# bytedance/ps-lite

Hardware: AMD Instinct MI355X
Metric: push+pull GB/s per worker + p50 round-trip µs, 1 MB & 64 MB, at 1/2/4/8 GPUs (higher is better)
Workload: dtype fp32; 1 GPU; model=dense push+pull (ps-lite test_benchmark PUSH_PULL), global_batch=128, seq_len=67108864, parallelism=byteps-joint x1 (worker+server per GPU), mode=dense, msg_bytes=67108864, batch_keys=False, overlap=True, op=assign

## Files before the change

csrc/coalesce_admit.h:

```cpp
#pragma once

#include <cstddef>
#include <cstdint>

namespace xps {
namespace kern {

struct Seg2 {
  void* dst0;
  void* dst1;
  const void* src;
  size_t nbytes;
};

static const int kMaxBatch2 = 64;

enum class Admit {
  kAdmit,
  kFlushFirst,
  kReject,
};

inline bool RangesOverlap(const void* a, const void* b, size_t alen, size_t blen) {
  uintptr_t p = reinterpret_cast<uintptr_t>(a), q = reinterpret_cast<uintptr_t>(b);
  return p < q + blen && q < p + alen;
}

inline Admit CoalesceAdmit(const Seg2* open, int n_open, const Seg2& s) {
  uintptr_t bits = reinterpret_cast<uintptr_t>(s.dst0) | reinterpret_cast<uintptr_t>(s.dst1) |
                   reinterpret_cast<uintptr_t>(s.src) | static_cast<uintptr_t>(s.nbytes);
  if (s.nbytes == 0 || (bits & 15u) != 0) return Admit::kReject;
  if (RangesOverlap(s.dst0, s.dst1, s.nbytes, s.nbytes) ||
      RangesOverlap(s.dst0, s.src, s.nbytes, s.nbytes) ||
      RangesOverlap(s.dst1, s.src, s.nbytes, s.nbytes)) {
    return Admit::kReject;
  }
  if (n_open >= kMaxBatch2) return Admit::kReject;
  for (int i = 0; i < n_open; ++i) {
    const Seg2& o = open[i];
    const void* theirs[3] = {o.dst0, o.dst1, o.src};
    for (const void* t : theirs) {
      if (RangesOverlap(s.dst0, t, s.nbytes, o.nbytes) ||
          RangesOverlap(s.dst1, t, s.nbytes, o.nbytes)) {
        return Admit::kFlushFirst;
      }
    }
    if (RangesOverlap(s.src, o.dst0, s.nbytes, o.nbytes) ||
        RangesOverlap(s.src, o.dst1, s.nbytes, o.nbytes)) {
      return Admit::kFlushFirst;
    }
  }
  return Admit::kAdmit;
}

}
}
```

csrc/customer.cc:

```cpp
#include "customer.h"

#include <chrono>

#include "postoffice.h"

namespace xps {

Customer::Customer(int app_id, int customer_id, RecvHandle handle, Postoffice* po)
    : app_id_(app_id), customer_id_(customer_id), handle_(std::move(handle)), po_(po) {
  po_->AddCustomer(this);
  thread_ = std::thread([this] { Receiving(); });
}

Customer::~Customer() {
  po_->RemoveCustomer(this);
  Message term;
  term.meta.control.cmd = Control::TERMINATE;
  queue_.Push(std::move(term));
  if (thread_.joinable()) thread_.join();
}

int Customer::NewRequest(int recver) {
  std::lock_guard<std::mutex> lk(mu_);
  int expected = recver >= 8 ? 1 : static_cast<int>(po_->GetNodeIDs(recver).size());
  tracker_.emplace_back();
  tracker_.back().expected = expected;
  return static_cast<int>(tracker_.size()) - 1;
}

Customer::Slot* Customer::GetSlot(int ts) {
  std::lock_guard<std::mutex> lk(mu_);
  XPS_CHECK_LT(static_cast<size_t>(ts), tracker_.size());
  return &tracker_[ts];
}

void Customer::WaitRequest(int ts) {
  Slot* s = GetSlot(ts);
  auto deadline = std::chrono::steady_clock::now() + std::chrono::microseconds(150);
  while (s->received.load(std::memory_order_acquire) < s->expected) {
    if (std::chrono::steady_clock::now() >= deadline) break;
  }
  if (s->received.load(std::memory_order_acquire) >= s->expected) return;
  static const int timeout_s = Environment::Get()->GetInt("XPS_WAIT_TIMEOUT_S", 0);
  std::unique_lock<std::mutex> lk(mu_);
  auto done = [s] { return s->received.load(std::memory_order_acquire) >= s->expected; };
  if (timeout_s <= 0) {
    cv_.wait(lk, done);
    return;
  }
  if (!cv_.wait_for(lk, std::chrono::seconds(timeout_s), done)) {
    XPS_LOG(Fatal) << "request ts=" << ts << " (app " << app_id_ << ") got "
                   << s->received.load() << "/" << s->expected << " responses after "
                   << timeout_s << " s — responder dead? (XPS_WAIT_TIMEOUT_S)";
  }
}

bool Customer::IsFinished(int ts) {
  Slot* s = GetSlot(ts);
  return s->received.load(std::memory_order_acquire) >= s->expected;
}

int Customer::NumResponse(int ts) {
  return GetSlot(ts)->received.load(std::memory_order_acquire);
}

void Customer::AddResponse(int ts, int num) {
  Slot* s = GetSlot(ts);
  int got = s->received.fetch_add(num, std::memory_order_acq_rel) + num;
  if (got >= s->expected) {
    std::lock_guard<std::mutex> lk(mu_);
    cv_.notify_all();
  }
}

thread_local int g_in_handler = 0;

bool InCustomerHandler() { return g_in_handler > 0; }

void Customer::RunHandle(Message& msg) {
  g_in_handler++;
  handle_(msg);
  g_in_handler--;
  if (!msg.meta.request) AddResponse(msg.meta.timestamp, 1);
}

void Customer::ProcessInline(Message& msg) {
  XPS_STAGE(customer_process);
  std::lock_guard<std::mutex> lk(handle_mu_);
  RunHandle(msg);
}

void Customer::Receiving() {
  while (true) {
    Message msg;
    queue_.WaitAndPop(&msg);
    if (msg.meta.control.cmd == Control::TERMINATE) break;
    std::lock_guard<std::mutex> lk(handle_mu_);
    RunHandle(msg);
  }
}

}
```

csrc/gpu_plane.cc:

```cpp
#include "gpu_plane.h"

#include <fcntl.h>
#include <hip/hip_runtime.h>
#include <semaphore.h>
#include <sys/prctl.h>
#include <time.h>
#include <unistd.h>

#include <cstring>

#include "hip_pool.h"
#include "host_par.h"
#include "host_pool.h"
#include "kernels.h"
#include "postoffice.h"
#include "wire.h"

namespace xps {

static const size_t kInlineMax = 4096;

#define XPS_HIP_CHECK(cmd)                                                            \
  do {                                                                                \
    hipError_t e_ = (cmd);                                                            \
    XPS_CHECK(e_ == hipSuccess) << "HIP error: " << hipGetErrorString(e_) << " in " #cmd; \
  } while (0)

std::atomic<uint64_t> g_zero_copy_recv{0};
std::atomic<uint64_t> g_fused_assign{0};

bool FusedAssignEnabled() {
  static const bool on = Environment::Get()->GetInt("XPS_FUSED_ASSIGN", 1) != 0;
  return on;
}

std::atomic<uint64_t> g_fused_launches{0};

bool CoalesceEnabled() {
  static const bool on = Environment::Get()->GetInt("XPS_COALESCE", 1) != 0;
  return on;
}

namespace {
struct CoTicket {
  const void* plane = nullptr;
  int peer = 0;
  std::shared_ptr<void> cev;
};
thread_local CoTicket t_co_ticket;

int64_t NowUs() {
  struct timespec ts;
  clock_gettime(CLOCK_MONOTONIC, &ts);
  return static_cast<int64_t>(ts.tv_sec) * 1000000 + ts.tv_nsec / 1000;
}
const int64_t kHoldQuietUs = 2000;
const size_t kCoBusyBytes = 16u << 20;

std::mutex g_map_mu;
struct HandleKey {
  char h[kIpcHandleBytes];
  bool operator==(const HandleKey& o) const { return memcmp(h, o.h, kIpcHandleBytes) == 0; }
};
struct HandleHash {
  size_t operator()(const HandleKey& k) const {
    size_t v = 1469598103934665603ull;
    for (char c : k.h) {
      v ^= static_cast<unsigned char>(c);
      v *= 1099511628211ull;
    }
    return v;
  }
};
std::unordered_map<HandleKey, void*, HandleHash> g_mapped;

class IpcOpenLock {
 public:
  IpcOpenLock() {
    sem_ = sem_open("/xps_ipc_open_lock", O_CREAT, 0600, 1);
  }
  void Lock() {
    if (sem_ == SEM_FAILED) return;
    struct timespec ts;
    clock_gettime(CLOCK_REALTIME, &ts);
    ts.tv_sec += 60;
    if (sem_timedwait(sem_, &ts) != 0) {
      XPS_LOG(Warning) << "ipc-open lock timeout; proceeding unlocked";
      timed_out_ = true;
    }
  }
  void Unlock() {
    if (sem_ != SEM_FAILED && !timed_out_) sem_post(sem_);
    timed_out_ = false;
  }

 private:
  sem_t* sem_ = SEM_FAILED;
  bool timed_out_ = false;
};
IpcOpenLock g_ipc_lock;
}

GpuPlane::GpuPlane(Postoffice* po, int device) : po_(po), device_(device) {
  my_host_hash_ = HostHash();
  inline_deliver_ = Environment::Get()->GetInt("XPS_INLINE_HANDLER", 1) != 0;
  lanes_ = Environment::Get()->GetInt("XPS_STREAMS_PER_PEER", 2);
  if (lanes_ < 1) lanes_ = 1;
  if (lanes_ > 2) lanes_ = 2;
  co_hold_ = Environment::Get()->GetInt("XPS_COALESCE_HOLD", 0) != 0;
  int cap_mb = Environment::Get()->GetInt("XPS_COALESCE_CAP_MB", 1024);
  co_byte_cap_ = static_cast<size_t>(cap_mb < 1 ? 1 : cap_mb) << 20;
}

GpuPlane::~GpuPlane() { Stop(); }

void GpuPlane::FillSelf(Node* self) {
  static std::once_flag gc_once;
  std::call_once(gc_once, [] { HostShmPool::GcStaleSegments(); });
  self->dev_id = device_;
  auto* pool = HbmPool::Get();
  if (device_ >= 0 && pool->initialized()) {
    self->pool_capacity = pool->capacity();
    self->pool_slab_bytes = pool->slab_bytes();
    self->pool_handles.resize(pool->slab_count());
    for (size_t i = 0; i < pool->slab_count(); ++i) {
      memcpy(self->pool_handles[i].data(), pool->slab_handle(i), kIpcHandleBytes);
    }
  }
  auto* hpool = HostShmPool::Get();
  hpool->Init(self->shm_uid);
  self->host_pool_uid = hpool->uid();
  self->host_pool_capacity = hpool->capacity();
  if (!started_) {
    auto* env = Environment::Get();
    if (!env->GetInt("XPS_PROBE_NO_RING", 0)) {
      XPS_CHECK(in_ring_.Create(self->shm_uid)) << "cannot create shm ring";
    }
    started_ = true;
    if (!env->GetInt("XPS_PROBE_NO_POLL", 0)) {
      poll_running_ = true;
      poll_thread_ = std::thread([this] { RingPollLoop(); });
    }
    if (device_ >= 0 && !env->GetInt("XPS_PROBE_NO_COMP", 0)) {
      comp_thread_ = std::thread([this] { CompletionLoop(); });
    }
  }
}

void GpuPlane::Stop() {
  if (stop_.exchange(true)) return;
  PrintStageStats(device_ >= 0 ? "gpu plane" : "host plane");
  if (poll_thread_.joinable()) poll_thread_.join();
  if (comp_thread_.joinable()) comp_thread_.join();
  {
    std::lock_guard<std::mutex> lk(local_mu_);
    for (auto& lm : local_q_) po_->van()->Deliver(std::move(lm.first));
    local_q_.clear();
  }
  if (device_ >= 0) {
    std::vector<Peer*> all;
    {
      std::shared_lock<std::shared_timed_mutex> lk(peers_mu_);
      for (auto& kv : peers_) all.push_back(kv.second.get());
    }
    for (Peer* peer : all) {
      CoFlush(peer);
      std::lock_guard<std::mutex> lk(peer->co.mu);
      peer->co.inflight.clear();
    }
  }
  {
    std::lock_guard<std::mutex> lk(pend_mu_);
    for (auto& kv : pending_) {
      for (auto& p : kv.second) {
        if (p.cev) {
          (void)hipEventSynchronize(p.cev->ev.load(std::memory_order_acquire));
          if (p.local_po) {
            DeliverLocal(p.local_po, p.resend, p.bytes);
          } else {
            Peer* peer = GetPeer(p.peer_id);
            auto ring = peer ? RingOf(peer) : nullptr;
            if (!ring || !ring->Push(p.payload.data(),
                                     static_cast<uint32_t>(p.payload.size()))) {
              (void)po_->van()->SendOverTcp(p.resend, p.peer_id);
            }
          }
          continue;
        }
        (void)hipEventSynchronize(p.ev);
        if (p.local_po) {
          DeliverLocal(p.local_po, p.resend, p.bytes);
          (void)hipEventDestroy(p.ev);
          continue;
        }
        Peer* peer = GetPeer(p.peer_id);
        auto ring = peer ? RingOf(peer) : nullptr;
        bool sent = ring && ring->Push(p.payload.data(),
                                       static_cast<uint32_t>(p.payload.size()));
        if (!sent) {
          (void)po_->van()->SendOverTcp(p.resend, p.peer_id);
        }
        (void)hipEventDestroy(p.ev);
      }
    }
    pending_.clear();
  }
  in_ring_.CloseAndUnlink();
  HostShmPool::Get()->Unlink();
  std::lock_guard<std::mutex> lk(ev_mu_);
  for (auto ev : event_pool_) (void)hipEventDestroy(ev);
  event_pool_.clear();
}

void GpuPlane::OnPeer(const Node& peer) {
  if (peer.host_hash != my_host_hash_) return;
  std::unique_lock<std::shared_timed_mutex> lk(peers_mu_);
  auto& p = peers_[peer.id];
  if (!p) p.reset(new Peer());
  if (p->node.shm_uid != 0 && peer.shm_uid != 0 && p->node.shm_uid != peer.shm_uid) {
    std::lock_guard<std::mutex> lk2(p->mu);
    XPS_LOG(Warning) << "peer " << peer.id << " was recovered (new process); resetting "
                        "plane caches for it";
    p->ring_ok.store(false, std::memory_order_release);
    p->ring_tried = false;
    std::atomic_store_explicit(&p->ring, std::shared_ptr<ShmRing>(),
                               std::memory_order_release);
    p->pool_tried = false;
    p->slab_bases.clear();
    p->local_po.store(nullptr, std::memory_order_release);
  }
  p->node = peer;
}

void GpuPlane::ImportPeers() {
  std::vector<int> ids;
  {
    std::shared_lock<std::shared_timed_mutex> lk(peers_mu_);
    for (auto& kv : peers_) ids.push_back(kv.first);
  }
  for (int id : ids) {
    Peer* p = GetPeer(id);
    if (p->node.pool_capacity) {
      bool ok = ImportPeerSlabs(p);
      XPS_VLOG(1) << "imported pool of peer " << id << " (" << p->node.pool_handles.size()
                  << " slabs): " << (ok ? "ok" : "FAILED");
    }
  }
}

GpuPlane::Peer* GpuPlane::GetPeer(int id) {
  {
    std::shared_lock<std::shared_timed_mutex> lk(peers_mu_);
    auto it = peers_.find(id);
    if (it != peers_.end()) return it->second.get();
  }
  std::unique_lock<std::shared_timed_mutex> lk(peers_mu_);
  auto& p = peers_[id];
  if (!p) {
    p.reset(new Peer());
    p->node = po_->van()->GetNode(id);
  }
  return p.get();
}

bool GpuPlane::EnsureRing(Peer* p) {
  if (p->ring_ok.load(std::memory_order_acquire)) return true;
  std::lock_guard<std::mutex> lk(p->mu);
  {
    auto cur = std::atomic_load_explicit(&p->ring, std::memory_order_acquire);
    if (cur && cur->ok()) return true;
  }
  if (p->ring_tried) return false;
  p->ring_tried = true;
  if (p->node.shm_uid == 0) return false;
  auto ring = std::make_shared<ShmRing>();
  if (!ring->Open(p->node.shm_uid)) return false;
  std::atomic_store_explicit(&p->ring, std::shared_ptr<ShmRing>(std::move(ring)),
                             std::memory_order_release);
  p->ring_ok.store(true, std::memory_order_release);
  return true;
}

std::shared_ptr<ShmRing> GpuPlane::RingOf(Peer* p) {
  if (!EnsureRing(p)) return nullptr;
  return std::atomic_load_explicit(&p->ring, std::memory_order_acquire);
}

bool GpuPlane::ImportPeerSlabs(Peer* p) {
  {
    std::lock_guard<std::mutex> lk(p->mu);
    if (p->pool_tried) return !p->slab_bases.empty();
    p->pool_tried = true;
  }
  std::vector<void*> bases;
  auto* pool = HbmPool::Get();
  size_t nslabs = p->node.pool_handles.size();
  bool same_process =
      pool->initialized() && nslabs == pool->slab_count() &&
      memcmp(p->node.pool_handles[0].data(), pool->slab_handle(0), kIpcHandleBytes) == 0;
  int peer_dev = p->node.dev_id;
  if (!same_process && peer_dev >= 0 && peer_dev != device_ &&
      Environment::Get()->GetInt("XPS_PEER_ACCESS_CHECK", 1)) {
    int ndev = 0;
    (void)hipGetDeviceCount(&ndev);
    if (peer_dev < ndev) {
      int can = 0;
      (void)hipDeviceCanAccessPeer(&can, device_, peer_dev);
      if (!can) {
        XPS_LOG(Warning) << "device " << device_ << " cannot peer-access device " << peer_dev
                         << " (peer node " << p->node.id
                         << "): keeping this peer on the TCP path";
        std::lock_guard<std::mutex> lk(p->mu);
        p->slab_bases.clear();
        return false;
      }
      XPS_HIP_CHECK(hipSetDevice(device_));
      hipError_t pe = hipDeviceEnablePeerAccess(peer_dev, 0);
      if (pe != hipSuccess && pe != hipErrorPeerAccessAlreadyEnabled) {
        XPS_LOG(Warning) << "hipDeviceEnablePeerAccess(" << peer_dev
                         << ") failed: " << hipGetErrorString(pe)
                         << " (continuing; hipIpc lazy enable may still cover it)";
      }
    }
  }
  for (size_t i = 0; i < nslabs; ++i) {
    void* base = nullptr;
    if (same_process) {
      base = pool->slab_base(i);
    } else {
      HandleKey key;
      memcpy(key.h, p->node.pool_handles[i].data(), kIpcHandleBytes);
      std::lock_guard<std::mutex> lk(g_map_mu);
      auto it = g_mapped.find(key);
      if (it != g_mapped.end()) {
        base = it->second;
      } else {
        XPS_HIP_CHECK(hipSetDevice(device_));
        hipIpcMemHandle_t h;
        memcpy(&h, p->node.pool_handles[i].data(), sizeof(h));
        XPS_VLOG(3) << "ipc-open slab " << i << " of peer " << p->node.id;
        g_ipc_lock.Lock();
        hipError_t e = hipIpcOpenMemHandle(&base, h, hipIpcMemLazyEnablePeerAccess);
        g_ipc_lock.Unlock();
        XPS_VLOG(3) << "ipc-open slab " << i << " of peer " << p->node.id << " -> " << base;
        if (e != hipSuccess) {
          XPS_LOG(Warning) << "hipIpcOpenMemHandle(peer " << p->node.id << " slab " << i
                           << ") failed: " << hipGetErrorString(e)
                           << " — peer stays on the TCP path";
          base = nullptr;
        } else {
          char probe[8];
          hipError_t e2 = hipMemcpy(probe, base, sizeof(probe), hipMemcpyDeviceToHost);
          if (e2 != hipSuccess) {
            XPS_LOG(Warning) << "peer " << p->node.id << " slab " << i
                             << " mapped but unreadable (" << hipGetErrorString(e2)
                             << ") — peer stays on the TCP path";
            base = nullptr;
          }
        }
        g_mapped[key] = base;
      }
    }
    if (!base) {
      std::lock_guard<std::mutex> lk(p->mu);
      p->slab_bases.clear();
      return false;
    }
    bases.push_back(base);
  }
  std::lock_guard<std::mutex> lk(p->mu);
  p->slab_bases = std::move(bases);
  return !p->slab_bases.empty();
}

char* GpuPlane::ResolvePeer(Peer* p, uint64_t global_off, uint64_t len) {
  if (!ImportPeerSlabs(p)) return nullptr;
  uint64_t slab_bytes = p->node.pool_slab_bytes;
  if (slab_bytes == 0) return nullptr;
  size_t idx = static_cast<size_t>(global_off / slab_bytes);
  uint64_t local = global_off % slab_bytes;
  std::lock_guard<std::mutex> lk(p->mu);
  if (idx >= p->slab_bases.size() || len > slab_bytes - local) {
    XPS_LOG(Warning) << "peer offset out of bounds: off=" << global_off << " len=" << len
                     << " slab=" << idx;
    return nullptr;
  }
  return static_cast<char*>(p->slab_bases[idx]) + local;
}

hipStream_t GpuPlane::StreamLane(int node_id, int lane) {
  if (lane >= lanes_) lane = lanes_ - 1;
  Peer* p = GetPeer(node_id);
  if (lane == 0) CoFlush(p);
  return RawLane(p, lane);
}

bool GpuPlane::LanesSplit(int node_id) {
  return lanes_ >= 2 && GetPeer(node_id)->node.dev_id != device_;
}


void GpuPlane::CoLaunchLocked(Peer* p) {
  Coalescer& co = p->co;
  if (co.n == 0) return;
  hipStream_t stream = RawLane(p, 0);
  XPS_HIP_CHECK(hipSetDevice(device_));
  if (co.n == 1) {
    const kern::Seg2& s = co.segs[0];
    kern::DenseAssign2(s.dst0, s.dst1, s.src, s.nbytes, stream);
  } else {
    kern::BatchedAssign2(co.segs, co.n, stream);
  }
  g_fused_launches.fetch_add(1, std::memory_order_relaxed);
  hipEvent_t ev = GetEvent();
  XPS_HIP_CHECK(hipEventRecord(ev, stream));
  co.open->bytes = co.bytes;
  co.open->ev.store(ev, std::memory_order_release);
  co.inflight.push_back(std::move(co.open));
  co.open.reset();
  co.n = 0;
  co.bytes = 0;
  co.n_open.store(0, std::memory_order_release);
}

bool GpuPlane::CoBusyLocked(Peer* p) {
  CoPruneLocked(p);
  size_t bytes = 0;
  for (auto& f : p->co.inflight) bytes += f->bytes;
  return p->co.inflight.size() >= 2 && bytes >= kCoBusyBytes;
}

void GpuPlane::CoPruneLocked(Peer* p) {
  auto& fl = p->co.inflight;
  while (!fl.empty()) {
    CoEvent* f = fl.front().get();
    if (!f->done.load(std::memory_order_acquire) &&
        hipEventQuery(f->ev.load(std::memory_order_acquire)) != hipSuccess) {
      break;
    }
    fl.pop_front();
  }
}

void GpuPlane::CoFlush(Peer* p) {
  if (p->co.n_open.load(std::memory_order_acquire) == 0) return;
  std::lock_guard<std::mutex> lk(p->co.mu);
  CoLaunchLocked(p);
}

std::shared_ptr<GpuPlane::CoEvent> GpuPlane::CoAppend(Peer* p, const kern::Seg2& seg) {
  if (!CoalesceEnabled()) return nullptr;
  Coalescer& co = p->co;
  std::lock_guard<std::mutex> lk(co.mu);
  kern::Admit a = kern::CoalesceAdmit(co.segs, co.n, seg);
  if (a != kern::Admit::kAdmit) CoLaunchLocked(p);
  if (a == kern::Admit::kReject) return nullptr;
  if (!co.open) co.open = std::make_shared<CoEvent>(this);
  std::shared_ptr<CoEvent> cev = co.open;
  co.segs[co.n++] = seg;
  co.bytes += seg.nbytes;
  co.n_open.store(co.n, std::memory_order_release);
  if (co.n >= kern::kMaxBatch || co.bytes >= co_byte_cap_) {
    CoLaunchLocked(p);
  } else if (co_hold_) {
    co.last_append_us = NowUs();
  } else {
    if (!CoBusyLocked(p)) CoLaunchLocked(p);
  }
  return cev;
}

bool GpuPlane::CoFrontUnlaunched(Peer* p, const std::shared_ptr<CoEvent>& cev) {
  Coalescer& co = p->co;
  std::lock_guard<std::mutex> lk(co.mu);
  if (co.open != cev) return true;
  if (co_hold_ && NowUs() - co.last_append_us < kHoldQuietUs) return false;
  CoLaunchLocked(p);
  return true;
}

void GpuPlane::CoRetired(Peer* p) {
  Coalescer& co = p->co;
  std::lock_guard<std::mutex> lk(co.mu);
  bool busy = CoBusyLocked(p);
  if (!co_hold_ && !busy) CoLaunchLocked(p);
}

bool GpuPlane::CoalesceAppend(int peer_id, const kern::Seg2& seg) {
  if (device_ < 0) return false;
  std::shared_ptr<CoEvent> cev = CoAppend(GetPeer(peer_id), seg);
  if (!cev) return false;
  t_co_ticket.plane = this;
  t_co_ticket.peer = peer_id;
  t_co_ticket.cev = std::move(cev);
  return true;
}

std::shared_ptr<GpuPlane::CoEvent> GpuPlane::TakeTicket(int peer_id) {
  if (!t_co_ticket.cev || t_co_ticket.plane != this || t_co_ticket.peer != peer_id) {
    return nullptr;
  }
  auto cev = std::static_pointer_cast<CoEvent>(t_co_ticket.cev);
  t_co_ticket.cev.reset();
  return cev;
}

void GpuPlane::CoalesceEnd(int peer_id) {
  if (!t_co_ticket.cev) return;
  t_co_ticket.cev.reset();
  CoFlush(GetPeer(peer_id));
}

hipStream_t GpuPlane::RawLane(Peer* p, int lane) {
  hipStream_t s = p->streams[lane].load(std::memory_order_acquire);
  if (s) return s;
  std::lock_guard<std::mutex> lk(p->mu);
  s = p->streams[lane].load(std::memory_order_relaxed);
  if (!s) {
    XPS_HIP_CHECK(hipSetDevice(device_));
    XPS_HIP_CHECK(hipStreamCreateWithFlags(&s, hipStreamNonBlocking));
    p->streams[lane].store(s, std::memory_order_release);
  }
  return s;
}

hipStream_t GpuPlane::StreamForPeer(int node_id) { return StreamLane(node_id, 0); }

hipStream_t GpuPlane::PullStreamForPeer(int node_id) {
  Peer* p = GetPeer(node_id);
  if (lanes_ < 2 || p->node.dev_id == device_) return StreamLane(node_id, 0);
  CoFlush(p);
  return StreamLane(node_id, 1);
}

std::vector<std::tuple<int, int64_t, int64_t>> GpuPlane::PeerBytes() {
  std::vector<std::tuple<int, int64_t, int64_t>> out;
  std::shared_lock<std::shared_timed_mutex> lk(peers_mu_);
  for (auto& kv : peers_) {
    int64_t tx = kv.second->tx_bytes.load(std::memory_order_relaxed);
    int64_t rx = kv.second->rx_bytes.load(std::memory_order_relaxed);
    if (tx || rx) out.emplace_back(kv.first, tx, rx);
  }
  return out;
}

hipEvent_t GpuPlane::GetEvent() {
  {
    std::lock_guard<std::mutex> lk(ev_mu_);
    if (!event_pool_.empty()) {
      hipEvent_t ev = event_pool_.back();
      event_pool_.pop_back();
      return ev;
    }
  }
  hipEvent_t ev;
  XPS_HIP_CHECK(hipSetDevice(device_));
  XPS_HIP_CHECK(hipEventCreateWithFlags(&ev, hipEventDisableTiming));
  return ev;
}

void GpuPlane::PutEvent(hipEvent_t ev) {
  std::lock_guard<std::mutex> lk(ev_mu_);
  event_pool_.push_back(ev);
}

Postoffice* GpuPlane::LocalPeer(Peer* p) {
  Postoffice* po = p->local_po.load(std::memory_order_acquire);
  if (po) return po;
  if (p->node.id == kEmptyNodeID) return nullptr;
  po = Postoffice::FindByNodeId(p->node.id);
  if (po) p->local_po.store(po, std::memory_order_release);
  return po;
}

static bool KernelLessAck(const Message& msg) {
  return !msg.meta.request && msg.meta.push && (msg.meta.option & kOptInPlace) &&
         (!msg.meta.pull || (msg.meta.option & kOptEntryPush));
}

static bool NeedsStaging(const Message& msg) {
  return !msg.meta.request && msg.meta.pull && msg.data.size() > 1 &&
         msg.data[1].on_device() && msg.data[1].size() > 0 &&
         (!(msg.meta.option & kOptPullAddr) || (msg.meta.option & kOptHostAddr));
}

bool GpuPlane::CanSend(const Message& msg, const Node& peer) {
  if (!started_ || stop_.load()) return false;
  if (peer.host_hash != my_host_hash_ || peer.shm_uid == 0) return false;
  if (LocalPeer(GetPeer(peer.id))) return !NeedsStaging(msg);
  if (peer.pool_capacity) {
    Peer* p = GetPeer(peer.id);
    std::lock_guard<std::mutex> lk(p->mu);
    if (p->pool_tried && p->slab_bases.empty()) return false;
  }
  size_t est = 160 + msg.meta.body.size();
  for (size_t i = 0; i < msg.data.size(); ++i) {
    const auto& d = msg.data[i];
    if (d.on_device()) {
      uint64_t off;
      if (!HbmPool::Get()->OffsetOf(d.data(), &off)) return false;
      est += 24;
      if (!msg.meta.request && msg.meta.pull && i == 1) {
        if (!(msg.meta.option & kOptPullAddr) || (msg.meta.option & kOptHostAddr) ||
            peer.pool_capacity == 0) {
          return false;
        }
      }
    } else if (d.size() > kInlineMax) {
      uint64_t off;
      if (!HostShmPool::Get()->OffsetOf(d.data(), &off)) return false;
      est += 24;
    } else {
      est += 24 + d.size();
    }
  }
  return est <= ShmRing::MaxPayload();
}

bool GpuPlane::Serialize(const Message& msg, const std::vector<char>& by_ref, std::string* out) {
  XPS_STAGE(serialize);
  std::string meta;
  PackMeta(msg.meta, &meta);
  out->clear();
  out->reserve(meta.size() + 64);
  ByteWriter w(out);
  w.U64(meta.size());
  w.Raw(meta.data(), meta.size());
  w.U8(static_cast<uint8_t>(msg.data.size()));
  for (size_t i = 0; i < msg.data.size(); ++i) {
    const auto& d = msg.data[i];
    if (by_ref[i] == 1) {
      uint64_t off = 0;
      XPS_CHECK(HbmPool::Get()->OffsetOf(d.data(), &off));
      w.U8(1);
      w.U64(off);
      w.U64(d.size());
    } else if (by_ref[i] == 2) {
      uint64_t off = 0;
      XPS_CHECK(HostShmPool::Get()->OffsetOf(d.data(), &off));
      w.U8(2);
      w.U64(off);
      w.U64(d.size());
    } else {
      w.U8(0);
      w.U64(d.size());
      w.Raw(d.data(), d.size());
    }
  }
  return out->size() <= ShmRing::MaxPayload();
}

void GpuPlane::DeliverLocal(Postoffice* lpo, Message& msg, int64_t bytes) {
  Van* van = lpo->van();
  if (!van) {
    XPS_LOG(Warning) << "local peer " << msg.meta.recver << " already finalized; dropping";
    return;
  }
  auto* rplane = dynamic_cast<GpuPlane*>(van->plane());
  static const bool queue_req = Environment::Get()->GetInt("XPS_LOCAL_QUEUE_REQ", 0) != 0;
  if (InCustomerHandler() || (queue_req && msg.meta.request)) {
    if (rplane && rplane->poll_running_) {
      rplane->EnqueueLocal(std::move(msg), bytes);
      return;
    }
    XPS_CHECK(!InCustomerHandler())
        << "in-handler local send needs the receiver's poll thread";
  }
  van->recv_bytes_ += bytes;
  for (auto& d : msg.data) {
    if (d.size() && (d.on_device() || d.size() > kInlineMax)) {
      g_zero_copy_recv.fetch_add(1, std::memory_order_relaxed);
    }
  }
  if (inline_deliver_) {
    van->DeliverInline(msg);
  } else {
    van->Deliver(std::move(msg));
  }
}

bool GpuPlane::LocalPullRead(int peer_id, void* dst, uint64_t entry_off, size_t len,
                             Message resp) {
  if (device_ < 0 || !started_ || stop_.load()) return false;
  Peer* p = GetPeer(peer_id);
  char* src = ResolvePeer(p, entry_off, len);
  if (!src) return false;
  XPS_STAGE(local_pull_read);
  hipStream_t stream;
  if (Postoffice* elpo = LocalPeer(p)) {
    auto* rplane = dynamic_cast<GpuPlane*>(elpo->van() ? elpo->van()->plane() : nullptr);
    if (!rplane) return false;
    static const bool queue_req = Environment::Get()->GetInt("XPS_LOCAL_QUEUE_REQ", 0) != 0;
    if (!inline_deliver_ || queue_req) return false;
    stream = rplane->StreamForPeer(po_->node_id());
  } else {
    stream = StreamForPeer(peer_id);
  }
  XPS_HIP_CHECK(hipSetDevice(device_));
  kern::DenseAssign(dst, src, len, stream);
  g_zero_copy_recv.fetch_add(1, std::memory_order_relaxed);
  hipEvent_t ev = GetEvent();
  XPS_HIP_CHECK(hipEventRecord(ev, stream));
  int64_t bytes = static_cast<int64_t>(len) + 64;
  {
    std::lock_guard<std::mutex> lk(pend_mu_);
    pending_[peer_id].push_back(Pending{ev, peer_id, std::string(), std::move(resp), Message(),
                                        bytes, po_});
  }
  pending_count_.fetch_add(1);
  p->rx_bytes.fetch_add(bytes, std::memory_order_relaxed);
  return true;
}

bool GpuPlane::EntryPushPull(Message& msg, Peer* p, int64_t* bytes_out) {
  if (!FusedAssignEnabled()) return false;
  if (!(msg.meta.option & kOptPullAddr) || (msg.meta.option & kOptHostAddr)) return false;
  static const bool local_one_sided =
      Environment::Get()->GetInt("XPS_LOCAL_ONE_SIDED", 0) != 0;
  Postoffice* elpo = LocalPeer(p);
  GpuPlane* rplane =
      elpo ? dynamic_cast<GpuPlane*>(elpo->van() ? elpo->van()->plane() : nullptr) : nullptr;
  bool can = elpo ? (local_one_sided && rplane != nullptr) : EnsureRing(p);
  if (!can) return false;
  SArray<char> vals = msg.data[1];
  size_t len = vals.size();
  if (len == 0) return false;
  char* entry = ResolvePeer(p, msg.meta.entry_addr, len);
  char* dst = static_cast<char*>(HbmPool::Get()->PtrOf(msg.meta.addr, len));
  if (!entry || !dst || !kern::Disjoint3(entry, dst, vals.data(), len)) return false;
  XPS_STAGE(entry_push_pull);
  std::shared_ptr<CoEvent> cev;
  static const bool co_one_sided =
      Environment::Get()->GetInt("XPS_COALESCE_ONE_SIDED", 0) != 0;
  if (!elpo && co_one_sided) cev = CoAppend(p, kern::Seg2{entry, dst, vals.data(), len});
  hipStream_t stream = nullptr;
  if (!cev) {
    stream = elpo ? rplane->StreamForPeer(po_->node_id()) : StreamForPeer(p->node.id);
    XPS_HIP_CHECK(hipSetDevice(device_));
    kern::DenseAssign2(entry, dst, vals.data(), len, stream);
    g_fused_launches.fetch_add(1, std::memory_order_relaxed);
  }
  g_fused_assign.fetch_add(1, std::memory_order_relaxed);
  g_zero_copy_recv.fetch_add(1, std::memory_order_relaxed);
  Message meta_msg;
  meta_msg.meta = msg.meta;
  meta_msg.meta.option |= kOptInPlace;
  meta_msg.meta.val_len = static_cast<int64_t>(len);
  meta_msg.meta.data_type.clear();
  for (size_t i = 0; i < msg.data.size(); ++i) {
    if (i == 1 || msg.data[i].on_device()) continue;
    meta_msg.data.push_back(msg.data[i]);
    meta_msg.meta.data_type.push_back(msg.meta.data_type[i]);
  }
  int64_t bytes = 64 + static_cast<int64_t>(len);
  Message keepalive;
  keepalive.data.push_back(vals);
  std::string payload;
  if (!elpo) {
    std::vector<char> br(meta_msg.data.size(), 0);
    XPS_CHECK(Serialize(meta_msg, br, &payload));
  }
  hipEvent_t ev = nullptr;
  if (!cev) {
    ev = GetEvent();
    XPS_HIP_CHECK(hipEventRecord(ev, stream));
  }
  {
    std::lock_guard<std::mutex> lk(pend_mu_);
    pending_[p->node.id].push_back(Pending{ev, p->node.id, std::move(payload),
                                           std::move(meta_msg), std::move(keepalive), bytes,
                                           elpo, std::move(cev)});
  }
  pending_count_.fetch_add(1);
  p->tx_bytes.fetch_add(bytes, std::memory_order_relaxed);
  *bytes_out = bytes;
  return true;
}

void GpuPlane::EnqueueLocal(Message msg, int64_t bytes) {
  {
    std::lock_guard<std::mutex> lk(local_mu_);
    local_q_.emplace_back(std::move(msg), bytes);
  }
  local_count_.fetch_add(1, std::memory_order_release);
}

int64_t GpuPlane::SendLocal(Message& msg, Peer* p, Postoffice* lpo) {
  XPS_STAGE(plane_send_local);
  bool response = !msg.meta.request;
  int64_t bytes = 64;
  for (auto& d : msg.data) bytes += static_cast<int64_t>(d.size());

  if (response && msg.meta.pull && msg.data.size() > 1 && !msg.data[1].on_device() &&
      msg.data[1].size() > 0 && (msg.meta.option & kOptPullAddr) &&
      (msg.meta.option & kOptHostAddr)) {
    void* base = HostShmPool::MapPeer(p->node.host_pool_uid, p->node.host_pool_capacity);
    SArray<char> vals = msg.data[1];
    if (base && msg.meta.addr <= p->node.host_pool_capacity &&
        vals.size() <= p->node.host_pool_capacity - msg.meta.addr) {
      HostPar::CopyBytes(static_cast<char*>(base) + msg.meta.addr, vals.data(), vals.size());
      g_zero_copy_recv.fetch_add(1, std::memory_order_relaxed);
      Message meta_msg;
      meta_msg.meta = msg.meta;
      meta_msg.meta.option |= kOptInPlace;
      meta_msg.meta.val_len = static_cast<int64_t>(vals.size());
      meta_msg.meta.data_type.clear();
      for (size_t i = 0; i < msg.data.size(); ++i) {
        if (i == 1 || msg.data[i].on_device()) continue;
        SArray<char> copy(msg.data[i].size());
        memcpy(copy.data(), msg.data[i].data(), msg.data[i].size());
        meta_msg.data.push_back(copy);
        meta_msg.meta.data_type.push_back(msg.meta.data_type[i]);
      }
      DeliverLocal(lpo, meta_msg, bytes);
      p->tx_bytes.fetch_add(bytes, std::memory_order_relaxed);
      return bytes;
    }
  }

  if (response && msg.meta.pull && msg.data.size() > 1 && msg.data[1].on_device() &&
      (msg.meta.option & kOptPullAddr) && !(msg.meta.option & kOptHostAddr)) {
    SArray<char> vals = msg.data[1];
    char* dst = ResolvePeer(p, msg.meta.addr, vals.size());
    if (!dst) {
      for (int l = 0; l < lanes_; ++l) (void)hipStreamSynchronize(StreamLane(p->node.id, l));
      return -1;
    }
    hipStream_t stream = (msg.meta.option & kOptPullLane) ? PullStreamForPeer(p->node.id)
                                                          : StreamForPeer(p->node.id);
    XPS_HIP_CHECK(hipSetDevice(device_));
    kern::DenseAssign(dst, vals.data(), vals.size(), stream);
    g_zero_copy_recv.fetch_add(1, std::memory_order_relaxed);
    Message meta_msg;
    meta_msg.meta = msg.meta;
    meta_msg.meta.option |= kOptInPlace;
    meta_msg.meta.val_len = static_cast<int64_t>(vals.size());
    meta_msg.meta.data_type.clear();
    for (size_t i = 0; i < msg.data.size(); ++i) {
      if (i == 1 || msg.data[i].on_device()) continue;
      meta_msg.data.push_back(msg.data[i]);
      meta_msg.meta.data_type.push_back(msg.meta.data_type[i]);
    }
    msg.data.clear();
    Message keepalive;
    keepalive.data.push_back(vals);
    hipEvent_t ev = GetEvent();
    XPS_HIP_CHECK(hipEventRecord(ev, stream));
    {
      std::lock_guard<std::mutex> lk(pend_mu_);
      pending_[p->node.id].push_back(Pending{ev, p->node.id, std::string(),
                                             std::move(meta_msg), std::move(keepalive), bytes,
                                             lpo});
    }
    pending_count_.fetch_add(1);
    p->tx_bytes.fetch_add(bytes, std::memory_order_relaxed);
    return bytes;
  }

  bool kernel_less_ack = KernelLessAck(msg);
  if (response && device_ >= 0 && !kernel_less_ack) {
    XPS_STAGE(local_defer);
    std::shared_ptr<CoEvent> cev = TakeTicket(p->node.id);
    hipEvent_t ev = nullptr;
    if (!cev) {
      hipStream_t stream = (msg.meta.option & kOptPullLane) ? PullStreamForPeer(p->node.id)
                                                            : StreamForPeer(p->node.id);
      ev = GetEvent();
      XPS_HIP_CHECK(hipSetDevice(device_));
      XPS_HIP_CHECK(hipEventRecord(ev, stream));
    }
    Message resend = msg;
    {
      std::lock_guard<std::mutex> lk(pend_mu_);
      pending_[p->node.id].push_back(Pending{ev, p->node.id, std::string(), std::move(resend),
                                             Message(), bytes, lpo, std::move(cev)});
    }
    pending_count_.fetch_add(1);
  } else {
    Message copy = msg;
    if (response) {
      for (auto& d : copy.data) {
        if (!d.on_device() && d.size()) {
          SArray<char> snap(d.size());
          memcpy(snap.data(), d.data(), d.size());
          d = snap;
        }
      }
    }
    DeliverLocal(lpo, copy, bytes);
  }
  p->tx_bytes.fetch_add(bytes, std::memory_order_relaxed);
  return bytes;
}

int64_t GpuPlane::Send(Message& msg, const Node& peer_node) {
  XPS_STAGE(plane_send);
  XPS_VLOG(3) << "plane send -> " << peer_node.id << ": " << msg.DebugString();
  Peer* p = GetPeer(peer_node.id);
  {
    std::lock_guard<std::mutex> lk(p->mu);
    if (p->node.shm_uid == 0) p->node = peer_node;
  }

  static const bool local_one_sided =
      Environment::Get()->GetInt("XPS_LOCAL_ONE_SIDED", 0) != 0;
  if (msg.meta.request && msg.meta.push && !msg.meta.pull &&
      (msg.meta.option & kOptEntryPush) && device_ >= 0 && msg.data.size() > 1 &&
      msg.data[1].on_device()) {
    Postoffice* elpo = LocalPeer(p);
    GpuPlane* rplane =
        elpo ? dynamic_cast<GpuPlane*>(elpo->van() ? elpo->van()->plane() : nullptr) : nullptr;
    bool can = elpo ? (local_one_sided && rplane != nullptr) : EnsureRing(p);
    SArray<char> vals = msg.data[1];
    char* dst = can ? ResolvePeer(p, msg.meta.addr, vals.size()) : nullptr;
    if (dst) {
      XPS_STAGE(entry_push);
      hipStream_t stream = elpo ? rplane->StreamForPeer(po_->node_id())
                                : StreamForPeer(p->node.id);
      XPS_HIP_CHECK(hipSetDevice(device_));
      kern::DenseAssign(dst, vals.data(), vals.size(), stream);
      g_zero_copy_recv.fetch_add(1, std::memory_order_relaxed);
      Message meta_msg;
      meta_msg.meta = msg.meta;
      meta_msg.meta.option |= kOptInPlace;
      meta_msg.meta.val_len = static_cast<int64_t>(vals.size());
      meta_msg.meta.data_type.clear();
      for (size_t i = 0; i < msg.data.size(); ++i) {
        if (i == 1 || msg.data[i].on_device()) continue;
        meta_msg.data.push_back(msg.data[i]);
        meta_msg.meta.data_type.push_back(msg.meta.data_type[i]);
      }
      int64_t bytes = 64 + static_cast<int64_t>(vals.size());
      Message keepalive;
      keepalive.data.push_back(vals);
      std::string payload;
      if (!elpo) {
        std::vector<char> br(meta_msg.data.size(), 0);
        XPS_CHECK(Serialize(meta_msg, br, &payload));
      }
      hipEvent_t ev = GetEvent();
      XPS_HIP_CHECK(hipEventRecord(ev, stream));
      {
        std::lock_guard<std::mutex> lk(pend_mu_);
        pending_[p->node.id].push_back(Pending{ev, p->node.id, std::move(payload),
                                               std::move(meta_msg), std::move(keepalive),
                                               bytes, elpo});
      }
      pending_count_.fetch_add(1);
      p->tx_bytes.fetch_add(bytes, std::memory_order_relaxed);
      return bytes;
    }
    msg.meta.option &= ~kOptEntryPush;
  }

  if (msg.meta.request && msg.meta.push && msg.meta.pull && (msg.meta.option & kOptEntryPush)) {
    int64_t bytes = 0;
    if (device_ >= 0 && msg.data.size() > 1 && msg.data[1].on_device() &&
        EntryPushPull(msg, p, &bytes)) {
      msg.meta.option |= kOptInPlace;
      return bytes;
    }
    msg.meta.option &= ~kOptEntryPush;
    msg.meta.entry_addr = 0;
  }

  if (Postoffice* lpo = LocalPeer(p)) return SendLocal(msg, p, lpo);
  bool response = !msg.meta.request;
  auto sync_peer_lanes = [this, &peer_node] {
    for (int l = 0; l < lanes_; ++l) (void)hipStreamSynchronize(StreamLane(peer_node.id, l));
  };
  if (!EnsureRing(p)) {
    if (response && device_ >= 0) sync_peer_lanes();
    return -1;
  }

  if (response && msg.meta.pull && msg.data.size() > 1 && !msg.data[1].on_device() &&
      msg.data[1].size() > 0 && (msg.meta.option & kOptPullAddr) &&
      (msg.meta.option & kOptHostAddr)) {
    void* base = HostShmPool::MapPeer(p->node.host_pool_uid, p->node.host_pool_capacity);
    SArray<char> vals = msg.data[1];
    if (base && msg.meta.addr <= p->node.host_pool_capacity &&
        vals.size() <= p->node.host_pool_capacity - msg.meta.addr) {
      HostPar::CopyBytes(static_cast<char*>(base) + msg.meta.addr, vals.data(), vals.size());
      Message meta_msg;
      meta_msg.meta = msg.meta;
      meta_msg.meta.option |= kOptInPlace;
      meta_msg.meta.val_len = static_cast<int64_t>(vals.size());
      for (size_t i = 0; i < msg.data.size(); ++i) {
        if (i == 1 || msg.data[i].on_device() || msg.data[i].size() > kInlineMax) continue;
        meta_msg.data.push_back(msg.data[i]);
        meta_msg.meta.data_type.push_back(msg.meta.data_type[i]);
      }
      std::vector<char> br(meta_msg.data.size(), 0);
      std::string payload;
      if (!Serialize(meta_msg, br, &payload)) {
        meta_msg.data.clear();
        meta_msg.meta.data_type.clear();
        XPS_CHECK(Serialize(meta_msg, {}, &payload));
      }
      int64_t bytes = static_cast<int64_t>(vals.size() + payload.size());
      auto ring = RingOf(p);
      if (!ring || !ring->Push(payload.data(), static_cast<uint32_t>(payload.size()))) return -1;
      p->tx_bytes.fetch_add(bytes, std::memory_order_relaxed);
      return bytes;
    }
    return -1;
  }

  if (response && msg.meta.pull && msg.data.size() > 1 && msg.data[1].on_device() &&
      (msg.meta.option & kOptPullAddr)) {
    SArray<char> vals = msg.data[1];
    char* dst = ResolvePeer(p, msg.meta.addr, vals.size());
    if (!dst) {
      sync_peer_lanes();
      return -1;
    }
    hipStream_t stream = (msg.meta.option & kOptPullLane) ? PullStreamForPeer(peer_node.id)
                                                          : StreamForPeer(peer_node.id);
    XPS_HIP_CHECK(hipSetDevice(device_));
    kern::DenseAssign(dst, vals.data(), vals.size(), stream);
    Message meta_msg;
    meta_msg.meta = msg.meta;
    meta_msg.meta.option |= kOptInPlace;
    meta_msg.meta.val_len = static_cast<int64_t>(vals.size());
    meta_msg.meta.data_type.clear();
    for (size_t i = 0; i < msg.data.size(); ++i) {
      if (i == 1 || msg.data[i].on_device()) continue;
      meta_msg.data.push_back(msg.data[i]);
      meta_msg.meta.data_type.push_back(msg.meta.data_type[i]);
    }
    std::vector<char> by_ref(meta_msg.data.size(), 0);
    std::string payload;
    if (!Serialize(meta_msg, by_ref, &payload)) {
      meta_msg.data.clear();
      meta_msg.meta.data_type.clear();
      XPS_CHECK(Serialize(meta_msg, {}, &payload));
    }
    int64_t bytes = static_cast<int64_t>(vals.size() + payload.size());
    msg.data.clear();
    Message keepalive;
    keepalive.data.push_back(vals);
    DeferSendInternal(p, peer_node.id, stream, std::move(meta_msg), std::move(keepalive),
                      std::move(payload), bytes);
    p->tx_bytes.fetch_add(bytes, std::memory_order_relaxed);
    return bytes;
  }

  std::vector<char> by_ref(msg.data.size(), 0);
  int64_t ref_bytes = 0;
  for (size_t i = 0; i < msg.data.size(); ++i) {
    if (msg.data[i].on_device()) {
      by_ref[i] = 1;
      ref_bytes += msg.data[i].size();
      if (i == 1) msg.meta.option |= kOptValsByRef;
    } else if (msg.data[i].size() > kInlineMax) {
      by_ref[i] = 2;
      ref_bytes += msg.data[i].size();
    }
  }
  std::string payload;
  if (!Serialize(msg, by_ref, &payload)) {
    if (response && device_ >= 0) (void)hipStreamSynchronize(StreamForPeer(peer_node.id));
    return -1;
  }
  int64_t bytes = static_cast<int64_t>(payload.size()) + ref_bytes;
  bool kernel_less_ack = KernelLessAck(msg);
  if (response && device_ >= 0 && !kernel_less_ack) {
    hipStream_t stream = (msg.meta.option & kOptPullLane) ? PullStreamForPeer(peer_node.id)
                                                          : StreamForPeer(peer_node.id);
    Message resend = msg;
    DeferSendInternal(p, peer_node.id, stream, std::move(resend), Message(), std::move(payload),
                      bytes);
  } else {
    auto ring = RingOf(p);
    if (!ring || !ring->Push(payload.data(), static_cast<uint32_t>(payload.size()))) return -1;
    XPS_VLOG(3) << "plane send done -> " << peer_node.id;
  }
  p->tx_bytes.fetch_add(bytes, std::memory_order_relaxed);
  return bytes;
}

void GpuPlane::DeferSendInternal(Peer* p, int peer_id, hipStream_t stream, Message resend,
                                 Message keepalive, std::string payload, int64_t bytes) {
  XPS_STAGE(defer_queue);
  XPS_CHECK_GE(device_, 0) << "deferred sends are a GPU-plane feature";
  hipEvent_t ev = GetEvent();
  XPS_HIP_CHECK(hipSetDevice(device_));
  XPS_HIP_CHECK(hipEventRecord(ev, stream));
  {
    std::lock_guard<std::mutex> lk(pend_mu_);
    pending_[peer_id].push_back(Pending{ev, peer_id, std::move(payload), std::move(resend),
                                        std::move(keepalive), bytes});
  }
  pending_count_.fetch_add(1);
  XPS_VLOG(3) << "deferred send queued -> " << peer_id;
}

void GpuPlane::CompletionLoop() {
  XPS_HIP_CHECK(hipSetDevice(device_));
  prctl(PR_SET_TIMERSLACK, 1000);
  const int kSpin = Environment::Get()->GetInt("XPS_POLL_SPIN", 200000);
  int idle = 0;
  std::vector<int> ids;
  while (!stop_.load()) {
    bool did = false;
    if (pending_count_.load(std::memory_order_acquire) > 0) {
      ids.clear();
      {
        std::lock_guard<std::mutex> lk(pend_mu_);
        for (auto& kv : pending_) {
          if (!kv.second.empty()) ids.push_back(kv.first);
        }
      }
      for (int id : ids) {
        while (!stop_.load()) {
          hipEvent_t front_ev = nullptr;
          std::shared_ptr<CoEvent> cev;
          {
            std::lock_guard<std::mutex> lk(pend_mu_);
            auto& dq = pending_[id];
            if (dq.empty()) break;
            front_ev = dq.front().ev;
            cev = dq.front().cev;
          }
          bool retired = false;
          if (cev) {
            front_ev = cev->ev.load(std::memory_order_acquire);
            if (!front_ev) {
              if (!CoFrontUnlaunched(GetPeer(id), cev)) break;
              continue;
            }
          }
          if (!cev || !cev->done.load(std::memory_order_acquire)) {
            hipError_t e = hipEventQuery(front_ev);
            if (e == hipErrorNotReady) break;
            XPS_CHECK(e == hipSuccess) << "hipEventQuery: " << hipGetErrorString(e);
            if (cev) {
              cev->done.store(true, std::memory_order_release);
              retired = true;
            }
          }
          XPS_STAGE(defer_release);
          if (retired) CoRetired(GetPeer(id));
          Pending front;
          {
            std::lock_guard<std::mutex> lk(pend_mu_);
            auto& dq = pending_[id];
            front = std::move(dq.front());
            dq.pop_front();
          }
          pending_count_.fetch_sub(1);
          if (front.local_po) {
            DeliverLocal(front.local_po, front.resend, front.bytes);
            if (front.ev) PutEvent(front.ev);
            did = true;
            continue;
          }
          Peer* peer = GetPeer(front.peer_id);
          auto ring = peer ? RingOf(peer) : nullptr;
          bool sent = ring && ring->Push(front.payload.data(),
                                         static_cast<uint32_t>(front.payload.size()));
          if (sent) {
            XPS_VLOG(3) << "deferred send done -> " << front.peer_id;
          } else {
            XPS_LOG(Warning) << "deferred plane send failed -> " << front.peer_id
                             << "; falling back to TCP";
            if (po_->van()->SendOverTcp(front.resend, front.peer_id) < 0) {
              XPS_LOG(Warning) << "TCP fallback to " << front.peer_id
                               << " failed too (peer dead?)";
            }
          }
          if (front.ev) PutEvent(front.ev);
          did = true;
        }
      }
    }
    if (did) {
      idle = 0;
    } else if (++idle > kSpin) {
      usleep(20);
    }
  }
}

void GpuPlane::RingPollLoop() {
  if (device_ >= 0) XPS_HIP_CHECK(hipSetDevice(device_));
  prctl(PR_SET_TIMERSLACK, 1000);
  const int kSpin = Environment::Get()->GetInt("XPS_POLL_SPIN", 200000);
  std::vector<char> buf(ShmRing::MaxPayload());
  int idle = 0;
  std::deque<std::pair<Message, int64_t>> local;
  while (!stop_.load()) {
    if (local_count_.load(std::memory_order_acquire) > 0) {
      {
        std::lock_guard<std::mutex> lk(local_mu_);
        local.swap(local_q_);
      }
      local_count_.fetch_sub(static_cast<int>(local.size()));
      for (auto& lm : local) {
        XPS_STAGE(local_handle);
        po_->van()->recv_bytes_ += lm.second;
        for (auto& d : lm.first.data) {
          if (d.size() && (d.on_device() || d.size() > kInlineMax)) {
            g_zero_copy_recv.fetch_add(1, std::memory_order_relaxed);
          }
        }
        if (inline_deliver_) {
          po_->van()->DeliverInline(lm.first);
        } else {
          po_->van()->Deliver(std::move(lm.first));
        }
      }
      idle = 0;
      local.clear();
    }
    uint32_t n = in_ring_.Pop(buf.data());
    if (n == 0) {
      if (++idle > kSpin) usleep(20);
      continue;
    }
    idle = 0;
    XPS_STAGE(ring_handle);
    ByteReader r(buf.data(), n);
    uint64_t meta_len = r.U64();
    Message msg;
    {
      std::vector<char> meta(meta_len);
      r.Raw(meta.data(), meta_len);
      UnpackMeta(meta.data(), meta_len, &msg.meta);
    }
    int nblobs = r.U8();
    int64_t ref_bytes = 0;
    bool ok = true;
    for (int i = 0; i < nblobs; ++i) {
      int kind = r.U8();
      if (kind == 0) {
        uint64_t len = r.U64();
        SArray<char> d(len);
        r.Raw(d.data(), len);
        msg.data.push_back(d);
      } else if (kind == 1) {
        uint64_t off = r.U64();
        uint64_t len = r.U64();
        Peer* sender = GetPeer(msg.meta.sender);
        char* ptr = sender ? ResolvePeer(sender, off, len) : nullptr;
        if (!ptr) {
          XPS_LOG(Warning) << "dropping by-ref blob: sender pool not mapped (from "
                           << msg.meta.sender << ")";
          ok = false;
          break;
        }
        msg.data.push_back(SArray<char>(ptr, len, device_));
        ref_bytes += len;
        g_zero_copy_recv.fetch_add(1, std::memory_order_relaxed);
      } else {
        uint64_t off = r.U64();
        uint64_t len = r.U64();
        Peer* sender = GetPeer(msg.meta.sender);
        void* base = sender ? HostShmPool::MapPeer(sender->node.host_pool_uid,
                                                   sender->node.host_pool_capacity)
                            : nullptr;
        if (!base || off > sender->node.host_pool_capacity ||
            len > sender->node.host_pool_capacity - off) {
          XPS_LOG(Warning) << "dropping host-ref blob: sender host pool not mapped (from "
                           << msg.meta.sender << ")";
          ok = false;
          break;
        }
        msg.data.push_back(SArray<char>(static_cast<char*>(base) + off, len, kCPU));
        ref_bytes += len;
        g_zero_copy_recv.fetch_add(1, std::memory_order_relaxed);
      }
    }
    if (!ok) continue;
    XPS_VLOG(3) << "ring recv: " << msg.DebugString();
    po_->van()->recv_bytes_ += n + ref_bytes;
    if (msg.meta.sender != kEmptyNodeID) {
      GetPeer(msg.meta.sender)->rx_bytes.fetch_add(n + ref_bytes, std::memory_order_relaxed);
    }
    if (inline_deliver_) {
      po_->van()->DeliverInline(msg);
    } else {
      po_->van()->Deliver(std::move(msg));
    }
  }
}

std::shared_ptr<DataPlane> CreateGpuPlane(Postoffice* po, int device) {
  return std::make_shared<GpuPlane>(po, device);
}

}
```

csrc/gpu_plane.h:

```cpp
#pragma once

#include <hip/hip_runtime.h>

#include <atomic>
#include <deque>
#include <memory>
#include <shared_mutex>
#include <thread>
#include <tuple>
#include <unordered_map>
#include <vector>

#include "kernels.h"
#include "shm_ring.h"
#include "van.h"

namespace xps {

extern std::atomic<uint64_t> g_zero_copy_recv;
extern std::atomic<uint64_t> g_fused_assign;
bool FusedAssignEnabled();
extern std::atomic<uint64_t> g_fused_launches;
bool CoalesceEnabled();

class Postoffice;

class GpuPlane : public DataPlane {
 public:
  GpuPlane(Postoffice* po, int device);
  ~GpuPlane() override;

  void FillSelf(Node* self) override;
  void ImportPeers() override;
  bool CanSend(const Message& msg, const Node& peer) override;
  int64_t Send(Message& msg, const Node& peer) override;
  void OnPeer(const Node& peer) override;
  void Stop() override;

  hipStream_t StreamForPeer(int node_id);
  hipStream_t PullStreamForPeer(int node_id);
  int lanes() const { return lanes_; }
  bool LanesSplit(int node_id);

  bool CoalesceAppend(int peer_id, const kern::Seg2& seg);
  void CoalesceEnd(int peer_id);
  std::vector<std::tuple<int, int64_t, int64_t>> PeerBytes();
  int device() const { return device_; }

  bool LocalPullRead(int peer_id, void* dst, uint64_t entry_off, size_t len, Message resp);
  hipEvent_t GetEvent();
  void PutEvent(hipEvent_t ev);
  char* PeerDst(int peer_id, uint64_t global_off, uint64_t len) {
    return ResolvePeer(GetPeer(peer_id), global_off, len);
  }

 private:
  struct CoEvent {
    explicit CoEvent(GpuPlane* pl) : plane(pl) {}
    ~CoEvent() {
      if (hipEvent_t e = ev.load(std::memory_order_acquire)) plane->PutEvent(e);
    }
    GpuPlane* plane;
    std::atomic<hipEvent_t> ev{nullptr};
    std::atomic<bool> done{false};
    size_t bytes = 0;
  };
  struct Coalescer {
    std::mutex mu;
    kern::Seg2 segs[kern::kMaxBatch];
    int n = 0;
    std::atomic<int> n_open{0};
    size_t bytes = 0;
    std::shared_ptr<CoEvent> open;
    std::deque<std::shared_ptr<CoEvent>> inflight;
    int64_t last_append_us = 0;
  };

  struct Peer {
    Node node;
    Coalescer co;
    std::atomic<Postoffice*> local_po{nullptr};
    std::shared_ptr<ShmRing> ring;
    bool ring_tried = false;
    std::atomic<bool> ring_ok{false};
    std::vector<void*> slab_bases;
    bool pool_tried = false;
    std::atomic<hipStream_t> streams[2] = {{nullptr}, {nullptr}};
    std::atomic<int64_t> tx_bytes{0};
    std::atomic<int64_t> rx_bytes{0};
    std::mutex mu;
  };

  struct Pending {
    hipEvent_t ev;
    int peer_id;
    std::string payload;
    Message resend;
    Message keepalive;
    int64_t bytes;
    Postoffice* local_po = nullptr;
    std::shared_ptr<CoEvent> cev;
  };

  Peer* GetPeer(int id);
  Postoffice* LocalPeer(Peer* p);
  int64_t SendLocal(Message& msg, Peer* p, Postoffice* lpo);
  void DeliverLocal(Postoffice* lpo, Message& msg, int64_t bytes);
  void EnqueueLocal(Message msg, int64_t bytes);
  bool EnsureRing(Peer* p);
  std::shared_ptr<ShmRing> RingOf(Peer* p);
  bool ImportPeerSlabs(Peer* p);
  char* ResolvePeer(Peer* p, uint64_t global_off, uint64_t len);
  bool Serialize(const Message& msg, const std::vector<char>& by_ref, std::string* out);
  void RingPollLoop();
  void CompletionLoop();
  hipStream_t StreamLane(int node_id, int lane);
  hipStream_t RawLane(Peer* p, int lane);
  std::shared_ptr<CoEvent> CoAppend(Peer* p, const kern::Seg2& seg);
  void CoLaunchLocked(Peer* p);
  void CoPruneLocked(Peer* p);
  bool CoBusyLocked(Peer* p);
  void CoFlush(Peer* p);
  bool CoFrontUnlaunched(Peer* p, const std::shared_ptr<CoEvent>& cev);
  void CoRetired(Peer* p);
  std::shared_ptr<CoEvent> TakeTicket(int peer_id);
  bool EntryPushPull(Message& msg, Peer* p, int64_t* bytes_out);
  void DeferSendInternal(Peer* p, int peer_id, hipStream_t stream, Message resend,
                         Message keepalive, std::string payload, int64_t bytes);

  Postoffice* po_;
  int device_;
  int lanes_ = 2;
  bool co_hold_ = false;
  size_t co_byte_cap_ = 1ull << 30;
  uint64_t my_host_hash_;
  ShmRing in_ring_;
  bool started_ = false;
  bool inline_deliver_ = true;

  std::shared_timed_mutex peers_mu_;
  std::unordered_map<int, std::unique_ptr<Peer>> peers_;

  std::thread poll_thread_;
  std::thread comp_thread_;
  std::atomic<bool> stop_{false};

  std::mutex pend_mu_;
  std::unordered_map<int, std::deque<Pending>> pending_;
  std::atomic<int> pending_count_{0};

  std::mutex local_mu_;
  std::deque<std::pair<Message, int64_t>> local_q_;
  std::atomic<int> local_count_{0};
  bool poll_running_ = false;

  std::mutex ev_mu_;
  std::vector<hipEvent_t> event_pool_;
};

std::shared_ptr<DataPlane> CreateGpuPlane(Postoffice* po, int device);

}
```

csrc/kv_app.h:

```cpp
#pragma once

#include <unistd.h>

#include <algorithm>
#include <atomic>
#include <chrono>
#include <condition_variable>
#include <functional>
#include <mutex>
#include <set>
#include <unordered_map>
#include <vector>

#include "gpu_plane.h"
#include "hip_pool.h"
#include "hip_util.h"
#include "host_par.h"
#include "host_pool.h"
#include "simple_app.h"

namespace xps {

static const int kCmdDefault = 0;
static const int kCmdAssign = 1;
static const int kCmdSum = 2;

template <typename V>
struct KVPairs {
  SArray<Key> keys;
  SArray<V> vals;
  SArray<int> lens;
  SArray<Key> keys_dev;
};

struct KVMeta {
  int cmd = 0;
  bool push = false;
  bool pull = false;
  int sender = kEmptyNodeID;
  int timestamp = -1;
  int customer_id = 0;
  Key key = 0;
  uint64_t addr = 0;
  uint64_t entry_addr = 0;
  int64_t val_len = 0;
  int option = 0;
  int src_dev = kCPU;
  int dst_dev = kCPU;
};

template <typename V>
class KVWorker : public SimpleApp {
 public:
  using Callback = std::function<void()>;
  using SlicedKVs = std::vector<std::pair<bool, KVPairs<V>>>;
  using Slicer = std::function<void(const KVPairs<V>&, const std::vector<Range>&, SlicedKVs*)>;

  explicit KVWorker(int app_id, int customer_id, int instance_idx = 0)
      : SimpleApp(Postoffice::GetWorker(instance_idx), DeferCustomer{}) {
    slicer_ = [this](const KVPairs<V>& s, const std::vector<Range>& r, SlicedKVs* out) {
      DefaultSlicer(s, r, out);
    };
    obj_.reset(new Customer(app_id, customer_id,
                            [this](const Message& m) { Process(m); }, po_));
  }

  int Push(const std::vector<Key>& keys, const std::vector<V>& vals,
           const std::vector<int>& lens = {}, int cmd = 0, const Callback& cb = nullptr) {
    return ZPush(SArray<Key>(keys), SArray<V>(vals), SArray<int>(lens), cmd, cb);
  }

  int Pull(const std::vector<Key>& keys, std::vector<V>* vals, std::vector<int>* lens = nullptr,
           int cmd = 0, const Callback& cb = nullptr) {
    SArray<Key> skeys(keys);
    int ts = AddPullRequest_(skeys, vals, lens, cmd, cb);
    return ts;
  }

  int ZPush(const SArray<Key>& keys, const SArray<V>& vals, const SArray<int>& lens = {},
            int cmd = 0, const Callback& cb = nullptr, const SArray<Key>& keys_dev = {}) {
    int ts = obj_->NewRequest(kServerGroup);
    AddCallback(ts, cb);
    KVPairs<V> kvs;
    kvs.keys = keys;
    kvs.vals = vals;
    kvs.lens = lens;
    kvs.keys_dev = keys_dev;
    Send(ts, true, false, cmd, kvs);
    return ts;
  }

  int ZPushPull(const SArray<Key>& keys, const SArray<V>& vals, SArray<V>* outs,
                const SArray<int>& lens = {}, int cmd = 0, const Callback& cb = nullptr,
                const SArray<Key>& keys_dev = {}) {
    XPS_CHECK(outs && outs->size()) << "ZPushPull needs a pre-sized outs buffer";
    int ts = obj_->NewRequest(kServerGroup);
    {
      std::lock_guard<std::mutex> lk(mu_);
      pull_dst_[ts] = {outs, nullptr};
    }
    AddCallback(ts, cb);
    KVPairs<V> kvs;
    kvs.keys = keys;
    kvs.vals = vals;
    kvs.lens = lens;
    kvs.keys_dev = keys_dev;
    Send(ts, true, true, cmd, kvs, outs);
    return ts;
  }

  int ZPull(const SArray<Key>& keys, SArray<V>* vals, SArray<int>* lens = nullptr, int cmd = 0,
            const Callback& cb = nullptr, const SArray<Key>& keys_dev = {}) {
    XPS_CHECK(vals && vals->size()) << "ZPull needs a pre-sized vals buffer";
    int ts = obj_->NewRequest(kServerGroup);
    {
      std::lock_guard<std::mutex> lk(mu_);
      pull_dst_[ts] = {vals, lens};
    }
    AddCallback(ts, cb);
    KVPairs<V> kvs;
    kvs.keys = keys;
    kvs.vals = *vals;
    if (lens) kvs.lens = *lens;
    kvs.keys_dev = keys_dev;
    Send(ts, false, true, cmd, kvs);
    return ts;
  }

  void Wait(int timestamp) { obj_->WaitRequest(timestamp); }

  bool HasEntry(const Key& key, size_t nbytes) {
    const auto& ranges = po_->GetServerKeyRanges();
    size_t i = 0;
    while (i + 1 < ranges.size() && key >= ranges[i + 1].begin) ++i;
    if (ranges.empty()) return false;
    int sid = ServerRankToID(static_cast<int>(i));
    std::lock_guard<std::mutex> lk(mu_);
    const EntryRec* rec = FindEntryLocked(sid, key);
    return rec && rec->len == static_cast<int64_t>(nbytes) &&
           po_->van()->GetNode(sid).shm_uid == rec->uid;
  }

  void set_slicer(Slicer s) { slicer_ = std::move(s); }

  void DefaultSlicer(const KVPairs<V>& send, const std::vector<Range>& ranges, SlicedKVs* sliced) {
    sliced->resize(ranges.size());
    size_t n = send.keys.size();
    std::vector<size_t> pos(ranges.size() + 1);
    const Key* begin = send.keys.begin();
    const Key* end = send.keys.end();
    for (size_t i = 0; i < ranges.size(); ++i) {
      pos[i] = std::lower_bound(begin, end, ranges[i].begin) - begin;
    }
    pos[ranges.size()] = n;
    std::vector<size_t> val_off(n + 1, 0);
    if (!send.lens.empty()) {
      XPS_CHECK_EQ(send.lens.size(), n);
      for (size_t i = 0; i < n; ++i) val_off[i + 1] = val_off[i] + send.lens[i];
    } else if (n > 0) {
      size_t k = send.vals.size() / n;
      for (size_t i = 0; i <= n; ++i) val_off[i] = i * k;
    }
    for (size_t i = 0; i < ranges.size(); ++i) {
      size_t a = pos[i], b = pos[i + 1];
      auto& out = (*sliced)[i];
      out.first = b > a;
      if (!out.first) continue;
      out.second.keys = send.keys.Segment(a, b);
      if (!send.keys_dev.empty()) {
        out.second.keys_dev = send.keys_dev.Segment(a, b);
      }
      if (!send.vals.empty()) {
        out.second.vals = send.vals.Segment(val_off[a], val_off[b]);
      }
      if (!send.lens.empty()) {
        out.second.lens = send.lens.Segment(a, b);
      }
    }
  }

 private:
  int AddPullRequest_(const SArray<Key>& keys, std::vector<V>* vals, std::vector<int>* lens,
                      int cmd, const Callback& cb) {
    int ts = obj_->NewRequest(kServerGroup);
    {
      std::lock_guard<std::mutex> lk(mu_);
      vec_pull_dst_[ts] = {vals, lens};
    }
    AddCallback(ts, cb);
    KVPairs<V> kvs;
    kvs.keys = keys;
    Send(ts, false, true, cmd, kvs);
    return ts;
  }

  void AddCallback(int ts, const Callback& cb) {
    if (!cb) return;
    std::lock_guard<std::mutex> lk(mu_);
    callbacks_[ts] = cb;
  }

  void Send(int ts, bool push, bool pull, int cmd, KVPairs<V>& kvs, SArray<V>* dst = nullptr) {
    SlicedKVs sliced;
    slicer_(kvs, po_->GetServerKeyRanges(), &sliced);
    int skipped = 0;
    for (auto& s : sliced)
      if (!s.first) ++skipped;
    if (skipped) obj_->AddResponse(ts, skipped);
    {
      std::lock_guard<std::mutex> lk(mu_);
      expected_[ts] = static_cast<int>(sliced.size()) - skipped;
    }
    if (static_cast<int>(sliced.size()) == skipped) {
      RunCallback(ts);
      return;
    }
    size_t val_elem_off = 0;
    for (size_t i = 0; i < sliced.size(); ++i) {
      if (!sliced[i].first) continue;
      auto& s = sliced[i].second;
      Message msg;
      msg.meta.app_id = obj_->app_id();
      msg.meta.customer_id = obj_->customer_id();
      msg.meta.request = true;
      msg.meta.push = push;
      msg.meta.pull = pull;
      msg.meta.head = cmd;
      msg.meta.timestamp = ts;
      msg.meta.recver = ServerRankToID(static_cast<int>(i));
      if (s.keys.size() >= 1) msg.meta.key = s.keys[0];
      msg.meta.src_dev = push ? s.vals.device() : kvs.vals.device();
      msg.meta.dst_dev = msg.meta.src_dev;
      if (!s.keys_dev.empty()) {
        msg.AddData(s.keys_dev);
      } else {
        msg.AddData(s.keys);
      }
      if (push) {
        msg.meta.val_len = static_cast<int64_t>(s.vals.nbytes());
        msg.AddData(s.vals);
        if (!s.lens.empty()) msg.AddData(s.lens);
        {
          std::lock_guard<std::mutex> lk(mu_);
          auto nit = entry_cache_.find(msg.meta.recver);
          if (nit != entry_cache_.end() && !nit->second.empty()) {
            if (!pull && s.keys.size() == 1 && cmd != kCmdSum && s.vals.on_device()) {
              auto it = nit->second.find(s.keys[0]);
              if (it != nit->second.end() &&
                  it->second.len == static_cast<int64_t>(s.vals.nbytes()) &&
                  po_->van()->GetNode(msg.meta.recver).shm_uid == it->second.uid) {
                msg.meta.addr = it->second.off;
                msg.meta.option |= kOptEntryPush;
                it->second.one_sided = true;
              } else if (it != nit->second.end()) {
                it->second.one_sided = false;
              }
            } else {
              for (size_t ki = 0; ki < s.keys.size(); ++ki) {
                auto it = nit->second.find(s.keys[ki]);
                if (it != nit->second.end()) it->second.one_sided = false;
              }
            }
          }
        }
        if (pull && dst) {
          size_t elem_off = static_cast<size_t>(s.vals.data() - kvs.vals.data());
          const V* dptr = dst->data() + elem_off;
          uint64_t off = 0;
          if (dst->on_device()) {
            if (HbmPool::Get()->OffsetOf(dptr, &off)) {
              msg.meta.addr = off;
              msg.meta.option |= kOptPullAddr;
            }
          } else if (HostShmPool::Get()->OffsetOf(dptr, &off)) {
            msg.meta.addr = off;
            msg.meta.option |= kOptPullAddr | kOptHostAddr;
          }
          if (s.keys.size() == 1 && cmd != kCmdSum && s.vals.on_device() &&
              dst->on_device() && (msg.meta.option & kOptPullAddr) && FusedAssignEnabled()) {
            std::lock_guard<std::mutex> lk(mu_);
            const EntryRec* rec = FindEntryLocked(msg.meta.recver, s.keys[0]);
            if (rec && rec->len == static_cast<int64_t>(s.vals.nbytes()) &&
                po_->van()->GetNode(msg.meta.recver).shm_uid == rec->uid) {
              msg.meta.entry_addr = rec->off;
              msg.meta.option |= kOptEntryPush;
            }
          }
        }
      } else {
        if (s.keys.size() == 1 && cmd != kCmdSum && s.vals.on_device() &&
            s.vals.nbytes() > 0) {
          uint64_t eoff = 0;
          bool hit = false;
          {
            std::lock_guard<std::mutex> lk(mu_);
            auto nit = entry_cache_.find(msg.meta.recver);
            if (nit != entry_cache_.end()) {
              auto it = nit->second.find(s.keys[0]);
              if (it != nit->second.end() && it->second.one_sided &&
                  it->second.len == static_cast<int64_t>(s.vals.nbytes()) &&
                  po_->van()->GetNode(msg.meta.recver).shm_uid == it->second.uid) {
                eoff = it->second.off;
                hit = true;
              }
            }
          }
          if (hit) {
            auto* plane = dynamic_cast<GpuPlane*>(po_->van()->plane());
            if (plane) {
              Message resp;
              resp.meta.app_id = obj_->app_id();
              resp.meta.customer_id = obj_->customer_id();
              resp.meta.request = false;
              resp.meta.pull = true;
              resp.meta.head = cmd;
              resp.meta.timestamp = ts;
              resp.meta.sender = msg.meta.recver;
              resp.meta.recver = po_->node_id();
              resp.meta.key = s.keys[0];
              resp.meta.option = kOptInPlace;
              resp.meta.val_len = static_cast<int64_t>(s.vals.nbytes());
              if (plane->LocalPullRead(msg.meta.recver, s.vals.data(), eoff,
                                       s.vals.nbytes(), std::move(resp))) {
                continue;
              }
            }
          }
        }
        msg.meta.val_len = static_cast<int64_t>(s.vals.nbytes());
        if (!s.vals.empty()) {
          uint64_t off = 0;
          if (s.vals.on_device()) {
            if (HbmPool::Get()->OffsetOf(s.vals.data(), &off)) {
              msg.meta.addr = off;
              msg.meta.option |= kOptPullAddr;
            }
          } else if (HostShmPool::Get()->OffsetOf(s.vals.data(), &off)) {
            msg.meta.addr = off;
            msg.meta.option |= kOptPullAddr | kOptHostAddr;
          }
        }
        if (!s.lens.empty()) msg.AddData(s.lens);
      }
      po_->van()->Send(msg);
      if (push && pull && s.keys.size() == 1) {
        bool did = (msg.meta.option & kOptEntryPush) && (msg.meta.option & kOptInPlace);
        std::lock_guard<std::mutex> lk(mu_);
        auto nit = entry_cache_.find(msg.meta.recver);
        if (nit != entry_cache_.end()) {
          auto it = nit->second.find(s.keys[0]);
          if (it != nit->second.end()) it->second.one_sided = did;
        }
      }
      (void)val_elem_off;
    }
  }

  void Process(const Message& msg) {
    if (msg.meta.request) return;
    int ts = msg.meta.timestamp;
    bool last = false;
    KVPairs<V> kvs;
    if (msg.meta.pull) {
      if (!msg.data.empty()) {
        kvs.keys = SArray<Key>::View(msg.data[0]);
        if (msg.data.size() > 1) kvs.vals = SArray<V>::View(msg.data[1]);
        if (msg.data.size() > 2) kvs.lens = SArray<int>::View(msg.data[2]);
      }
      if (kvs.keys.empty() || kvs.keys.on_device()) {
        kvs.keys = SArray<Key>({msg.meta.key});
      }
    }
    {
      std::lock_guard<std::mutex> lk(mu_);
      if (msg.meta.pull) {
        if (msg.meta.push && (msg.meta.option & kOptEntryAddr)) {
          CacheEntryLocked(msg.meta.sender, msg.meta.key, msg.meta.entry_addr, msg.meta.val_len);
        }
        auto& got = recv_kvs_[ts];
        got.push_back(RecvSlice{kvs, msg.meta.option, msg.meta.val_len});
        last = static_cast<int>(got.size()) >= expected_[ts];
      } else {
        if (msg.meta.option & kOptEntryAddr) {
          CacheEntryLocked(msg.meta.sender, msg.meta.key, msg.meta.addr, msg.meta.val_len);
        }
        int n = ++push_acks_[ts];
        last = n >= expected_[ts];
      }
    }
    if (last) {
      if (msg.meta.pull) MergePull(ts);
      RunCallback(ts);
    }
  }

  void MergePull(int ts) {
    std::vector<RecvSlice> got;
    SArray<V>* dst_vals = nullptr;
    SArray<int>* dst_lens = nullptr;
    std::vector<V>* vec_vals = nullptr;
    std::vector<int>* vec_lens = nullptr;
    {
      std::lock_guard<std::mutex> lk(mu_);
      got.swap(recv_kvs_[ts]);
      recv_kvs_.erase(ts);
      auto it = pull_dst_.find(ts);
      if (it != pull_dst_.end()) {
        dst_vals = it->second.first;
        dst_lens = it->second.second;
        pull_dst_.erase(it);
      }
      auto it2 = vec_pull_dst_.find(ts);
      if (it2 != vec_pull_dst_.end()) {
        vec_vals = it2->second.first;
        vec_lens = it2->second.second;
        vec_pull_dst_.erase(it2);
      }
    }
    std::sort(got.begin(), got.end(), [](const RecvSlice& a, const RecvSlice& b) {
      Key ka = a.kvs.keys.empty() ? 0 : a.kvs.keys[0];
      Key kb = b.kvs.keys.empty() ? 0 : b.kvs.keys[0];
      return ka < kb;
    });
    if (vec_vals) {
      vec_vals->clear();
      if (vec_lens) vec_lens->clear();
      for (auto& g : got) {
        vec_vals->insert(vec_vals->end(), g.kvs.vals.begin(), g.kvs.vals.end());
        if (vec_lens) {
          for (size_t i = 0; i < g.kvs.lens.size(); ++i) vec_lens->push_back(g.kvs.lens[i]);
        }
      }
      return;
    }
    if (!dst_vals) return;
    size_t off = 0;
    for (auto& g : got) {
      if (g.option & kOptInPlace) {
        off += static_cast<size_t>(g.val_len) / sizeof(V);
        continue;
      }
      size_t n = g.kvs.vals.size();
      if (n == 0) continue;
      XPS_CHECK_LE(off + n, dst_vals->size()) << "pull response overflows dst";
      if (dst_vals->on_device()) {
        gpu::CopyHostToDevice(dst_vals->data() + off, g.kvs.vals.data(), n * sizeof(V),
                              dst_vals->device());
      } else {
        memcpy(dst_vals->data() + off, g.kvs.vals.data(), n * sizeof(V));
      }
      off += n;
    }
    if (dst_lens && !got.empty()) {
      size_t loff = 0;
      for (auto& g : got) {
        for (size_t i = 0; i < g.kvs.lens.size() && loff < dst_lens->size(); ++i) {
          (*dst_lens)[loff++] = g.kvs.lens[i];
        }
      }
    }
  }

  void RunCallback(int ts) {
    Callback cb;
    {
      std::lock_guard<std::mutex> lk(mu_);
      auto it = callbacks_.find(ts);
      if (it != callbacks_.end()) {
        cb = it->second;
        callbacks_.erase(it);
      }
      expected_.erase(ts);
      push_acks_.erase(ts);
    }
    if (cb) cb();
  }

  struct RecvSlice {
    KVPairs<V> kvs;
    int option = 0;
    int64_t val_len = 0;
  };

  struct EntryRec {
    uint64_t off;
    int64_t len;
    uint64_t uid;
    bool one_sided = false;
  };
  std::unordered_map<int, std::unordered_map<Key, EntryRec>> entry_cache_;

  void CacheEntryLocked(int server_id, Key key, uint64_t off, int64_t len) {
    entry_cache_[server_id][key] = EntryRec{off, len, po_->van()->GetNode(server_id).shm_uid};
  }

  const EntryRec* FindEntryLocked(int server_id, Key key) const {
    auto nit = entry_cache_.find(server_id);
    if (nit == entry_cache_.end()) return nullptr;
    auto it = nit->second.find(key);
    return it == nit->second.end() ? nullptr : &it->second;
  }

  Slicer slicer_;
  std::mutex mu_;
  std::unordered_map<int, Callback> callbacks_;
  std::unordered_map<int, int> expected_;
  std::unordered_map<int, int> push_acks_;
  std::unordered_map<int, std::vector<RecvSlice>> recv_kvs_;
  std::unordered_map<int, std::pair<SArray<V>*, SArray<int>*>> pull_dst_;
  std::unordered_map<int, std::pair<std::vector<V>*, std::vector<int>*>> vec_pull_dst_;
};

template <typename V>
class KVServer : public SimpleApp {
 public:
  using ReqHandle = std::function<void(const KVMeta&, const KVPairs<V>&, KVServer<V>*)>;

  explicit KVServer(int app_id, int instance_idx = 0)
      : SimpleApp(Postoffice::GetServer(instance_idx), DeferCustomer{}) {
    obj_.reset(new Customer(app_id, app_id, [this](const Message& m) { Process(m); }, po_));
  }

  void set_request_handle(ReqHandle h) {
    {
      std::lock_guard<std::mutex> lk(handle_mu_);
      request_handle2_ = std::move(h);
      handle_set_.store(true, std::memory_order_release);
    }
    handle_cv_.notify_all();
  }

  void Response(const KVMeta& req, const KVPairs<V>& res = KVPairs<V>()) {
    Message msg;
    msg.meta.app_id = obj_->app_id();
    msg.meta.customer_id = req.customer_id;
    msg.meta.request = false;
    msg.meta.push = req.push;
    msg.meta.pull = req.pull;
    msg.meta.head = req.cmd;
    msg.meta.timestamp = req.timestamp;
    msg.meta.recver = req.sender;
    msg.meta.key = req.key;
    msg.meta.addr = req.addr;
    msg.meta.entry_addr = req.entry_addr;
    msg.meta.option = req.option;
    msg.meta.val_len = req.val_len;
    msg.meta.src_dev = res.vals.device();
    msg.meta.dst_dev = req.dst_dev;
    if (req.pull && (!res.vals.empty() || !res.keys.empty())) {
      if (!res.vals.empty()) msg.meta.val_len = static_cast<int64_t>(res.vals.nbytes());
      msg.AddData(res.keys);
      msg.AddData(res.vals);
      if (!res.lens.empty()) msg.AddData(res.lens);
    }
    po_->van()->Send(msg);
  }

 private:
  void Process(const Message& msg) {
    if (msg.meta.simple_app) {
      SimpleApp::Process(msg);
      return;
    }
    KVMeta meta;
    meta.cmd = msg.meta.head;
    meta.push = msg.meta.push;
    meta.pull = msg.meta.pull;
    meta.sender = msg.meta.sender;
    meta.timestamp = msg.meta.timestamp;
    meta.customer_id = msg.meta.customer_id;
    meta.key = msg.meta.key;
    meta.addr = msg.meta.addr;
    meta.entry_addr = msg.meta.entry_addr;
    meta.val_len = msg.meta.val_len;
    meta.option = msg.meta.option;
    meta.src_dev = msg.meta.src_dev;
    meta.dst_dev = msg.meta.dst_dev;
    KVPairs<V> kvs;
    if (!msg.data.empty()) {
      kvs.keys = SArray<Key>::View(msg.data[0]);
      if (msg.data.size() > 1 && msg.meta.push) kvs.vals = SArray<V>::View(msg.data[1]);
      size_t lens_idx = msg.meta.push ? 2 : 1;
      if (msg.data.size() > lens_idx) kvs.lens = SArray<int>::View(msg.data[lens_idx]);
    } else if (msg.meta.key || msg.meta.val_len) {
      kvs.keys = SArray<Key>({msg.meta.key});
    }
    if (!handle_set_.load(std::memory_order_acquire)) {
      std::unique_lock<std::mutex> lk(handle_mu_);
      bool ok = handle_cv_.wait_for(lk, std::chrono::seconds(60),
                                    [this] { return handle_set_.load(); });
      XPS_CHECK(ok) << "KVServer has no request handle after 60 s";
    }
    request_handle2_(meta, kvs, this);
  }

  ReqHandle request_handle2_;
  std::mutex handle_mu_;
  std::condition_variable handle_cv_;
  std::atomic<bool> handle_set_{false};
};

inline void SumInto(float* dst, const float* src, size_t n) { HostPar::SumF32(dst, src, n); }
template <typename V>
inline void SumInto(V* dst, const V* src, size_t n) {
  for (size_t j = 0; j < n; ++j) dst[j] += src[j];
}

template <typename V>
struct KVServerDefaultHandle {
  void operator()(const KVMeta& req, const KVPairs<V>& kvs, KVServer<V>* server) {
    size_t n = kvs.keys.size();
    KVPairs<V> res;
    if (req.push) {
      XPS_CHECK(!kvs.vals.on_device()) << "default handle is CPU-only";
      size_t off = 0;
      for (size_t i = 0; i < n; ++i) {
        size_t len = kvs.lens.empty() ? kvs.vals.size() / n : kvs.lens[i];
        auto& entry = store[kvs.keys[i]];
        if (entry.size() < len) entry.resize(len, V(0));
        if (req.cmd == kCmdAssign) {
          HostPar::CopyBytes(entry.data(), kvs.vals.data() + off, len * sizeof(V));
        } else {
          SumInto(entry.data(), kvs.vals.data() + off, len);
        }
        off += len;
      }
    }
    if (req.pull) {
      res.keys = kvs.keys;
      if (n == 1) {
        auto& entry = store[kvs.keys[0]];
        res.vals = SArray<V>(entry.data(), entry.size(), kCPU);
        SArray<int> lens(1);
        lens[0] = static_cast<int>(entry.size());
        res.lens = lens;
      } else {
        size_t total = 0;
        for (size_t i = 0; i < n; ++i) total += store[kvs.keys[i]].size();
        res.vals.Resize(total);
        SArray<int> lens(n);
        size_t off = 0;
        for (size_t i = 0; i < n; ++i) {
          auto& entry = store[kvs.keys[i]];
          std::copy(entry.begin(), entry.end(), res.vals.data() + off);
          off += entry.size();
          lens[i] = static_cast<int>(entry.size());
        }
        res.lens = lens;
      }
    }
    server->Response(req, res);
  }
  std::unordered_map<Key, std::vector<V>> store;
};

template <typename V>
struct KVServerReduceHandle {
  explicit KVServerReduceHandle(int num_workers) : num_workers_(std::max(1, num_workers)) {}

  void operator()(const KVMeta& req, const KVPairs<V>& kvs, KVServer<V>* server) {
    XPS_CHECK(!(req.push && req.pull))
        << "ZPushPull is not supported in reduce mode (pulls are held per round)";
    if (req.push) {
      HandlePush(req, kvs, server);
    } else if (req.pull) {
      HandlePull(req, kvs, server);
    } else {
      server->Response(req);
    }
  }

  struct Group {
    std::vector<Key> keys;
    std::vector<size_t> lens;
    std::vector<V> buf;
    int pushes = 0;
    int pulls = 0;
    std::vector<KVMeta> waiting_pulls;
    std::vector<KVMeta> waiting_next_pulls;
    std::vector<std::pair<KVMeta, KVPairs<V>>> waiting_pushes;
    std::set<int> pulled;
  };
  std::unordered_map<uint64_t, Group> store;
  int num_workers_;

  Group& GroupFor(const SArray<Key>& keys) {
    uint64_t h = 1469598103934665603ull;
    const unsigned char* p = reinterpret_cast<const unsigned char*>(keys.data());
    for (size_t i = 0; i < keys.nbytes(); ++i) {
      h ^= p[i];
      h *= 1099511628211ull;
    }
    Group& g = store[h];
    if (g.keys.empty()) {
      g.keys.assign(keys.begin(), keys.end());
    } else {
      XPS_CHECK(g.keys.size() == keys.size() &&
                std::equal(g.keys.begin(), g.keys.end(), keys.begin()))
          << "reduce mode needs a consistent key->message grouping across workers";
    }
    return g;
  }

 private:
  void HandlePush(const KVMeta& req, const KVPairs<V>& kvs, KVServer<V>* server) {
    XPS_CHECK(!kvs.vals.on_device()) << "KVServerReduceHandle is CPU-only";
    size_t n = kvs.keys.size();
    Group& g = GroupFor(kvs.keys);
    if (g.pushes >= num_workers_) {
      g.waiting_pushes.emplace_back(req, kvs);
      return;
    }
    if (g.lens.size() != n) {
      g.lens.resize(n);
      for (size_t i = 0; i < n; ++i) {
        g.lens[i] = kvs.lens.empty() ? kvs.vals.size() / n : static_cast<size_t>(kvs.lens[i]);
      }
    }
    size_t total = 0;
    for (size_t l : g.lens) total += l;
    if (g.buf.size() < total) g.buf.resize(total, V(0));
    const V* __restrict__ v = kvs.vals.data();
    V* __restrict__ b = g.buf.data();
    if (g.pushes == 0) {
      HostPar::CopyBytes(b, v, total * sizeof(V));
    } else {
      SumInto(b, v, total);
    }
    g.pushes++;
    server->Response(req);
    if (g.pushes >= num_workers_) {
      std::vector<KVMeta> waiting;
      waiting.swap(g.waiting_pulls);
      for (auto& w : waiting) RespondPull(w, g, server);
    }
  }

  void HandlePull(const KVMeta& req, const KVPairs<V>& kvs, KVServer<V>* server) {
    Group& g = GroupFor(kvs.keys);
    if (g.pulled.count(req.sender)) {
      g.waiting_next_pulls.push_back(req);
      return;
    }
    if (g.pushes < num_workers_) {
      g.waiting_pulls.push_back(req);
      return;
    }
    RespondPull(req, g, server);
  }

  void RespondPull(const KVMeta& req, Group& g, KVServer<V>* server) {
    KVPairs<V> res;
    res.keys = SArray<Key>(g.keys);
    res.vals = SArray<V>(g.buf.data(), g.buf.size(), kCPU);
    SArray<int> lens(g.keys.size());
    for (size_t i = 0; i < g.keys.size(); ++i) lens[i] = static_cast<int>(g.lens[i]);
    res.lens = lens;
    server->Response(req, res);
    g.pulled.insert(req.sender);
    g.pulls++;
    if (g.pulls >= num_workers_) {
      g.pushes = 0;
      g.pulls = 0;
      g.pulled.clear();
      std::vector<std::pair<KVMeta, KVPairs<V>>> dpush;
      dpush.swap(g.waiting_pushes);
      for (auto& d : dpush) HandlePush(d.first, d.second, server);
      std::vector<KVMeta> dpull;
      dpull.swap(g.waiting_next_pulls);
      for (auto& d : dpull) {
        if (g.pushes >= num_workers_) {
          RespondPull(d, g, server);
        } else {
          g.waiting_pulls.push_back(d);
        }
      }
    }
  }
};

}
```

csrc/message.h:

```cpp
#pragma once

#include <array>
#include <sstream>
#include <string>
#include <vector>

#include "sarray.h"

namespace xps {

static const int kIpcHandleBytes = 64;

struct Node {
  enum Role : int { SCHEDULER = 0, SERVER = 1, WORKER = 2, JOINT = 3 };
  static const char* RoleStr(int r) {
    static const char* s[] = {"scheduler", "server", "worker", "joint"};
    return (r >= 0 && r < 4) ? s[r] : "?";
  }
  int role = -1;
  int id = kEmptyNodeID;
  std::string hostname;
  int port = -1;
  int aux_id = -1;
  int dev_id = kCPU;
  uint64_t host_hash = 0;
  int is_recovery = 0;
  uint64_t pool_capacity = 0;
  uint64_t pool_slab_bytes = 0;
  std::vector<std::array<char, kIpcHandleBytes>> pool_handles;
  uint64_t shm_uid = 0;
  uint64_t host_pool_uid = 0;
  uint64_t host_pool_capacity = 0;

  std::string DebugString() const {
    std::ostringstream os;
    os << "role=" << RoleStr(role) << " id=" << id << " addr=" << hostname << ":" << port
       << " dev=" << dev_id << " aux=" << aux_id << (is_recovery ? " recovery" : "");
    return os.str();
  }
};

struct Control {
  enum Command : int { EMPTY = 0, ADD_NODE, BARRIER, HEARTBEAT, TERMINATE, ACK, HANDSHAKE };
  int cmd = EMPTY;
  std::vector<Node> node;
  int barrier_group = 0;
  int barrier_token = 0;
  int instance_barrier = 0;
  uint64_t msg_sig = 0;
  bool empty() const { return cmd == EMPTY; }
  std::string DebugString() const {
    std::ostringstream os;
    static const char* names[] = {"EMPTY",     "ADD_NODE", "BARRIER",  "HEARTBEAT",
                                  "TERMINATE", "ACK",      "HANDSHAKE"};
    os << "cmd=" << names[cmd];
    if (cmd == BARRIER) os << " group=" << barrier_group << " tok=" << barrier_token;
    for (auto& n : node) os << " {" << n.DebugString() << "}";
    return os.str();
  }
};

static const int kOptInPlace = 1;
static const int kOptValsByRef = 2;
static const int kOptPullAddr = 4;
static const int kOptHostAddr = 8;
static const int kOptPullLane = 16;
static const int kOptEntryAddr = 32;
static const int kOptEntryPush = 64;

enum DataType : int { kChar = 0, kInt32, kInt64, kUint64, kFloat32, kFloat64, kUint8 };
inline size_t DataTypeSize(int t) {
  switch (t) {
    case kChar: case kUint8: return 1;
    case kInt32: case kFloat32: return 4;
    default: return 8;
  }
}

struct Meta {
  static const int kEmpty = -1;
  int app_id = kEmpty;
  int customer_id = kEmpty;
  int timestamp = kEmpty;
  int sender = kEmptyNodeID;
  int recver = kEmptyNodeID;
  bool request = false;
  bool push = false;
  bool pull = false;
  bool simple_app = false;
  int head = kEmpty;
  std::string body;
  Key key = 0;
  uint64_t addr = 0;
  uint64_t entry_addr = 0;
  int64_t val_len = 0;
  int option = 0;
  uint64_t msg_sig = 0;
  uint64_t seq = 0;
  std::vector<int> data_type;
  int src_dev = kCPU;
  int dst_dev = kCPU;
  Control control;

  std::string DebugString() const {
    std::ostringstream os;
    os << "meta[app=" << app_id << " cust=" << customer_id << " ts=" << timestamp
       << " " << sender << "->" << recver
       << (request ? " req" : " res") << (push ? " push" : "") << (pull ? " pull" : "")
       << " key=" << key << " val_len=" << val_len;
    if (!control.empty()) os << " ctrl{" << control.DebugString() << "}";
    os << "]";
    return os.str();
  }
};

struct Message {
  Meta meta;
  std::vector<SArray<char>> data;

  template <typename V>
  void AddData(const SArray<V>& v) {
    XPS_CHECK_LT(data.size(), 4u);
    meta.data_type.push_back(DataTypeOf<V>());
    data.push_back(SArray<char>::View(v));
  }

  template <typename V>
  static int DataTypeOf();

  std::string DebugString() const {
    std::ostringstream os;
    os << meta.DebugString();
    if (!data.empty()) {
      os << " data:[";
      for (auto& d : data) os << d.size() << (d.on_device() ? "d" : "h") << ",";
      os << "]";
    }
    return os.str();
  }
};

template <> inline int Message::DataTypeOf<char>() { return kChar; }
template <> inline int Message::DataTypeOf<uint8_t>() { return kUint8; }
template <> inline int Message::DataTypeOf<int>() { return kInt32; }
template <> inline int Message::DataTypeOf<int64_t>() { return kInt64; }
template <> inline int Message::DataTypeOf<uint64_t>() { return kUint64; }
template <> inline int Message::DataTypeOf<float>() { return kFloat32; }
template <> inline int Message::DataTypeOf<double>() { return kFloat64; }

}
```

csrc/postoffice.cc:

```cpp
#include "postoffice.h"

#include <chrono>

#include "van.h"

namespace xps {

Postoffice::Postoffice(int role, int instance_idx) : role_(role), instance_idx_(instance_idx) {}

Postoffice::~Postoffice() = default;

void Postoffice::EnsureVan() {
  if (!van_) van_.reset(new Van(this));
}

void Postoffice::Start(int customer_id, bool do_barrier) {
  if (started_) return;
  auto* env = Environment::Get();
  num_workers_ = env->GetInt("DMLC_NUM_WORKER", 0);
  num_servers_ = env->GetInt("DMLC_NUM_SERVER", 0);
  node_id_ = kEmptyNodeID;
  {
    std::lock_guard<std::mutex> lk(mu_);
    server_key_ranges_.clear();
  }
  EnsureVan();
  started_ = true;
  van_->Start(customer_id);
  if (van_->my_node().is_recovery) do_barrier = false;
  if (do_barrier) {
    Barrier(customer_id, kScheduler | kServerGroup | kWorkerGroup);
  }
  if (do_barrier && !is_scheduler()) {
    for (int id : GetNodeIDs(kServerGroup | kWorkerGroup)) {
      if (id == node_id_ && van_->plane()) van_->plane()->ImportPeers();
      Barrier(customer_id, kServerGroup | kWorkerGroup);
    }
  }
}

void Postoffice::Finalize(int customer_id, bool do_barrier) {
  if (!started_) return;
  if (do_barrier) {
    Barrier(customer_id, kScheduler | kServerGroup | kWorkerGroup);
  }
  van_->Stop();
  van_.reset();
  started_ = false;
  if (exit_cb_) exit_cb_();
}

int Postoffice::my_rank() const { return IDtoRank(node_id_); }

std::vector<int> Postoffice::GetNodeIDs(int group) const {
  std::vector<int> ids;
  if (group & kScheduler) ids.push_back(kScheduler);
  if (group & kServerGroup) {
    for (int r = 0; r < num_servers_; ++r) ids.push_back(ServerRankToID(r));
  }
  if (group & kWorkerGroup) {
    for (int r = 0; r < num_workers_; ++r) ids.push_back(WorkerRankToID(r));
  }
  return ids;
}

const std::vector<Range>& Postoffice::GetServerKeyRanges() {
  std::lock_guard<std::mutex> lk(mu_);
  if (server_key_ranges_.empty()) {
    int n = std::max(num_servers_, 1);
    uint64_t step = kMaxKey / n;
    for (int i = 0; i < n; ++i) {
      Range r;
      r.begin = step * i;
      r.end = (i == n - 1) ? kMaxKey : step * (i + 1);
      server_key_ranges_.push_back(r);
    }
  }
  return server_key_ranges_;
}

void Postoffice::AddCustomer(Customer* c) {
  std::lock_guard<std::mutex> lk(mu_);
  int key = (c->app_id() << 16) | (c->customer_id() & 0xFFFF);
  XPS_CHECK_EQ(customers_.count(key), 0u)
      << "duplicate customer app=" << c->app_id() << " id=" << c->customer_id();
  customers_[key] = c;
  customer_cv_.notify_all();
}

void Postoffice::RemoveCustomer(Customer* c) {
  std::lock_guard<std::mutex> lk(mu_);
  customers_.erase((c->app_id() << 16) | (c->customer_id() & 0xFFFF));
}

Customer* Postoffice::GetCustomer(int app_id, int customer_id, int timeout_sec) const {
  int key = (app_id << 16) | (customer_id & 0xFFFF);
  std::unique_lock<std::mutex> lk(mu_);
  bool ok = customer_cv_.wait_for(lk, std::chrono::seconds(timeout_sec),
                                  [&] { return customers_.count(key) > 0; });
  return ok ? customers_.at(key) : nullptr;
}

void Postoffice::Barrier(int customer_id, int group) {
  XPS_CHECK(van_->IsReady());
  int token;
  {
    std::lock_guard<std::mutex> lk(barrier_mu_);
    barrier_done_ = false;
    token = ++barrier_seq_;
    barrier_token_ = token;
    barrier_group_ = group;
  }
  Message req;
  req.meta.control.cmd = Control::BARRIER;
  req.meta.control.barrier_group = group;
  req.meta.request = true;
  req.meta.recver = kScheduler;
  req.meta.app_id = 0;
  req.meta.customer_id = customer_id;
  req.meta.timestamp = token;
  van_->Send(req);
  std::unique_lock<std::mutex> lk(barrier_mu_);
  barrier_cv_.wait(lk, [this] { return barrier_done_; });
}

void Postoffice::Manage(const Message& msg) {
  if (msg.meta.control.cmd == Control::BARRIER && !msg.meta.request) {
    std::lock_guard<std::mutex> lk(barrier_mu_);
    if (msg.meta.control.barrier_group != barrier_group_ ||
        msg.meta.timestamp != barrier_token_) {
      XPS_VLOG(2) << "ignoring stale barrier response (group "
                  << msg.meta.control.barrier_group << " token " << msg.meta.timestamp << ")";
      return;
    }
    barrier_done_ = true;
    barrier_cv_.notify_all();
  }
}

void Postoffice::UpdateHeartbeat(int node_id, time_t t) {
  std::lock_guard<std::mutex> lk(heartbeat_mu_);
  heartbeats_[node_id] = t;
}

std::vector<int> Postoffice::GetDeadNodes(int timeout_sec) {
  std::vector<int> dead;
  if (!van_->IsReady() || timeout_sec == 0) return dead;
  time_t now = time(nullptr);
  std::lock_guard<std::mutex> lk(heartbeat_mu_);
  for (int id : GetNodeIDs(kWorkerGroup | kServerGroup)) {
    auto it = heartbeats_.find(id);
    if ((it == heartbeats_.end() || it->second + timeout_sec < now) &&
        start_time_ + timeout_sec < now) {
      dead.push_back(id);
    }
  }
  return dead;
}

namespace {
std::mutex reg_mu;
std::unique_ptr<Postoffice> reg_scheduler;
std::vector<std::unique_ptr<Postoffice>> reg_servers;
std::vector<std::unique_ptr<Postoffice>> reg_workers;
}

Postoffice* Postoffice::GetScheduler() {
  std::lock_guard<std::mutex> lk(reg_mu);
  if (!reg_scheduler) reg_scheduler.reset(new Postoffice(Node::SCHEDULER));
  return reg_scheduler.get();
}

Postoffice* Postoffice::GetServer(int idx) {
  std::lock_guard<std::mutex> lk(reg_mu);
  while (static_cast<int>(reg_servers.size()) <= idx) {
    reg_servers.emplace_back(new Postoffice(Node::SERVER, reg_servers.size()));
  }
  return reg_servers[idx].get();
}

Postoffice* Postoffice::GetWorker(int idx) {
  std::lock_guard<std::mutex> lk(reg_mu);
  while (static_cast<int>(reg_workers.size()) <= idx) {
    reg_workers.emplace_back(new Postoffice(Node::WORKER, reg_workers.size()));
  }
  return reg_workers[idx].get();
}

Postoffice* Postoffice::FindByNodeId(int id) {
  std::lock_guard<std::mutex> lk(reg_mu);
  auto match = [id](Postoffice* po) {
    return po && po->started_ && po->node_id_ == id && po->van_ && po->van_->IsReady();
  };
  if (match(reg_scheduler.get())) return reg_scheduler.get();
  for (auto& p : reg_servers) {
    if (match(p.get())) return p.get();
  }
  for (auto& p : reg_workers) {
    if (match(p.get())) return p.get();
  }
  return nullptr;
}

void Postoffice::ClearRegistry() {
  std::lock_guard<std::mutex> lk(reg_mu);
  if (reg_scheduler) reg_scheduler.release();
  for (auto& p : reg_servers) p.release();
  for (auto& p : reg_workers) p.release();
  reg_servers.clear();
  reg_workers.clear();
}

}
```

csrc/postoffice.h:

```cpp
#pragma once

#include <atomic>
#include <condition_variable>
#include <memory>
#include <mutex>
#include <unordered_map>
#include <vector>

#include "customer.h"
#include "message.h"

namespace xps {

class Van;

struct Range {
  uint64_t begin = 0;
  uint64_t end = 0;
  uint64_t size() const { return end - begin; }
};

class Postoffice {
 public:
  Postoffice(int role, int instance_idx = 0);
  ~Postoffice();

  void EnsureVan();
  void Start(int customer_id, bool do_barrier);
  void Finalize(int customer_id, bool do_barrier);

  Van* van() const { return van_.get(); }
  int role() const { return role_; }
  bool is_worker() const { return role_ == Node::WORKER; }
  bool is_server() const { return role_ == Node::SERVER; }
  bool is_scheduler() const { return role_ == Node::SCHEDULER; }
  int num_workers() const { return num_workers_; }
  int num_servers() const { return num_servers_; }
  int instance_idx() const { return instance_idx_; }

  int my_rank() const;
  int node_id() const { return node_id_; }
  void set_node_id(int id) { node_id_ = id; }
  int preferred_rank() const { return preferred_rank_; }
  void set_preferred_rank(int r) { preferred_rank_ = r; }

  std::vector<int> GetNodeIDs(int group) const;
  const std::vector<Range>& GetServerKeyRanges();

  void AddCustomer(Customer* c);
  void RemoveCustomer(Customer* c);
  Customer* GetCustomer(int app_id, int customer_id, int timeout_sec = 15) const;

  void Barrier(int customer_id, int group);
  void Manage(const Message& msg);

  void UpdateHeartbeat(int node_id, time_t t);
  std::vector<int> GetDeadNodes(int timeout_sec = 60);

  void RegisterExitCallback(std::function<void()> cb) { exit_cb_ = std::move(cb); }

  static Postoffice* GetScheduler();
  static Postoffice* GetServer(int idx = 0);
  static Postoffice* GetWorker(int idx = 0);
  static Postoffice* FindByNodeId(int id);
  static void ClearRegistry();

 private:
  friend class Van;

  int role_;
  int instance_idx_;
  std::atomic<int> node_id_{kEmptyNodeID};
  int preferred_rank_ = -1;
  int num_workers_ = 0;
  int num_servers_ = 0;
  std::unique_ptr<Van> van_;
  bool started_ = false;

  mutable std::mutex mu_;
  std::unordered_map<int, Customer*> customers_;
  mutable std::condition_variable customer_cv_;

  std::mutex barrier_mu_;
  std::condition_variable barrier_cv_;
  bool barrier_done_ = false;
  int barrier_seq_ = 0;
  int barrier_token_ = 0;
  int barrier_group_ = 0;

  std::mutex heartbeat_mu_;
  std::unordered_map<int, time_t> heartbeats_;
  time_t start_time_ = time(nullptr);

  std::vector<Range> server_key_ranges_;
  std::function<void()> exit_cb_;
};

}
```

csrc/pybind.cc:

```cpp
#include <pybind11/functional.h>
#include <pybind11/numpy.h>
#include <pybind11/pybind11.h>
#include <pybind11/stl.h>

#include <atomic>
#include <thread>

#include "gpu_plane.h"
#include "hip_pool.h"
#include "hip_util.h"
#include "host_pool.h"
#include "kernels.h"
#include "kv_app.h"
#include "kv_utils.h"
#include "ps.h"
#include "server_handlers.h"
#include "shm_ring.h"
#include "simple_app.h"
#include "tile_runs.h"
#include "van.h"
#include "wire.h"

namespace py = pybind11;
using namespace xps;
// ... 238 lines not shown
      fclose(f);
    } else {
      XPS_LOG(Fatal) << "no checkpointable handler installed";
    }
  }

  void LoadCheckpoint(const std::string& path) {
    py::gil_scoped_release rel;
    if (dense_) {
      dense_->Load(path);
    } else if (sparse_) {
      sparse_->Load(path);
    } else if (default_ || reduce_) {
      FILE* f = fopen(path.c_str(), "rb");
      XPS_CHECK(f) << "cannot open checkpoint " << path;
      uint64_t n = 0;
      XPS_CHECK_EQ(fread(&n, 8, 1, f), 1u);
      for (uint64_t i = 0; i < n; ++i) {
        uint64_t key, len;
        XPS_CHECK_EQ(fread(&key, 8, 1, f), 1u);
        XPS_CHECK_EQ(fread(&len, 8, 1, f), 1u);
        auto& v = default_ ? default_->store[key]
                           : reduce_->store[key].buf;
        v.resize(len / sizeof(float));
        XPS_CHECK_EQ(fread(v.data(), 1, len, f), len);
      }
      fclose(f);
    } else {
      XPS_LOG(Fatal) << "no checkpointable handler installed";
    }
  }

  void SetGpuDenseHandle(const std::string& mode, const std::string& dtype) {
    DenseMode m = mode == "sum" ? DenseMode::kSum
                  : mode == "reduce" ? DenseMode::kReduce
                                     : DenseMode::kAssign;
    DenseDtype d = dtype == "bf16" ? DenseDtype::kBf16 : DenseDtype::kF32;
    auto h = std::make_shared<GpuDenseHandler>(s_.postoffice(), m, d);
    dense_ = h;
    s_.set_request_handle([h](const KVMeta& m2, const KVPairs<float>& kvs, KVServer<float>* srv) {
      (*h)(m2, kvs, srv);
    });
  }

  void SetGpuSparseHandle(size_t rows, size_t row_len, bool accumulate, int key_shift) {
    auto h = std::make_shared<GpuSparseHandler>(s_.postoffice(), rows, row_len, accumulate,
                                                key_shift);
    sparse_ = h;
    s_.set_request_handle([h](const KVMeta& m, const KVPairs<float>& kvs, KVServer<float>* srv) {
      (*h)(m, kvs, srv);
    });
  }

  uintptr_t SparseTablePtr() const { return sparse_ ? sparse_->table_ptr() : 0; }

  void SetPythonHandle(py::function fn) {
    s_.set_request_handle([fn](const KVMeta& m, const KVPairs<float>& kvs, KVServer<float>* srv) {
      KVPairs<float> res;
      {
        py::gil_scoped_acquire gil;
        py::dict meta;
        meta["cmd"] = m.cmd;
        meta["push"] = m.push;
        meta["pull"] = m.pull;
        meta["sender"] = m.sender;
        meta["timestamp"] = m.timestamp;
        meta["key"] = m.key;
        meta["val_len"] = m.val_len;
        py::array_t<uint64_t> keys(kvs.keys.size());
        std::copy(kvs.keys.begin(), kvs.keys.end(), keys.mutable_data());
        py::array_t<float> vals(kvs.vals.size());
        if (kvs.vals.size()) {
          XPS_CHECK(!kvs.vals.on_device()) << "python handle got device vals";
          std::copy(kvs.vals.begin(), kvs.vals.end(), vals.mutable_data());
        }
        py::object out = fn(meta, keys, vals);
        if (m.pull) {
          XPS_CHECK(!out.is_none()) << "pull handler must return vals";
          auto arr = py::cast<py::array_t<float>>(out);
          res.keys = kvs.keys;
          res.vals.CopyFrom(arr.data(), arr.size());
          size_t n = kvs.keys.size();
          SArray<int> lens(n);
          for (size_t i = 0; i < n; ++i) lens[i] = static_cast<int>(arr.size() / n);
          res.lens = lens;
        }
      }
      srv->Response(m, res);
    });
  }

 private:
  KVServer<float> s_;
  std::shared_ptr<GpuSparseHandler> sparse_;
  std::shared_ptr<GpuDenseHandler> dense_;
  std::shared_ptr<KVServerDefaultHandle<float>> default_;
  std::shared_ptr<KVServerReduceHandle<float>> reduce_;
};

class PySimpleApp {
 public:
  PySimpleApp(const std::string& role, int app_id, int customer_id)
      : app_(app_id, role == "worker" ? customer_id : app_id, GetPO(role)) {}

  void SetRequestHandle(py::function fn) {
    app_.set_request_handle([fn](const SimpleData& d, SimpleApp* app) {
      std::string reply;
      {
        py::gil_scoped_acquire gil;
        py::object out = fn(d.head, py::bytes(d.body));
        if (!out.is_none()) reply = py::cast<std::string>(out);
      }
      app->Response(d, reply);
    });
  }

  void SetResponseHandle(py::function fn) {
    app_.set_response_handle([fn](const SimpleData& d, SimpleApp*) {
      py::gil_scoped_acquire gil;
      fn(d.head, py::bytes(d.body));
    });
  }

  int Request(int head, const std::string& body, int recver) {
    py::gil_scoped_release rel;
    return app_.Request(head, body, recver);
  }

  void Wait(int ts) {
    py::gil_scoped_release rel;
    app_.Wait(ts);
  }

 private:
  SimpleApp app_;
};

}

PYBIND11_MODULE(_core, m) {
  m.doc() = "xps: MI355X-native parameter-server core";

  m.def("init_env", [](const std::map<std::string, std::string>& kv) {
    Environment::Get()->Init(kv);
  });
  m.def("env", [](const std::string& k) { return Environment::Get()->GetStr(k, ""); });
  m.def("start",
        [](int customer_id, const std::string& role, int rank, bool barrier, int device) {
          py::gil_scoped_release rel;
          Start(customer_id, role, rank, barrier, device);
        },
        py::arg("customer_id") = 0, py::arg("role") = "worker", py::arg("rank") = -1,
        py::arg("barrier") = true, py::arg("device") = -2);
  m.def("finalize",
        [](int customer_id, const std::string& role, bool barrier) {
          py::gil_scoped_release rel;
          Finalize(customer_id, role, barrier);
        },
        py::arg("customer_id") = 0, py::arg("role") = "worker", py::arg("barrier") = true);
  m.def("clear_registry", []() { Postoffice::ClearRegistry(); });
  m.def("barrier", [](const std::string& role, int group, int idx) {
    py::gil_scoped_release rel;
    GetPO(role, idx)->Barrier(0, group);
  }, py::arg("role"), py::arg("group"), py::arg("idx") = 0);
  m.def("num_workers", &NumWorkers);
  m.def("num_servers", &NumServers);
  m.def("my_rank", [](const std::string& role, int idx) { return GetPO(role, idx)->my_rank(); },
        py::arg("role"), py::arg("idx") = 0);
  m.def("node_id", [](const std::string& role, int idx) { return GetPO(role, idx)->node_id(); },
        py::arg("role"), py::arg("idx") = 0);
  m.def("send_bytes", [](const std::string& role) {
    auto* van = GetPO(role)->van();
    return van ? van->send_bytes_.load() : int64_t(0);
  });
  m.def("recv_bytes", [](const std::string& role) {
    auto* van = GetPO(role)->van();
    return van ? van->recv_bytes_.load() : int64_t(0);
  });
  m.def("gpu_count", []() { return gpu::DeviceCount(); });
  m.def("device_sync", [](int dev) {
    py::gil_scoped_release rel;
    gpu::DeviceSync(dev);
  }, py::arg("dev") = -1);

  m.attr("SCHEDULER_GROUP") = kScheduler;
  m.attr("SERVER_GROUP") = kServerGroup;
  m.attr("WORKER_GROUP") = kWorkerGroup;

  m.def("pool_init", [](int device, size_t capacity) { HbmPool::Get()->Init(device, capacity); },
        py::arg("device"), py::arg("capacity") = 0);
  m.def("pool_ipc_handle", [](size_t slab) {
    return py::bytes(HbmPool::Get()->slab_handle(slab), kIpcHandleBytes);
  }, py::arg("slab") = 0);
  m.def("make_stream_events", []() {
    py::gil_scoped_release rel;
    hipStream_t s;
    XPS_CHECK(hipStreamCreateWithFlags(&s, hipStreamNonBlocking) == hipSuccess);
    hipEvent_t ev;
    XPS_CHECK(hipEventCreateWithFlags(&ev, hipEventDisableTiming) == hipSuccess);
    XPS_CHECK(hipEventRecord(ev, s) == hipSuccess);
    while (hipEventQuery(ev) != hipSuccess) {}
    return reinterpret_cast<uintptr_t>(s);
  });
  m.def("kernel_on_stream", [](uintptr_t stream, uintptr_t dst, uintptr_t src, size_t n) {
    py::gil_scoped_release rel;
    kern::DenseSumF32(reinterpret_cast<float*>(dst), reinterpret_cast<float*>(src), n,
                      reinterpret_cast<hipStream_t>(stream));
    hipEvent_t ev;
    XPS_CHECK(hipEventCreateWithFlags(&ev, hipEventDisableTiming) == hipSuccess);
    XPS_CHECK(hipEventRecord(ev, reinterpret_cast<hipStream_t>(stream)) == hipSuccess);
    while (hipEventQuery(ev) != hipSuccess) {}
    (void)hipEventDestroy(ev);
  });
  m.def("ipc_open", [](py::bytes handle) {
    std::string h = handle;
    py::gil_scoped_release rel;
    hipIpcMemHandle_t hh;
    memcpy(&hh, h.data(), sizeof(hh));
    void* ptr = nullptr;
    hipError_t e = hipIpcOpenMemHandle(&ptr, hh, hipIpcMemLazyEnablePeerAccess);
    XPS_CHECK(e == hipSuccess) << "hipIpcOpenMemHandle: " << hipGetErrorString(e);
    return reinterpret_cast<uintptr_t>(ptr);
  });
  m.def("pool_in_use", []() { return HbmPool::Get()->bytes_in_use(); });
  m.def("pool_contains", [](uintptr_t p) {
    uint64_t off = 0;
    return HbmPool::Get()->OffsetOf(reinterpret_cast<const void*>(p), &off);
  });
  py::class_<PoolBuffer>(m, "PoolBuffer")
      .def_property_readonly("ptr", &PoolBuffer::ptr)
      .def_property_readonly("nbytes", &PoolBuffer::nbytes)
      .def_property_readonly("device", &PoolBuffer::device)
      .def("copy_from", &PoolBuffer::copy_from)
      .def("to_numpy_f32", &PoolBuffer::to_numpy_f32);
  m.def("pool_alloc", [](size_t nbytes) {
    PoolBuffer b;
    b.arr = HbmPool::Get()->AllocArray(nbytes);
    return b;
  });
  m.def("host_alloc", [](size_t nbytes) {
    PoolBuffer b;
    b.arr = HostShmPool::Get()->AllocArray(nbytes);
    return b;
  });

  py::class_<PyKVWorker>(m, "KVWorker")
      .def(py::init<int, int, int>(), py::arg("app_id") = 0, py::arg("customer_id") = 0,
           py::arg("instance_idx") = 0)
      .def("push", &PyKVWorker::Push, py::arg("keys"), py::arg("vals"),
           py::arg("lens") = py::array_t<int>())
      .def("pull", &PyKVWorker::PullBlocking, py::arg("keys"))
      .def("zpush_ptr", &PyKVWorker::ZPushPtr, py::arg("keys"), py::arg("vals_ptr"),
           py::arg("vals_bytes"), py::arg("device"), py::arg("lens") = py::array_t<int>(),
           py::arg("cmd") = 0, py::arg("keys_dev_ptr") = 0)
      .def("zpushpull_ptr", &PyKVWorker::ZPushPullPtr, py::arg("keys"), py::arg("vals_ptr"),
           py::arg("out_ptr"), py::arg("nbytes"), py::arg("device") = -1,
           py::arg("lens") = py::array_t<int>(), py::arg("cmd") = 0,
           py::arg("keys_dev_ptr") = 0)
      .def("zpull_ptr", &PyKVWorker::ZPullPtr, py::arg("keys"), py::arg("vals_ptr"),
           py::arg("vals_bytes"), py::arg("device"), py::arg("lens") = py::array_t<int>(),
           py::arg("cmd") = 0, py::arg("keys_dev_ptr") = 0)
      .def("wait", &PyKVWorker::Wait)
      .def("round", &PyKVWorker::Round, py::arg("keys"), py::arg("ptrs"), py::arg("nbytes"),
           py::arg("device"), py::arg("cmd") = 0, py::arg("pull") = false)
      .def("round_mixed", &PyKVWorker::RoundMixed, py::arg("keys"), py::arg("push_ptrs"),
           py::arg("pull_ptrs"), py::arg("sizes"), py::arg("device"), py::arg("cmd") = 0,
           py::arg("overlap") = true);

  py::class_<PyKVServer>(m, "KVServer")
      .def(py::init<int, int>(), py::arg("app_id") = 0, py::arg("instance_idx") = 0)
      .def("set_default_handle", &PyKVServer::SetDefaultHandle)
      .def("set_reduce_handle", &PyKVServer::SetReduceHandle, py::arg("num_workers"))
      .def("set_gpu_dense_handle", &PyKVServer::SetGpuDenseHandle, py::arg("mode") = "assign",
           py::arg("dtype") = "f32")
      .def("set_gpu_sparse_handle", &PyKVServer::SetGpuSparseHandle, py::arg("rows"),
           py::arg("row_len"), py::arg("accumulate") = true, py::arg("key_shift") = 0)
      .def("register_entry", &PyKVServer::RegisterEntry, py::arg("key"), py::arg("ptr"),
           py::arg("nbytes"), py::arg("device") = 0)
      .def("sparse_table_ptr", &PyKVServer::SparseTablePtr)
      .def("save_checkpoint", &PyKVServer::SaveCheckpoint)
      .def("load_checkpoint", &PyKVServer::LoadCheckpoint)
      .def("set_python_handle", &PyKVServer::SetPythonHandle);

  m.def("zero_copy_recv_count", []() { return g_zero_copy_recv.load(); });
  m.def("fused_assign_count", []() { return g_fused_assign.load(); });
  m.def("fused_assign_launches", []() { return g_fused_launches.load(); });
  m.def("coalesce_admit",
        [](const std::vector<std::tuple<uintptr_t, uintptr_t, uintptr_t, size_t>>& open,
           const std::tuple<uintptr_t, uintptr_t, uintptr_t, size_t>& seg) {
          auto conv = [](const std::tuple<uintptr_t, uintptr_t, uintptr_t, size_t>& t) {
            return kern::Seg2{reinterpret_cast<void*>(std::get<0>(t)),
                              reinterpret_cast<void*>(std::get<1>(t)),
                              reinterpret_cast<const void*>(std::get<2>(t)), std::get<3>(t)};
          };
          std::vector<kern::Seg2> segs;
          for (auto& t : open) segs.push_back(conv(t));
          switch (kern::CoalesceAdmit(segs.data(), static_cast<int>(segs.size()), conv(seg))) {
            case kern::Admit::kAdmit: return "admit";
            case kern::Admit::kFlushFirst: return "flush";
            default: return "reject";
          }
        },
        py::arg("open"), py::arg("seg"));
  m.def("tile_runs",
        [](const std::vector<unsigned long long>& chunk_counts,
           unsigned long long chunks_per_block, unsigned long long block_index) {
          if (chunks_per_block == 0) throw std::invalid_argument("tile_runs: empty tile");
          std::vector<unsigned long long> prefix(chunk_counts.size() + 1, 0);
          for (size_t i = 0; i < chunk_counts.size(); ++i) {
            if (chunk_counts[i] == 0) throw std::invalid_argument("tile_runs: empty segment");
            prefix[i + 1] = prefix[i] + chunk_counts[i];
          }
          int n = static_cast<int>(chunk_counts.size());
          std::vector<std::tuple<int, unsigned long long, unsigned long long>> out;
          kern::TileRunIter it = kern::TileRunsBegin(prefix.data(), n, chunks_per_block,
                                                     block_index);
          kern::TileRun run;
          while (kern::TileRunsNext(prefix.data(), &it, &run)) {
            out.emplace_back(run.seg, run.lo, run.hi);
          }
          return out;
        },
        py::arg("chunk_counts"), py::arg("chunks_per_block"), py::arg("block_index"));

  m.def("plane_peer_bytes", [](const std::string& role, int idx) {
    py::dict out;
    auto* po = GetPO(role, idx);
    auto* plane = po->van() ? dynamic_cast<GpuPlane*>(po->van()->plane()) : nullptr;
    if (plane) {
      for (auto& t : plane->PeerBytes()) {
        out[py::int_(std::get<0>(t))] = py::make_tuple(std::get<1>(t), std::get<2>(t));
      }
    }
    return out;
  }, py::arg("role") = "worker", py::arg("idx") = 0);

  m.def("_order_nodes", [](std::vector<std::tuple<std::string, std::string, int>> in) {
    std::vector<Node> nodes;
    for (auto& t : in) {
      Node n;
      n.role = std::get<0>(t) == "worker" ? Node::WORKER : Node::SERVER;
      n.hostname = std::get<1>(t);
      n.port = std::get<2>(t);
      nodes.push_back(n);
    }
    auto less = NodeRankOrder(nodes);
    std::sort(nodes.begin(), nodes.end(), less);
    std::vector<std::tuple<std::string, std::string, int>> out;
    for (auto& n : nodes) {
      out.emplace_back(n.role == Node::WORKER ? "worker" : "server", n.hostname, n.port);
    }
    return out;
  });

  m.def("_host_pool_init_for_test", [](uint64_t uid, size_t bytes) {
    HostShmPool::Get()->Init(uid, bytes);
  });
  m.def("_gc_stale_shm", []() { HostShmPool::GcStaleSegments(); });

  m.def("_ring_stress", [](int producers, int per, int payload) {
    ShmRing ring;
    XPS_CHECK(ring.Create(0xabcdef12345ull + getpid()));
    std::atomic<long> received{0}, sum{0}, pushed{0};
    std::atomic<bool> done{false};
    std::thread consumer([&]() {
      std::vector<char> buf(ShmRing::MaxPayload());
      while (true) {
        uint32_t n = ring.Pop(buf.data());
        if (n == 0) {
          if (done.load() && received.load() >= pushed.load()) break;
          std::this_thread::yield();
          continue;
        }
        long v = 0;
        for (uint32_t i = 0; i < n; ++i) v += static_cast<unsigned char>(buf[i]);
        sum.fetch_add(v);
        received.fetch_add(1);
      }
    });
    std::vector<std::thread> ps;
    std::atomic<long> expect{0};
    for (int p = 0; p < producers; ++p) {
      ps.emplace_back([&, p]() {
        std::vector<char> msg(payload);
        for (int i = 0; i < per; ++i) {
          for (int b = 0; b < payload; ++b) msg[b] = static_cast<char>((p + i + b) & 0x7f);
          long v = 0;
          for (int b = 0; b < payload; ++b) v += static_cast<unsigned char>(msg[b]);
          if (ring.Push(msg.data(), payload)) {
            expect.fetch_add(v);
            pushed.fetch_add(1);
          }
        }
      });
    }
    for (auto& t : ps) t.join();
    done.store(true);
    consumer.join();
    ring.CloseAndUnlink();
    return py::make_tuple(static_cast<long>(received.load()),
                          static_cast<long>(pushed.load()),
                          sum.load() == expect.load());
  });

  m.def("_test_meta_roundtrip", []() {
    Meta m;
    m.app_id = 7;
    m.customer_id = 3;
    m.timestamp = 42;
    m.sender = 9;
    m.recver = 8;
    m.request = true;
    m.push = true;
    m.head = 2;
    m.body = "hello\x00world";
    m.key = 0xDEADBEEFCAFEull;
    m.addr = 1234567;
    m.val_len = 1 << 20;
    m.option = kOptPullAddr | kOptHostAddr;
    m.seq = 987654321;
    m.data_type = {kUint64, kFloat32, kInt32};
    m.control.cmd = Control::ADD_NODE;
    Node n;
    n.role = Node::WORKER;
    n.id = 11;
    n.hostname = "10.0.0.5";
    n.port = 1234;
    n.shm_uid = 0x1122334455667788ull;
    n.host_pool_uid = 77;
    n.host_pool_capacity = 1 << 30;
    n.pool_capacity = 2ull << 30;
    n.pool_slab_bytes = 1ull << 30;
    n.pool_handles.resize(2);
    n.pool_handles[0][0] = 'x';
    n.pool_handles[1][63] = 'y';
    m.control.node.push_back(n);
    std::string buf;
    PackMeta(m, &buf);
    Meta out;
    UnpackMeta(buf.data(), buf.size(), &out);
    bool ok = out.app_id == m.app_id && out.customer_id == m.customer_id &&
              out.timestamp == m.timestamp && out.sender == m.sender &&
              out.recver == m.recver && out.request == m.request && out.push == m.push &&
              out.head == m.head && out.body == m.body && out.key == m.key &&
              out.addr == m.addr && out.val_len == m.val_len && out.option == m.option &&
              out.seq == m.seq &&
              out.data_type == m.data_type && out.control.cmd == m.control.cmd &&
              out.control.node.size() == 1;
    auto& on = out.control.node[0];
    ok = ok && on.role == n.role && on.id == n.id && on.hostname == n.hostname &&
         on.port == n.port && on.shm_uid == n.shm_uid && on.host_pool_uid == n.host_pool_uid &&
         on.host_pool_capacity == n.host_pool_capacity && on.pool_capacity == n.pool_capacity &&
         on.pool_slab_bytes == n.pool_slab_bytes && on.pool_handles.size() == 2 &&
         on.pool_handles[0][0] == 'x' && on.pool_handles[1][63] == 'y';
    return ok;
  });

  m.def("_pack_meta_sample", []() {
    Meta m;
    m.app_id = 1;
    m.body = "abc";
    m.control.cmd = Control::ADD_NODE;
    Node n;
    n.hostname = "127.0.0.1";
    n.pool_handles.resize(1);
    m.control.node.push_back(n);
    std::string buf;
    PackMeta(m, &buf);
    return py::bytes(buf);
  });
  m.def("_meta_roundtrip_fields",
        [](int app_id, int customer_id, int timestamp, int sender, int recver, bool request,
           bool push, bool pull, bool simple_app, int head, const std::string& body, uint64_t key,
           uint64_t addr, int64_t val_len, int option, uint64_t msg_sig, uint64_t seq,
           const std::string& hostname, int port, uint64_t shm_uid, int nhandles) {
          Meta m;
          m.app_id = app_id;
          m.customer_id = customer_id;
          m.timestamp = timestamp;
          m.sender = sender;
          m.recver = recver;
          m.request = request;
          m.push = push;
          m.pull = pull;
          m.simple_app = simple_app;
          m.head = head;
          m.body = body;
          m.key = key;
          m.addr = addr;
          m.val_len = val_len;
          m.option = option;
          m.msg_sig = msg_sig;
          m.seq = seq;
          m.control.cmd = Control::ADD_NODE;
          Node n;
          n.hostname = hostname;
          n.port = port;
          n.shm_uid = shm_uid;
          n.pool_handles.resize(nhandles);
          m.control.node.push_back(n);
          std::string buf;
          PackMeta(m, &buf);
          Meta o;
          UnpackMeta(buf.data(), buf.size(), &o);
          auto& on = o.control.node.at(0);
          return o.app_id == m.app_id && o.customer_id == m.customer_id &&
                 o.timestamp == m.timestamp && o.sender == m.sender && o.recver == m.recver &&
                 o.request == m.request && o.push == m.push && o.pull == m.pull &&
                 o.simple_app == m.simple_app && o.head == m.head && o.body == m.body &&
                 o.key == m.key && o.addr == m.addr && o.val_len == m.val_len &&
                 o.option == m.option && o.msg_sig == m.msg_sig && o.seq == m.seq &&
                 on.hostname == n.hostname && on.port == n.port && on.shm_uid == n.shm_uid &&
                 on.pool_handles.size() == static_cast<size_t>(nhandles);
        });

  m.def("_unpack_meta_raw", [](py::bytes b) {
    std::string s = b;
    Meta out;
    UnpackMeta(s.data(), s.size(), &out);
    return true;
  });

  m.def("parallel_ordered_match",
        [](py::array_t<uint64_t> src_keys, py::array_t<float> src_vals,
           py::array_t<uint64_t> dst_keys, size_t k, bool accumulate, int nthreads) {
          SArray<Key> sk;
          sk.CopyFrom(src_keys.data(), src_keys.size());
          SArray<float> sv;
          sv.CopyFrom(src_vals.data(), src_vals.size());
          SArray<Key> dk;
          dk.CopyFrom(dst_keys.data(), dst_keys.size());
          SArray<float> dv;
          size_t n = ParallelOrderedMatch(sk, sv, dk, &dv, k,
                                          accumulate ? AssignOp::kPlus : AssignOp::kAssign,
                                          nthreads);
          py::array_t<float> out(dv.size());
          std::copy(dv.begin(), dv.end(), out.mutable_data());
          return py::make_tuple(n, out);
        },
        py::arg("src_keys"), py::arg("src_vals"), py::arg("dst_keys"), py::arg("k") = 1,
        py::arg("accumulate") = false, py::arg("nthreads") = 4);
  m.def("parallel_sort", [](py::array_t<uint64_t> keys, int nthreads) {
    SArray<Key> k;
    k.CopyFrom(keys.data(), keys.size());
    ParallelSort(&k, nthreads);
    py::array_t<uint64_t> out(k.size());
    std::copy(k.begin(), k.end(), out.mutable_data());
    return out;
  }, py::arg("keys"), py::arg("nthreads") = 4);

  m.def("k_dense_assign", [](uintptr_t dst, uintptr_t src, size_t nbytes) {
    kern::DenseAssign(reinterpret_cast<void*>(dst), reinterpret_cast<void*>(src), nbytes, nullptr);
    gpu::DeviceSync(-1);
  });
  m.def("k_dense_assign2",
        [](uintptr_t dst0, uintptr_t dst1, uintptr_t src, size_t nbytes, int grid_cap) {
          kern::DenseAssign2(reinterpret_cast<void*>(dst0), reinterpret_cast<void*>(dst1),
                             reinterpret_cast<void*>(src), nbytes, nullptr, grid_cap);
          gpu::DeviceSync(-1);
        },
        py::arg("dst0"), py::arg("dst1"), py::arg("src"), py::arg("nbytes"),
        py::arg("grid_cap") = 0);
  m.def("k_batched_assign2",
        [](const std::vector<std::tuple<uintptr_t, uintptr_t, uintptr_t, size_t>>& segs,
           int tile_cap) {
          std::vector<kern::Seg2> v;
          for (auto& t : segs) {
            v.push_back(kern::Seg2{reinterpret_cast<void*>(std::get<0>(t)),
                                   reinterpret_cast<void*>(std::get<1>(t)),
                                   reinterpret_cast<const void*>(std::get<2>(t)),
                                   std::get<3>(t)});
            if (kern::CoalesceAdmit(nullptr, 0, v.back()) != kern::Admit::kAdmit) {
              throw std::invalid_argument("k_batched_assign2: segment " +
                                          std::to_string(v.size() - 1) +
                                          " is misaligned, not a 16 B multiple or "
                                          "self-overlapping");
            }
          }
          kern::BatchedAssign2(v.data(), static_cast<int>(v.size()), nullptr, tile_cap);
          gpu::DeviceSync(-1);
        },
        py::arg("segs"), py::arg("tile_cap") = 0);
  m.def("k_dense_sum_f32", [](uintptr_t dst, uintptr_t src, size_t n) {
    kern::DenseSumF32(reinterpret_cast<float*>(dst), reinterpret_cast<float*>(src), n, nullptr);
    gpu::DeviceSync(-1);
  });
  m.def("k_dense_sum_bf16", [](uintptr_t dst, uintptr_t src, size_t n) {
    kern::DenseSumBf16(reinterpret_cast<uint16_t*>(dst), reinterpret_cast<uint16_t*>(src), n,
                       nullptr);
    gpu::DeviceSync(-1);
  });
  m.def("k_sparse_gather_f32",
        [](uintptr_t table, uintptr_t rows, size_t nrows, size_t row_len, uintptr_t out) {
          kern::SparseGatherF32(reinterpret_cast<float*>(table),
                                reinterpret_cast<uint64_t*>(rows), nrows, row_len,
                                reinterpret_cast<float*>(out), nullptr);
          gpu::DeviceSync(-1);
        });
  m.def("k_sparse_scatter_add_f32",
        [](uintptr_t table, uintptr_t rows, size_t nrows, size_t row_len, uintptr_t src,
           bool atomic) {
          kern::SparseScatterAddF32(reinterpret_cast<float*>(table),
                                    reinterpret_cast<uint64_t*>(rows), nrows, row_len,
                                    reinterpret_cast<float*>(src), atomic, nullptr);
          gpu::DeviceSync(-1);
        });
// ... 10 lines not shown
```

csrc/server_handlers.cc:

```cpp
#include "server_handlers.h"

#include "gpu_plane.h"
#include "hip_pool.h"
#include "kernels.h"

namespace xps {

#define XPS_HIP_CHECK(cmd)                                                            \
  do {                                                                                \
    hipError_t e_ = (cmd);                                                            \
    XPS_CHECK(e_ == hipSuccess) << "HIP error: " << hipGetErrorString(e_) << " in " #cmd; \
  } while (0)

static GpuPlane* ThePlane(Postoffice* po) {
  return dynamic_cast<GpuPlane*>(po->van() ? po->van()->plane() : nullptr);
}

static hipStream_t PeerStream(Postoffice* po, int sender, hipStream_t* fallback) {
  auto* plane = ThePlane(po);
  if (plane) return plane->StreamForPeer(sender);
  if (!*fallback) {
    XPS_HIP_CHECK(hipStreamCreateWithFlags(fallback, hipStreamNonBlocking));
  }
  return *fallback;
}

static hipStream_t PeerPullStream(Postoffice* po, int sender, hipStream_t* fallback) {
  auto* plane = ThePlane(po);
  if (plane) return plane->PullStreamForPeer(sender);
  if (!*fallback) {
    XPS_HIP_CHECK(hipStreamCreateWithFlags(fallback, hipStreamNonBlocking));
  }
  return *fallback;
}

static hipEvent_t EventAlloc(Postoffice* po) {
  if (auto* plane = ThePlane(po)) return plane->GetEvent();
  hipEvent_t ev;
  XPS_HIP_CHECK(hipEventCreateWithFlags(&ev, hipEventDisableTiming));
  return ev;
}

static void EventFree(Postoffice* po, hipEvent_t ev) {
  if (auto* plane = ThePlane(po)) {
    plane->PutEvent(ev);
  } else {
    (void)hipEventDestroy(ev);
  }
}


static EventRef MakeEventRef(Postoffice* po, hipStream_t s) {
  hipEvent_t ev = EventAlloc(po);
  XPS_HIP_CHECK(hipEventRecord(ev, s));
  return EventRef(ev, [po](hipEvent_t e) { EventFree(po, e); });
}

GpuDenseHandler::GpuDenseHandler(Postoffice* po, DenseMode mode, DenseDtype dtype)
    : po_(po), mode_(mode), dtype_(dtype) {
  XPS_CHECK(HbmPool::Get()->initialized()) << "GpuDenseHandler needs the HBM pool";
  num_workers_ = std::max(1, po_->num_workers());
  chain_ = num_workers_ > 1;
}

void GpuDenseHandler::SumKernel(void* dst, const void* src, size_t nbytes, hipStream_t s) {
  if (dtype_ == DenseDtype::kBf16) {
    kern::DenseSumBf16(static_cast<uint16_t*>(dst), static_cast<const uint16_t*>(src),
                       nbytes / 2, s);
  } else {
    kern::DenseSumF32(static_cast<float*>(dst), static_cast<const float*>(src), nbytes / 4, s);
  }
}

void GpuDenseHandler::BatchedSum(const kern::CopyDesc* descs, int n, hipStream_t s) {
  if (dtype_ == DenseDtype::kBf16) {
    kern::BatchedSumBf16(descs, n, s);
  } else {
    kern::BatchedSumF32(descs, n, s);
  }
}

bool GpuDenseHandler::NeedChain(int sender) {
  if (chain_) return true;
  auto* plane = ThePlane(po_);
  return plane && plane->LanesSplit(sender);
}

GpuDenseHandler::~GpuDenseHandler() = default;

void GpuDenseHandler::OrderAfter(Entry* e, hipStream_t s) {
  if (e->last_ev) XPS_HIP_CHECK(hipStreamWaitEvent(s, e->last_ev.get(), 0));
}

hipStream_t GpuDenseHandler::Stream(int sender) {
  return PeerStream(po_, sender, &fallback_stream_);
}

hipStream_t GpuDenseHandler::PullStream(int sender) {
  return PeerPullStream(po_, sender, &fallback_stream_);
}

void GpuDenseHandler::operator()(const KVMeta& req, const KVPairs<float>& kvs,
                                 KVServer<float>* server) {
  if (req.push && req.pull) {
    XPS_CHECK(mode_ != DenseMode::kReduce)
        << "ZPushPull is not supported in reduce mode (pulls are held per round)";
    if (req.option & kOptInPlace) {
      server->Response(req);
      return;
    }
    if (TryFusedAssign(req, kvs, server)) return;
    HandlePush(req, kvs, server, false);
    HandlePull(req, kvs, server);
    return;
  }
  if (req.push) {
    HandlePush(req, kvs, server);
  } else if (req.pull) {
    HandlePull(req, kvs, server);
  } else {
    server->Response(req);
  }
}

bool GpuDenseHandler::TryFusedAssign(const KVMeta& req, const KVPairs<float>& kvs,
                                     KVServer<float>* server) {
  if (!FusedAssignEnabled()) return false;
  if (mode_ != DenseMode::kAssign || req.cmd == kCmdSum) return false;
  if (kvs.keys.size() != 1 || !kvs.vals.on_device()) return false;
  if (!(req.option & kOptPullAddr) || (req.option & kOptHostAddr)) return false;
  size_t len = kvs.lens.empty() ? kvs.vals.nbytes()
                                : static_cast<size_t>(kvs.lens[0]) * sizeof(float);
  if (len == 0 || len != kvs.vals.nbytes() || static_cast<int64_t>(len) != req.val_len) {
    return false;
  }
  auto* plane = ThePlane(po_);
  if (!plane) return false;
  char* dst = plane->PeerDst(req.sender, req.addr, len);
  if (!dst) return false;
  XPS_STAGE(dense_fused_assign);
  XPS_HIP_CHECK(hipSetDevice(HbmPool::Get()->device()));
  Entry* e;
  {
    std::lock_guard<std::mutex> lk(mu_);
    e = &store_[kvs.keys[0]];
    if (e->buf.size() < len) {
      if (!e->buf.empty()) e->retired.push_back(e->buf);
      e->buf = HbmPool::Get()->AllocArray(len);
      XPS_HIP_CHECK(hipMemset(e->buf.data(), 0, len));
    }
  }
  if (e->buf.size() != len) return false;
  const char* src = reinterpret_cast<const char*>(kvs.vals.data());
  if (!kern::Disjoint3(e->buf.data(), dst, src, len)) return false;
  bool chain = NeedChain(req.sender);
  bool coalesced = !chain && !e->last_ev &&
                   plane->CoalesceAppend(req.sender, kern::Seg2{e->buf.data(), dst, src, len});
  if (!coalesced) {
    hipStream_t stream = Stream(req.sender);
    OrderAfter(e, stream);
    kern::DenseAssign2(e->buf.data(), dst, src, len, stream);
    g_fused_launches.fetch_add(1, std::memory_order_relaxed);
    if (chain) e->last_ev = MakeEventRef(po_, stream);
  }
  g_fused_assign.fetch_add(1, std::memory_order_relaxed);
  g_zero_copy_recv.fetch_add(1, std::memory_order_relaxed);
  KVMeta r = req;
  r.option |= kOptInPlace;
  r.option &= ~(kOptPullLane | kOptEntryPush);
  r.val_len = static_cast<int64_t>(len);
  uint64_t eoff = 0;
  if (HbmPool::Get()->OffsetOf(e->buf.data(), &eoff)) {
    r.entry_addr = eoff;
    r.option |= kOptEntryAddr;
  }
  server->Response(r);
  if (coalesced) plane->CoalesceEnd(req.sender);
  return true;
}

GpuDenseHandler::Group* GpuDenseHandler::GroupFor(const SArray<Key>& keys) {
  uint64_t h = 1469598103934665603ull;
  const unsigned char* p = reinterpret_cast<const unsigned char*>(keys.data());
  for (size_t i = 0; i < keys.nbytes(); ++i) {
    h ^= p[i];
    h *= 1099511628211ull;
  }
  Group* g;
  {
    std::lock_guard<std::mutex> lk(mu_);
    g = &groups_[h];
  }
  if (g->keys.empty()) {
    g->keys.assign(keys.begin(), keys.end());
    g->ents.reserve(keys.size());
    std::lock_guard<std::mutex> lk(mu_);
    for (Key k : g->keys) g->ents.push_back(&store_[k]);
  } else {
    XPS_CHECK(g->keys.size() == keys.size() &&
              std::equal(g->keys.begin(), g->keys.end(), keys.begin()))
        << "reduce mode needs a consistent key->message grouping across workers "
           "(key-set hash collision or inconsistent bucketing)";
  }
  return g;
}

void GpuDenseHandler::HandleReducePush(const KVMeta& req, const KVPairs<float>& kvs,
                                       KVServer<float>* server) {
  XPS_STAGE(reduce_push);
  size_t n = kvs.keys.size();
  Group* g = GroupFor(kvs.keys);
  if (g->pushes >= num_workers_) {
    g->waiting_pushes.emplace_back(req, kvs);
    return;
  }
  XPS_CHECK(kvs.vals.on_device()) << "reduce mode needs device vals (pool buffers)";
  if (g->lens.size() != n) {
    g->lens.resize(n);
    for (size_t i = 0; i < n; ++i) {
      g->lens[i] = kvs.lens.empty() ? kvs.vals.nbytes() / n
                                    : static_cast<size_t>(kvs.lens[i]) * sizeof(float);
    }
  }
  hipStream_t stream = Stream(req.sender);
  XPS_HIP_CHECK(hipSetDevice(HbmPool::Get()->device()));
  if (g->last_ev) XPS_HIP_CHECK(hipStreamWaitEvent(stream, g->last_ev.get(), 0));
  bool first = g->pushes == 0;
  if (first) {
    for (auto& ev : g->pull_guard) {
      XPS_HIP_CHECK(hipStreamWaitEvent(stream, ev.get(), 0));
    }
    g->pull_guard.clear();
  }
  std::vector<kern::CopyDesc> descs;
  descs.reserve(n);
  size_t off = 0;
  bool aligned = true;
  for (size_t i = 0; i < n; ++i) {
    size_t len = g->lens[i];
    Entry* e = g->ents[i];
    if (e->buf.size() < len) e->buf = HbmPool::Get()->AllocArray(len);
    descs.push_back({e->buf.data(), reinterpret_cast<const char*>(kvs.vals.data()) + off, len});
    aligned = aligned && (len % 16 == 0);
    off += len;
  }
  if (aligned) {
    if (first) {
      kern::BatchedAssign(descs.data(), static_cast<int>(n), stream);
    } else {
      BatchedSum(descs.data(), static_cast<int>(n), stream);
    }
  } else {
    for (auto& d : descs) {
      if (first) {
        kern::DenseAssign(d.dst, d.src, d.nbytes, stream);
      } else {
        SumKernel(d.dst, d.src, d.nbytes, stream);
      }
    }
  }
  g->pushes++;
  EventRef ev = MakeEventRef(po_, stream);
  g->round_events.push_back(ev);
  g->last_ev = ev;
  server->Response(req);
  if (g->pushes >= num_workers_) {
    std::vector<KVMeta> waiting;
    waiting.swap(g->waiting_pulls);
    for (auto& w : waiting) RespondPull(w, g, server);
  }
}

void GpuDenseHandler::HandlePush(const KVMeta& req, const KVPairs<float>& kvs,
                                 KVServer<float>* server, bool respond) {
  XPS_STAGE(dense_push);
  size_t n = kvs.keys.size();
  XPS_CHECK_GT(n, 0u);
  if (mode_ == DenseMode::kReduce) {
    HandleReducePush(req, kvs, server);
    return;
  }
  if (req.option & kOptInPlace) {
    if (respond) server->Response(req);
    return;
  }
  hipStream_t stream = Stream(req.sender);
  XPS_HIP_CHECK(hipSetDevice(HbmPool::Get()->device()));
  bool chain = NeedChain(req.sender);
  bool sum_all = mode_ == DenseMode::kAssign ? req.cmd == kCmdSum : req.cmd != kCmdAssign;
  if (kvs.vals.on_device() && n > 1) {
    std::vector<kern::CopyDesc> descs;
    std::vector<Entry*> ents;
    descs.reserve(n);
    ents.reserve(n);
    size_t boff = 0;
    bool aligned = true;
    for (size_t i = 0; i < n; ++i) {
      size_t len = kvs.lens.empty() ? kvs.vals.nbytes() / n
                                    : static_cast<size_t>(kvs.lens[i]) * sizeof(float);
      Entry* e;
      {
        std::lock_guard<std::mutex> lk(mu_);
        e = &store_[kvs.keys[i]];
        if (e->buf.size() < len) {
          e->buf = HbmPool::Get()->AllocArray(len);
          XPS_HIP_CHECK(hipMemset(e->buf.data(), 0, len));
        }
      }
      ents.push_back(e);
      descs.push_back({e->buf.data(),
                       reinterpret_cast<const char*>(kvs.vals.data()) + boff, len});
      aligned = aligned && (len % 16 == 0) && (boff % 16 == 0);
      boff += len;
    }
    if (aligned) {
      for (Entry* e : ents) OrderAfter(e, stream);
      if (sum_all) {
        BatchedSum(descs.data(), static_cast<int>(n), stream);
      } else {
        kern::BatchedAssign(descs.data(), static_cast<int>(n), stream);
      }
      if (chain) {
        EventRef ev = MakeEventRef(po_, stream);
        for (Entry* e : ents) e->last_ev = ev;
      }
      auto* plane0 = po_->van() ? po_->van()->plane() : nullptr;
      if (!plane0) XPS_HIP_CHECK(hipStreamSynchronize(stream));
      if (respond) server->Response(req);
      return;
    }
  }
  size_t off = 0;
  bool synced = false;
  Entry* last_e = nullptr;
  for (size_t i = 0; i < n; ++i) {
    size_t len = kvs.lens.empty() ? kvs.vals.nbytes() / n
                                  : static_cast<size_t>(kvs.lens[i]) * sizeof(float);
    Entry* e;
    {
      std::lock_guard<std::mutex> lk(mu_);
      e = &store_[kvs.keys[i]];
      if (e->buf.size() < len) {
        if (!e->buf.empty()) e->retired.push_back(e->buf);
        e->buf = HbmPool::Get()->AllocArray(len);
        XPS_HIP_CHECK(hipMemset(e->buf.data(), 0, len));
      }
    }
    last_e = e;
    bool sum = sum_all;
    const char* src = reinterpret_cast<const char*>(kvs.vals.data()) + off;
    if (kvs.vals.on_device()) {
      OrderAfter(e, stream);
      {
        XPS_STAGE(push_kernel_launch);
        if (sum) {
          SumKernel(e->buf.data(), src, len, stream);
        } else {
          kern::DenseAssign(e->buf.data(), src, len, stream);
        }
      }
      if (chain) {
        XPS_STAGE(push_chain_event);
        e->last_ev = MakeEventRef(po_, stream);
      }
    } else {
      if (chain && e->last_ev) {
        XPS_HIP_CHECK(hipEventSynchronize(e->last_ev.get()));
        e->last_ev.reset();
      }
      if (sum) {
        SArray<char> scratch = HbmPool::Get()->AllocArray(len);
        XPS_HIP_CHECK(hipMemcpy(scratch.data(), src, len, hipMemcpyHostToDevice));
        SumKernel(e->buf.data(), scratch.data(), len, stream);
        XPS_HIP_CHECK(hipStreamSynchronize(stream));
        synced = true;
      } else {
        XPS_HIP_CHECK(hipMemcpy(e->buf.data(), src, len, hipMemcpyHostToDevice));
      }
    }
    off += len;
  }
  auto* plane = po_->van() ? po_->van()->plane() : nullptr;
  if (!plane && !synced) XPS_HIP_CHECK(hipStreamSynchronize(stream));
  if (!respond) return;
  if (mode_ == DenseMode::kAssign && n == 1 && last_e && plane) {
    uint64_t eoff = 0;
    if (HbmPool::Get()->OffsetOf(last_e->buf.data(), &eoff)) {
      KVMeta r = req;
      r.addr = eoff;
      r.val_len = static_cast<int64_t>(last_e->buf.size());
      r.option |= kOptEntryAddr;
      server->Response(r);
      return;
    }
  }
  server->Response(req);
}

void GpuDenseHandler::RespondPull(const KVMeta& req, Group* g, KVServer<float>* server) {
  XPS_STAGE(reduce_respond_pull);
  hipStream_t stream = PullStream(req.sender);
  for (auto& ev : g->round_events) {
    XPS_HIP_CHECK(hipStreamWaitEvent(stream, ev.get(), 0));
  }
  size_t n = g->keys.size();
  size_t total = 0;
  for (size_t len : g->lens) total += len;
  SArray<Key> keys(g->keys);
  SArray<int> lens(n);
  for (size_t i = 0; i < n; ++i) lens[i] = static_cast<int>(g->lens[i] / sizeof(float));
  bool responded = false;
  if (req.option & kOptPullAddr) {
    if (auto* plane = ThePlane(po_)) {
      std::vector<kern::CopyDesc> descs;
      descs.reserve(n);
      uint64_t off = 0;
      bool ok = true;
      for (size_t i = 0; i < n && ok; ++i) {
        size_t len = g->lens[i];
        char* dst = plane->PeerDst(req.sender, req.addr + off, len);
        ok = dst != nullptr && len % 16 == 0;
        if (ok) {
          descs.push_back({dst, g->ents[i]->buf.data(), len});
          off += len;
        }
      }
      if (ok) {
        kern::BatchedAssign(descs.data(), static_cast<int>(n), stream);
        KVMeta r2 = req;
        r2.option |= kOptInPlace | kOptPullLane;
        r2.val_len = static_cast<int64_t>(total);
        KVPairs<float> res2;
        res2.keys = keys;
        res2.lens = lens;
        server->Response(r2, res2);
        responded = true;
      }
    }
  }
  if (!responded) {
    KVPairs<float> res;
    res.keys = keys;
    res.lens = lens;
    if (n == 1) {
      res.vals = SArray<float>::View(g->ents[0]->buf);
    } else {
      SArray<char> tmp = HbmPool::Get()->AllocArray(total);
      std::vector<kern::CopyDesc> descs;
      descs.reserve(n);
      size_t off = 0;
      bool aligned = true;
      for (size_t i = 0; i < n; ++i) {
        descs.push_back({tmp.data() + off, g->ents[i]->buf.data(), g->lens[i]});
        aligned = aligned && (g->lens[i] % 16 == 0) && (off % 16 == 0);
        off += g->lens[i];
      }
      if (aligned) {
        kern::BatchedAssign(descs.data(), static_cast<int>(n), stream);
      } else {
        for (auto& d : descs) kern::DenseAssign(d.dst, d.src, d.nbytes, stream);
      }
// ... 322 lines not shown
```

csrc/van.cc:

```cpp
#include <tuple>

#include "van.h"

#include <unistd.h>

#include <algorithm>
#include <chrono>
#include <random>
#include <set>

#include "hip_util.h"
#include "postoffice.h"
#include "resender.h"
#include "wire.h"

namespace xps {

Van::Van(Postoffice* po) : po_(po) {}

Van::~Van() { Stop(); }

void Van::Start(int customer_id) {
  auto* env = Environment::Get();
  scheduler_.role = Node::SCHEDULER;
  scheduler_.id = kScheduler;
  scheduler_.hostname = env->GetStr("DMLC_PS_ROOT_URI", "127.0.0.1");
  scheduler_.port = env->GetInt("DMLC_PS_ROOT_PORT", 9000);

  my_node_.role = po_->role();
  my_node_.hostname = LocalIP();
  my_node_.host_hash = HostHash();
  my_node_.aux_id = po_->preferred_rank() >= 0 ? po_->preferred_rank()
                                               : env->GetInt("DMLC_RANK", -1);
  std::random_device rd;
  my_uid_ = (static_cast<uint64_t>(rd()) << 32) ^ rd() ^ (static_cast<uint64_t>(getpid()) << 16);
  my_node_.shm_uid = my_uid_;
  if (plane_) plane_->FillSelf(&my_node_);

  drop_rate_ = env->GetInt("PS_DROP_MSG", 0);
  heartbeat_interval_ = env->GetInt("PS_HEARTBEAT_INTERVAL", 0);
  if (env->GetInt("PS_RESEND", 0)) {
    resender_.reset(new Resender(env->GetInt("PS_RESEND_TIMEOUT", 1000), 10, this));
  }
  if (env->GetInt("ENABLE_PROFILING", 0)) {
    std::string path = env->GetStr("PROFILE_PATH", "");
    if (path.empty()) {
      path = std::string("xps_profile_van_") +
             (po_->is_worker() ? "worker" : po_->is_server() ? "server" : "sched") + "_" +
             std::to_string(getpid());
    } else {
      path += "_" + std::to_string(getpid());
    }
    trace_file_ = fopen(path.c_str(), "w");
  }

  int want_port = 0;
  if (po_->is_scheduler()) {
    want_port = scheduler_.port;
    my_node_ = scheduler_;
    my_node_.host_hash = HostHash();
    my_node_.shm_uid = my_uid_;
    if (plane_) plane_->FillSelf(&my_node_);
  } else if (env->GetInt("DMLC_PORT", 0) && po_->instance_idx() == 0) {
    want_port = env->GetInt("DMLC_PORT", 0);
  }
  int bound = listener_.Bind(want_port, po_->is_scheduler() ? 1 : 40);
  XPS_CHECK_GE(bound, 0) << "failed to bind port " << want_port << " role "
                         << Node::RoleStr(my_node_.role);
  my_node_.port = bound;
  listener_.StartAccepting([this](int fd) { OnNewConnection(fd); });

  XPS_VLOG(1) << "van up: " << my_node_.DebugString();

  if (po_->is_scheduler()) {
    po_->set_node_id(kScheduler);
    {
      std::lock_guard<std::mutex> lk(nodes_mu_);
      nodes_[kScheduler] = my_node_;
    }
    if (po_->num_workers() + po_->num_servers() == 0) ready_ = true;
  } else {
    int fd = TcpConnect(scheduler_.hostname, scheduler_.port);
    XPS_CHECK_GE(fd, 0) << "cannot reach scheduler at " << scheduler_.hostname << ":"
                        << scheduler_.port;
    auto conn = std::make_shared<TcpConn>(fd);
    {
      std::lock_guard<std::mutex> lk(conn_mu_);
      conns_[kScheduler] = conn;
      recv_threads_.emplace_back([this, conn] { RecvLoop(conn); });
    }
    {
      std::lock_guard<std::mutex> lk(nodes_mu_);
      nodes_[kScheduler] = scheduler_;
    }
    Message req;
    req.meta.control.cmd = Control::ADD_NODE;
    req.meta.request = true;
    req.meta.sender = kEmptyNodeID;
    req.meta.recver = kScheduler;
    req.meta.control.node.push_back(my_node_);
    std::string meta;
    PackMeta(req.meta, &meta);
    conn->SendFrame(meta, {});
  }

  auto deadline = std::chrono::steady_clock::now() + std::chrono::seconds(
      Environment::Get()->GetInt("XPS_BOOTSTRAP_TIMEOUT", 300));
  while (!ready_.load()) {
    XPS_CHECK(std::chrono::steady_clock::now() < deadline)
        << "bootstrap timeout: " << my_node_.DebugString();
    usleep(2000);
  }

  if (heartbeat_interval_ > 0 && !po_->is_scheduler()) {
    heartbeat_thread_ = std::thread([this] { HeartbeatLoop(); });
  }
}

void Van::Stop() {
  if (stopping_.exchange(true)) return;
  if (plane_) plane_->Stop();
  listener_.Stop();
  std::vector<std::thread> threads;
  {
    std::lock_guard<std::mutex> lk(conn_mu_);
    for (auto& kv : conns_) kv.second->Close();
    threads.swap(recv_threads_);
  }
  for (auto& t : threads) {
    if (t.joinable()) t.join();
  }
  if (heartbeat_thread_.joinable()) heartbeat_thread_.join();
  resender_.reset();
  if (trace_file_) {
    fclose(trace_file_);
    trace_file_ = nullptr;
  }
}

Node Van::GetNode(int id) {
  std::lock_guard<std::mutex> lk(nodes_mu_);
  auto it = nodes_.find(id);
  XPS_CHECK(it != nodes_.end()) << "unknown node id " << id;
  return it->second;
}

int64_t Van::Send(Message& msg) {
  if (msg.meta.sender == kEmptyNodeID) msg.meta.sender = my_node_.id;
  int recver = msg.meta.recver;
  XPS_CHECK_NE(recver, kEmptyNodeID) << "message has no recver";
  if (recver >= 8 || recver == kScheduler) return SendToNode(msg, recver);
  int64_t total = 0;
  for (int id : po_->GetNodeIDs(recver)) {
    Message copy = msg;
    copy.meta.recver = id;
    int64_t n = SendToNode(copy, id);
    if (n >= 0) total += n;
  }
  return total;
}

int64_t Van::SendToNode(Message& msg, int id) {
  MaybeTrace(msg, false);
  if (id != my_node_.id && msg.meta.control.empty() && msg.meta.seq == 0) {
    std::lock_guard<std::mutex> lk(order_mu_);
    msg.meta.seq = ++send_seq_[id];
  }
  if (id == my_node_.id) {
    Message copy = msg;
    int64_t approx = static_cast<int64_t>(msg.meta.val_len);
    send_bytes_ += approx;
    Deliver(std::move(copy));
    return approx;
  }
  if (plane_ && msg.meta.control.empty()) {
    Node peer;
    {
      std::lock_guard<std::mutex> lk(nodes_mu_);
      auto it = nodes_.find(id);
      if (it != nodes_.end()) peer = it->second;
    }
    if (peer.id != kEmptyNodeID && plane_->CanSend(msg, peer)) {
      int64_t n = plane_->Send(msg, peer);
      if (n >= 0) {
        send_bytes_ += n;
        return n;
      }
    }
  }
  return SendOverTcp(msg, id);
}

int64_t Van::SendOverTcp(Message& msg, int id) {
  if (resender_ && msg.meta.control.empty()) resender_->AddOutgoing(msg);
  auto conn = GetOrDial(id);
  if (!conn) {
    XPS_LOG(Warning) << "no route to node " << id << " from " << my_node_.id;
    return -1;
  }
  std::string meta;
  PackMeta(msg.meta, &meta);
  std::vector<SArray<char>> host_data;
  host_data.reserve(msg.data.size());
  for (auto& d : msg.data) {
    host_data.push_back(d.on_device() ? gpu::StageToHost(d) : d);
  }
  int64_t n = conn->SendFrame(meta, host_data);
  if (n > 0) send_bytes_ += n;
  return n;
}

std::shared_ptr<TcpConn> Van::GetOrDial(int id) {
  {
    std::lock_guard<std::mutex> lk(conn_mu_);
    auto it = conns_.find(id);
    if (it != conns_.end()) return it->second;
  }
  Node n;
  {
    std::lock_guard<std::mutex> lk(nodes_mu_);
    auto it = nodes_.find(id);
    if (it == nodes_.end()) return nullptr;
    n = it->second;
  }
  int fd = TcpConnect(n.hostname, n.port, 20);
  if (fd < 0) return nullptr;
  auto conn = std::make_shared<TcpConn>(fd);
  {
    std::lock_guard<std::mutex> lk(conn_mu_);
    if (stopping_.load()) {
      conn->Close();
      return nullptr;
    }
    auto it = conns_.find(id);
    if (it != conns_.end()) {
      conn->Close();
      return it->second;
    }
    conns_[id] = conn;
    recv_threads_.emplace_back([this, conn] { RecvLoop(conn); });
  }
  Message hs;
  hs.meta.control.cmd = Control::HANDSHAKE;
  hs.meta.sender = my_node_.id;
  hs.meta.recver = id;
  std::string meta;
  PackMeta(hs.meta, &meta);
  conn->SendFrame(meta, {});
  return conn;
}

void Van::OnNewConnection(int fd) {
  auto conn = std::make_shared<TcpConn>(fd);
  std::lock_guard<std::mutex> lk(conn_mu_);
  if (stopping_.load()) {
    conn->Close();
    return;
  }
  recv_threads_.emplace_back([this, conn] { RecvLoop(conn); });
}

void Van::RecvLoop(std::shared_ptr<TcpConn> conn) {
  while (true) {
    std::string meta;
    std::vector<SArray<char>> data;
    int64_t n = conn->RecvFrame(&meta, &data);
    if (n < 0) {
      if (!stopping_.load()) XPS_VLOG(2) << "connection closed on " << my_node_.id;
      std::lock_guard<std::mutex> lk(conn_mu_);
      for (auto it = conns_.begin(); it != conns_.end();) {
        if (it->second == conn) {
          it = conns_.erase(it);
        } else {
          ++it;
        }
      }
      return;
    }
    recv_bytes_ += n;
    Message msg;
    UnpackMeta(meta.data(), meta.size(), &msg.meta);
    msg.data = std::move(data);
    if (msg.meta.sender != kEmptyNodeID) {
      std::lock_guard<std::mutex> lk(conn_mu_);
      auto it = conns_.find(msg.meta.sender);
      if (it == conns_.end() || it->second->closed()) conns_[msg.meta.sender] = conn;
    }
    if (!msg.meta.control.empty()) {
      ProcessControl(msg, conn);
    } else {
      MaybeTrace(msg, true);
      if (drop_rate_ > 0 && msg.meta.request) {
        std::lock_guard<std::mutex> lk(sched_mu_);
        if (static_cast<int>(drop_rng_() % 100) < drop_rate_) {
          XPS_VLOG(2) << "drop-test: dropping " << msg.DebugString();
          continue;
        }
      }
      if (resender_ && resender_->AddIncoming(msg)) continue;
      DeliverData(msg);
    }
  }
}

void Van::Deliver(Message msg) {
  if (!msg.meta.control.empty()) {
    ProcessControl(msg, nullptr);
  } else {
    DeliverData(msg);
  }
}

void Van::InlineData(Message& msg) {
  int app_id = msg.meta.app_id;
  int customer_id = po_->is_worker() ? msg.meta.customer_id : app_id;
  Customer* c = po_->GetCustomer(app_id, customer_id, 15);
  XPS_CHECK(c) << "no customer (app=" << app_id << ", customer=" << customer_id
               << ") on node " << my_node_.id << " for " << msg.DebugString();
  c->ProcessInline(msg);
}

void Van::GatedDeliver(Message& msg) {
  uint64_t seq = msg.meta.seq;
  Flow* f;
  {
    std::lock_guard<std::mutex> lk(order_mu_);
    auto& slot = recv_flows_[msg.meta.sender];
    if (!slot) slot.reset(new Flow());
    f = slot.get();
  }
  std::unique_lock<std::mutex> lk(f->mu);
  if (seq < f->expected) {
    InlineData(msg);
    return;
  }
  if (f->held.empty()) f->hold_since = std::chrono::steady_clock::now();
  f->held.emplace(seq, std::move(msg));
  while (!f->held.empty() && f->held.begin()->first == f->expected) {
    Message m = std::move(f->held.begin()->second);
    f->held.erase(f->held.begin());
    f->expected++;
    InlineData(m);
    f->hold_since = std::chrono::steady_clock::now();
  }
  if (f->held.empty()) return;
  int timeout_ms = Environment::Get()->GetInt("XPS_ORDER_TIMEOUT_MS", 10000);
  if (std::chrono::steady_clock::now() - f->hold_since >
      std::chrono::milliseconds(timeout_ms)) {
    XPS_LOG(Warning) << "sequence gap from node "
                     << f->held.begin()->second.meta.sender << " (expected " << f->expected
                     << ") unfilled for " << timeout_ms << " ms; flushing out of order";
    while (!f->held.empty()) {
      Message m = std::move(f->held.begin()->second);
      uint64_t s2 = f->held.begin()->first;
      f->held.erase(f->held.begin());
      f->expected = s2 + 1;
      InlineData(m);
    }
  }
}

void Van::ResetFlow(int peer_id) {
  Flow* f = nullptr;
  {
    std::lock_guard<std::mutex> lk(order_mu_);
    send_seq_.erase(peer_id);
    auto it = recv_flows_.find(peer_id);
    if (it != recv_flows_.end()) f = it->second.get();
  }
  if (f) {
    std::lock_guard<std::mutex> lk(f->mu);
    f->expected = 1;
    f->held.clear();
  }
}

void Van::DeliverData(Message& msg) {
  if (msg.meta.seq != 0) {
    GatedDeliver(msg);
    return;
  }
  DeliverDataNow(msg);
}

void Van::DeliverDataNow(Message& msg) {
  int app_id = msg.meta.app_id;
  int customer_id = po_->is_worker() ? msg.meta.customer_id : app_id;
  Customer* c = po_->GetCustomer(app_id, customer_id, 15);
  XPS_CHECK(c) << "no customer (app=" << app_id << ", customer=" << customer_id << ") on node "
               << my_node_.id << " for " << msg.DebugString();
  c->Accept(std::move(msg));
}

void Van::DeliverInline(Message& msg) {
  if (!msg.meta.control.empty()) {
    ProcessControl(msg, nullptr);
    return;
  }
  if (msg.meta.seq != 0) {
    GatedDeliver(msg);
    return;
  }
  int app_id = msg.meta.app_id;
  int customer_id = po_->is_worker() ? msg.meta.customer_id : app_id;
  Customer* c = po_->GetCustomer(app_id, customer_id, 15);
  XPS_CHECK(c) << "no customer (app=" << app_id << ", customer=" << customer_id
               << ") on node " << my_node_.id << " for " << msg.DebugString();
  c->ProcessInline(msg);
}

void Van::ProcessControl(Message& msg, const std::shared_ptr<TcpConn>& conn) {
  auto& ctrl = msg.meta.control;
  switch (ctrl.cmd) {
    case Control::HANDSHAKE:
      break;
    case Control::ADD_NODE:
      if (po_->is_scheduler() && msg.meta.request) {
        ProcessAddNodeAtScheduler(msg, conn);
      } else {
        ProcessNodeListAssigned(msg);
      }
      break;
    case Control::BARRIER:
      if (msg.meta.request) {
        ProcessBarrierAtScheduler(msg);
      } else {
        po_->Manage(msg);
      }
      break;
    case Control::HEARTBEAT:
      ProcessHeartbeat(msg);
      break;
    case Control::ACK:
      if (resender_) resender_->HandleAck(ctrl.msg_sig);
      break;
    case Control::TERMINATE:
      stopping_ = true;
      break;
    default:
      XPS_LOG(Warning) << "unknown control " << ctrl.cmd;
  }
}

std::function<bool(const Node&, const Node&)> NodeRankOrder(const std::vector<Node>& batch) {
  auto* env = Environment::Get();
  std::map<std::string, int> host_idx;
  {
    std::string hosts = env->GetStr("BYTEPS_ORDERED_HOSTS", "");
    int idx = 0;
    size_t start = 0;
    while (start <= hosts.size() && !hosts.empty()) {
      size_t comma = hosts.find(',', start);
      std::string h = hosts.substr(start, comma == std::string::npos ? comma : comma - start);
      if (!h.empty()) host_idx[h] = idx++;
      if (comma == std::string::npos) break;
      start = comma + 1;
    }
  }
  bool mixed = env->GetInt("BYTEPS_ENABLE_MIXED_MODE", 0) != 0;
  std::set<std::string> worker_hosts;
  if (mixed) {
    for (auto& n : batch)
      if (n.role == Node::WORKER) worker_hosts.insert(n.hostname);
  }
  auto key = [host_idx, mixed, worker_hosts](const Node& n) {
    auto it = host_idx.find(n.hostname);
    int order = it == host_idx.end() ? (1 << 30) : it->second;
    int coloc = 0;
    if (mixed && n.role == Node::SERVER) coloc = worker_hosts.count(n.hostname) ? 1 : 0;
    return std::make_tuple(order, coloc, n.hostname, n.port);
  };
  return [key](const Node& a, const Node& b) { return key(a) < key(b); };
}

void Van::ProcessAddNodeAtScheduler(Message& msg, const std::shared_ptr<TcpConn>& conn) {
  if (ready_.load()) {
    ProcessRecoveryAtScheduler(msg, conn);
    return;
  }
  std::vector<std::pair<Node, std::shared_ptr<TcpConn>>> batch;
  {
    std::lock_guard<std::mutex> lk(sched_mu_);
    XPS_CHECK_EQ(msg.meta.control.node.size(), 1u);
    pending_nodes_.emplace_back(msg.meta.control.node[0], conn);
    int expected = po_->num_workers() + po_->num_servers();
    XPS_VLOG(1) << "scheduler: " << pending_nodes_.size() << "/" << expected << " nodes joined ("
                << msg.meta.control.node[0].DebugString() << ")";
    if (static_cast<int>(pending_nodes_.size()) < expected) return;
    batch.swap(pending_nodes_);
  }
  {
    std::vector<Node> nodes;
    nodes.reserve(batch.size());
    for (auto& p : batch) nodes.push_back(p.first);
    auto less = NodeRankOrder(nodes);
    std::sort(batch.begin(), batch.end(),
              [&less](const auto& a, const auto& b) { return less(a.first, b.first); });
  }
  std::set<int> taken;
  auto assign = [&](Node& n) {
    int rank = n.aux_id;
    if (rank >= 0) {
      int id = n.role == Node::WORKER ? WorkerRankToID(rank) : ServerRankToID(rank);
      XPS_CHECK(!taken.count(id)) << "duplicate pinned rank " << rank;
      n.id = id;
      taken.insert(id);
      return;
    }
    for (int r = 0;; ++r) {
      int id = n.role == Node::WORKER ? WorkerRankToID(r) : ServerRankToID(r);
      if (!taken.count(id)) {
        n.id = id;
        taken.insert(id);
        return;
      }
    }
  };
  for (auto& p : batch)
    if (p.first.aux_id >= 0) assign(p.first);
  for (auto& p : batch)
    if (p.first.aux_id < 0) assign(p.first);

  Message reply;
  reply.meta.control.cmd = Control::ADD_NODE;
  reply.meta.request = false;
  reply.meta.sender = kScheduler;
  reply.meta.control.node.push_back(my_node_);
  {
    std::lock_guard<std::mutex> lk(nodes_mu_);
    for (auto& p : batch) {
      nodes_[p.first.id] = p.first;
      reply.meta.control.node.push_back(p.first);
    }
  }
  {
    std::lock_guard<std::mutex> lk(conn_mu_);
    for (auto& p : batch) conns_[p.first.id] = p.second;
  }
  if (plane_) {
    for (auto& p : batch) plane_->OnPeer(p.first);
  }
  std::string meta;
  for (auto& p : batch) {
    reply.meta.recver = p.first.id;
    PackMeta(reply.meta, &meta);
    p.second->SendFrame(meta, {});
  }
  XPS_VLOG(1) << "scheduler: assigned ids, cluster up (" << batch.size() << " nodes)";
  ready_ = true;
}

void Van::ProcessRecoveryAtScheduler(Message& msg, const std::shared_ptr<TcpConn>& conn) {
  XPS_CHECK_EQ(msg.meta.control.node.size(), 1u);
  Node node = msg.meta.control.node[0];
  int timeout = Environment::Get()->GetInt("PS_HEARTBEAT_TIMEOUT", 10);
  std::vector<int> dead = po_->GetDeadNodes(timeout);
  int assigned = kEmptyNodeID;
  for (int id : dead) {
    bool want_worker = node.role == Node::WORKER;
    if (IsWorkerID(id) == want_worker) {
      assigned = id;
      break;
    }
  }
  if (assigned == kEmptyNodeID) {
    XPS_LOG(Warning) << "late ADD_NODE but no dead " << Node::RoleStr(node.role)
                     << " to recover (" << node.DebugString() << ")";
    return;
  }
  node.id = assigned;
  node.is_recovery = 1;
  XPS_VLOG(1) << "scheduler: recovering node " << assigned << " as " << node.DebugString();
  {
    std::lock_guard<std::mutex> lk(nodes_mu_);
    nodes_[assigned] = node;
  }
  {
    std::lock_guard<std::mutex> lk(conn_mu_);
    conns_[assigned] = conn;
  }
  po_->UpdateHeartbeat(assigned, time(nullptr));
  if (plane_) plane_->OnPeer(node);
  Message reply;
  reply.meta.control.cmd = Control::ADD_NODE;
  reply.meta.request = false;
  reply.meta.sender = kScheduler;
  reply.meta.recver = assigned;
  {
    std::lock_guard<std::mutex> lk(nodes_mu_);
    for (auto& kv : nodes_) reply.meta.control.node.push_back(kv.second);
  }
  std::string meta;
  PackMeta(reply.meta, &meta);
  conn->SendFrame(meta, {});
  Message update;
  update.meta.control.cmd = Control::ADD_NODE;
  update.meta.request = false;
  update.meta.sender = kScheduler;
  update.meta.control.node.push_back(node);
  for (int id : po_->GetNodeIDs(kServerGroup | kWorkerGroup)) {
    if (id == assigned) continue;
    update.meta.recver = id;
    Message copy = update;
    SendToNode(copy, id);
  }
}

void Van::ProcessNodeListAssigned(Message& msg) {
  bool was_ready = ready_.load();
  {
    std::lock_guard<std::mutex> lk(nodes_mu_);
    for (auto& n : msg.meta.control.node) {
      auto it = nodes_.find(n.id);
      if (it != nodes_.end() && it->second.shm_uid != 0 && n.shm_uid != 0 &&
          it->second.shm_uid != n.shm_uid) {
        {
          std::lock_guard<std::mutex> lk2(conn_mu_);
          auto cit = conns_.find(n.id);
          if (cit != conns_.end()) {
            cit->second->Close();
            conns_.erase(cit);
          }
        }
        ResetFlow(n.id);
      }
      nodes_[n.id] = n;
      if (n.shm_uid == my_uid_ && n.role == my_node_.role) {
        my_node_ = n;
        po_->set_node_id(n.id);
      }
    }
  }
  if (plane_) {
    std::lock_guard<std::mutex> lk(nodes_mu_);
    for (auto& kv : nodes_) {
      if (kv.second.id != my_node_.id) plane_->OnPeer(kv.second);
    }
  }
  if (was_ready) {
    XPS_VLOG(1) << "node list update processed (" << msg.meta.control.node.size() << " nodes)";
    return;
  }
  XPS_CHECK_NE(my_node_.id, kEmptyNodeID) << "node list did not contain me";
  if (my_node_.is_recovery) {
    XPS_VLOG(1) << "recovered as " << my_node_.DebugString();
    if (plane_) plane_->ImportPeers();
  } else {
    XPS_VLOG(1) << "joined as " << my_node_.DebugString();
  }
  ready_ = true;
}

void Van::ProcessBarrierAtScheduler(Message& msg) {
  XPS_CHECK(po_->is_scheduler());
  int group = msg.meta.control.barrier_group;
  std::vector<std::pair<int, int>> release;
  {
    std::lock_guard<std::mutex> lk(sched_mu_);
    auto& waiters = barrier_waiters_[group];
    waiters.emplace_back(msg.meta.sender, msg.meta.timestamp);
    size_t expected = po_->GetNodeIDs(group).size();
    XPS_VLOG(2) << "barrier group " << group << ": " << waiters.size() << "/" << expected;
    if (waiters.size() < expected) return;
    release.swap(waiters);
  }
  std::stable_partition(release.begin(), release.end(),
                        [this](const auto& w) { return w.first != my_node_.id; });
  Message res;
  res.meta.control.cmd = Control::BARRIER;
  res.meta.request = false;
  res.meta.control.barrier_group = group;
  res.meta.sender = my_node_.id;
  for (auto& w : release) {
    res.meta.recver = w.first;
    res.meta.timestamp = w.second;
    Message copy = res;
    SendToNode(copy, w.first);
  }
}

void Van::ProcessHeartbeat(Message& msg) {
  if (msg.meta.request) {
    po_->UpdateHeartbeat(msg.meta.sender, time(nullptr));
    Message ack;
    ack.meta.control.cmd = Control::HEARTBEAT;
    ack.meta.request = false;
    ack.meta.recver = msg.meta.sender;
    Send(ack);
  } else {
    po_->UpdateHeartbeat(kScheduler, time(nullptr));
  }
}

void Van::HeartbeatLoop() {
  while (!stopping_.load()) {
    for (int i = 0; i < heartbeat_interval_ * 10 && !stopping_.load(); ++i) usleep(100 * 1000);
    if (stopping_.load()) break;
    Message hb;
    hb.meta.control.cmd = Control::HEARTBEAT;
    hb.meta.request = true;
    hb.meta.recver = kScheduler;
    Send(hb);
  }
}

void Van::MaybeTrace(const Message& msg, bool recv) {
  if (!trace_file_ || !msg.meta.control.empty()) return;
  auto now = std::chrono::duration_cast<std::chrono::microseconds>(
                 std::chrono::system_clock::now().time_since_epoch())
                 .count();
  std::lock_guard<std::mutex> lk(trace_mu_);
  fprintf(trace_file_, "%llu\t%s_van_%s_%s\t%lld\n",
          static_cast<unsigned long long>(msg.meta.key),
          po_->is_worker() ? "worker" : "server", recv ? "recv" : "send",
          msg.meta.push ? "push" : "pull", static_cast<long long>(now));
}

}
```

csrc/van.h:

```cpp
#pragma once

#include <atomic>
#include <memory>
#include <random>
#include <thread>
#include <chrono>
#include <map>
#include <unordered_map>
#include <vector>
#include <functional>

#include "message.h"
#include "tcp.h"

namespace xps {

class Postoffice;
class Resender;

class DataPlane {
 public:
  virtual ~DataPlane() = default;
  virtual bool CanSend(const Message& msg, const Node& peer) = 0;
  virtual int64_t Send(Message& msg, const Node& peer) = 0;
  virtual void OnPeer(const Node& peer) {}
  virtual void FillSelf(Node* self) {}
  virtual void ImportPeers() {}
  virtual void Stop() {}
};

class Van {
 public:
  explicit Van(Postoffice* po);
  ~Van();

  void Start(int customer_id);
  void Stop();

  int64_t Send(Message& msg);

  const Node& my_node() const { return my_node_; }
  Node GetNode(int id);
  bool IsReady() const { return ready_.load(); }

  void SetDataPlane(std::shared_ptr<DataPlane> p) { plane_ = std::move(p); }
  DataPlane* plane() const { return plane_.get(); }

  void Deliver(Message msg);
  void DeliverInline(Message& msg);

  Postoffice* postoffice() const { return po_; }

  int64_t SendOverTcp(Message& msg, int id);

  std::atomic<int64_t> send_bytes_{0};
  std::atomic<int64_t> recv_bytes_{0};

 private:
  int64_t SendToNode(Message& msg, int id);
  std::shared_ptr<TcpConn> GetOrDial(int id);
  void OnNewConnection(int fd);
  void RecvLoop(std::shared_ptr<TcpConn> conn);
  void ProcessControl(Message& msg, const std::shared_ptr<TcpConn>& conn);
  void ProcessAddNodeAtScheduler(Message& msg, const std::shared_ptr<TcpConn>& conn);
  void ProcessRecoveryAtScheduler(Message& msg, const std::shared_ptr<TcpConn>& conn);
  void ProcessNodeListAssigned(Message& msg);
  void ProcessBarrierAtScheduler(Message& msg);
  void ProcessHeartbeat(Message& msg);
  void DeliverData(Message& msg);
  void DeliverDataNow(Message& msg);
  void InlineData(Message& msg);
  void GatedDeliver(Message& msg);
  void ResetFlow(int peer_id);
  void HeartbeatLoop();

  Postoffice* po_;
  Node my_node_;
  Node scheduler_;
  uint64_t my_uid_ = 0;
  TcpListener listener_;

  std::mutex conn_mu_;
  std::mutex order_mu_;
  std::unordered_map<int, uint64_t> send_seq_;
  struct Flow {
    std::mutex mu;
    uint64_t expected = 1;
    std::map<uint64_t, Message> held;
    std::chrono::steady_clock::time_point hold_since;
  };
  std::unordered_map<int, std::unique_ptr<Flow>> recv_flows_;
  std::unordered_map<int, std::shared_ptr<TcpConn>> conns_;
  std::vector<std::thread> recv_threads_;
  std::atomic<bool> stopping_{false};

  std::mutex nodes_mu_;
  std::unordered_map<int, Node> nodes_;

  std::mutex sched_mu_;
  std::vector<std::pair<Node, std::shared_ptr<TcpConn>>> pending_nodes_;
  std::unordered_map<int, std::vector<std::pair<int, int>>> barrier_waiters_;
  std::unordered_map<int, std::unordered_map<uint64_t, time_t>> dead_ignore_;

  std::shared_ptr<DataPlane> plane_;
  std::unique_ptr<Resender> resender_;
  std::atomic<bool> ready_{false};
  int drop_rate_ = 0;
  std::mt19937 drop_rng_{12345};
  std::thread heartbeat_thread_;
  int heartbeat_interval_ = 0;

  void MaybeTrace(const Message& msg, bool recv);
  FILE* trace_file_ = nullptr;
  std::mutex trace_mu_;
};

std::function<bool(const Node&, const Node&)> NodeRankOrder(const std::vector<Node>& batch);

}
```

Measured before the change: 3828 GB/s.

## Reduce host-side overhead across send, coalescing, request tracking and node lookup paths

Bundles many independent host-path changes. It adds a small-segment hold policy to the coalescer (a floor size plus a quiet window, flushed when the caller waits), keeps per-request state in a Req struct instead of several locked maps, and adds a single-key fast path in the slicer. It also stores nodes as shared_ptr so lookups avoid copying Node, computes group size without building an ID vector, adds an atomic fast path for peer slab import, moves messages instead of copying them, skips the reorder map for in-order sequence numbers, and calls hipSetDevice only on slow paths. The hold policy can add latency to small messages, and the many concurrent changes carry correctness risk.

```diff
diff --git a/csrc/coalesce_admit.h b/csrc/coalesce_admit.h
--- a/csrc/coalesce_admit.h
+++ b/csrc/coalesce_admit.h
@@ -53,5 +53,32 @@
   return Admit::kAdmit;
 }
 
+static const int kCoFloorKb = 16 << 10;
+static const int kCoQuietUs = 40;
+
+enum class Hold {
+  kLaunch,
+  kHold,
+};
+
+inline Hold CoalesceHold(size_t open_bytes, int open_count, size_t seg_bytes, bool busy,
+                         bool same_process, size_t floor_bytes, size_t byte_cap,
+                         bool hold_mode) {
+  size_t bytes = open_bytes + seg_bytes;
+  if (open_count + 1 >= kMaxBatch2 || bytes >= byte_cap) return Hold::kLaunch;
+  if (hold_mode) return Hold::kHold;
+  if (same_process && bytes < floor_bytes) return Hold::kHold;
+  return busy ? Hold::kHold : Hold::kLaunch;
+}
+
+inline bool CoalesceHoldNeedsBusy(size_t open_bytes, int open_count, size_t seg_bytes,
+                                  bool same_process, size_t floor_bytes, size_t byte_cap,
+                                  bool hold_mode) {
+  return CoalesceHold(open_bytes, open_count, seg_bytes, false, same_process, floor_bytes,
+                      byte_cap, hold_mode) !=
+         CoalesceHold(open_bytes, open_count, seg_bytes, true, same_process, floor_bytes,
+                      byte_cap, hold_mode);
+}
+
 }
 }
diff --git a/csrc/customer.cc b/csrc/customer.cc
--- a/csrc/customer.cc
+++ b/csrc/customer.cc
@@ -22,7 +22,7 @@
 
 int Customer::NewRequest(int recver) {
   std::lock_guard<std::mutex> lk(mu_);
-  int expected = recver >= 8 ? 1 : static_cast<int>(po_->GetNodeIDs(recver).size());
+  int expected = recver >= 8 ? 1 : po_->GroupSize(recver);
   tracker_.emplace_back();
   tracker_.back().expected = expected;
   return static_cast<int>(tracker_.size()) - 1;
diff --git a/csrc/gpu_plane.cc b/csrc/gpu_plane.cc
--- a/csrc/gpu_plane.cc
+++ b/csrc/gpu_plane.cc
@@ -35,6 +35,7 @@
 }
 
 std::atomic<uint64_t> g_fused_launches{0};
+std::atomic<int> g_co_open{0};
 
 bool CoalesceEnabled() {
   static const bool on = Environment::Get()->GetInt("XPS_COALESCE", 1) != 0;
@@ -110,6 +111,10 @@
   co_hold_ = Environment::Get()->GetInt("XPS_COALESCE_HOLD", 0) != 0;
   int cap_mb = Environment::Get()->GetInt("XPS_COALESCE_CAP_MB", 1024);
   co_byte_cap_ = static_cast<size_t>(cap_mb < 1 ? 1 : cap_mb) << 20;
+  int floor_kb = Environment::Get()->GetInt("XPS_COALESCE_FLOOR_KB", kern::kCoFloorKb);
+  co_floor_bytes_ = static_cast<size_t>(floor_kb < 0 ? 0 : floor_kb) << 10;
+  int quiet_us = Environment::Get()->GetInt("XPS_COALESCE_QUIET_US", kern::kCoQuietUs);
+  co_quiet_us_ = quiet_us < 1 ? 1 : quiet_us;
 }
 
 GpuPlane::~GpuPlane() { Stop(); }
@@ -226,6 +231,7 @@
     std::atomic_store_explicit(&p->ring, std::shared_ptr<ShmRing>(),
                                std::memory_order_release);
     p->pool_tried = false;
+    p->pool_ok.store(false, std::memory_order_release);
     p->slab_bases.clear();
     p->local_po.store(nullptr, std::memory_order_release);
   }
@@ -287,6 +293,7 @@
 }
 
 bool GpuPlane::ImportPeerSlabs(Peer* p) {
+  if (p->pool_ok.load(std::memory_order_acquire)) return true;
   {
     std::lock_guard<std::mutex> lk(p->mu);
     if (p->pool_tried) return !p->slab_bases.empty();
@@ -370,6 +377,7 @@
   }
   std::lock_guard<std::mutex> lk(p->mu);
   p->slab_bases = std::move(bases);
+  p->pool_ok.store(!p->slab_bases.empty(), std::memory_order_release);
   return !p->slab_bases.empty();
 }
 
@@ -404,23 +412,31 @@
   Coalescer& co = p->co;
   if (co.n == 0) return;
   hipStream_t stream = RawLane(p, 0);
-  XPS_HIP_CHECK(hipSetDevice(device_));
-  if (co.n == 1) {
-    const kern::Seg2& s = co.segs[0];
-    kern::DenseAssign2(s.dst0, s.dst1, s.src, s.nbytes, stream);
-  } else {
-    kern::BatchedAssign2(co.segs, co.n, stream);
+  {
+    XPS_STAGE(co_launch);
+    XPS_HIP_CHECK(hipSetDevice(device_));
+    if (co.n == 1) {
+      const kern::Seg2& s = co.segs[0];
+      kern::DenseAssign2(s.dst0, s.dst1, s.src, s.nbytes, stream);
+    } else {
+      kern::BatchedAssign2(co.segs, co.n, stream);
+    }
   }
   g_fused_launches.fetch_add(1, std::memory_order_relaxed);
   hipEvent_t ev = GetEvent();
-  XPS_HIP_CHECK(hipEventRecord(ev, stream));
+  {
+    XPS_STAGE(co_event_record);
+    XPS_HIP_CHECK(hipEventRecord(ev, stream));
+  }
   co.open->bytes = co.bytes;
   co.open->ev.store(ev, std::memory_order_release);
   co.inflight.push_back(std::move(co.open));
   co.open.reset();
   co.n = 0;
   co.bytes = 0;
+  co.small_hold = false;
   co.n_open.store(0, std::memory_order_release);
+  g_co_open.fetch_sub(1, std::memory_order_acq_rel);
 }
 
 bool GpuPlane::CoBusyLocked(Peer* p) {
@@ -434,9 +450,9 @@
   auto& fl = p->co.inflight;
   while (!fl.empty()) {
     CoEvent* f = fl.front().get();
-    if (!f->done.load(std::memory_order_acquire) &&
-        hipEventQuery(f->ev.load(std::memory_order_acquire)) != hipSuccess) {
-      break;
+    if (!f->done.load(std::memory_order_acquire)) {
+      XPS_STAGE(co_event_query);
+      if (hipEventQuery(f->ev.load(std::memory_order_acquire)) != hipSuccess) break;
     }
     fl.pop_front();
   }
@@ -448,33 +464,84 @@
   CoLaunchLocked(p);
 }
 
+void GpuPlane::FlushAllOpen() {
+  if (device_ < 0) return;
+  std::vector<Peer*> all;
+  {
+    std::shared_lock<std::shared_timed_mutex> lk(peers_mu_);
+    for (auto& kv : peers_) all.push_back(kv.second.get());
+  }
+  for (Peer* p : all) CoFlush(p);
+}
+
+void GpuPlane::FlushHeld() {
+  if (g_co_open.load(std::memory_order_acquire) == 0) return;
+  XPS_STAGE(co_flush_held);
+  FlushAllOpen();
+  std::vector<GpuPlane*> local;
+  {
+    std::shared_lock<std::shared_timed_mutex> lk(peers_mu_);
+    for (auto& kv : peers_) {
+      Postoffice* lpo = LocalPeer(kv.second.get());
+      Van* van = lpo ? lpo->van() : nullptr;
+      auto* rplane = van ? dynamic_cast<GpuPlane*>(van->plane()) : nullptr;
+      if (rplane && rplane != this && rplane->device_ >= 0) local.push_back(rplane);
+    }
+  }
+  int me = po_->node_id();
+  for (GpuPlane* rplane : local) {
+    Peer* mine = nullptr;
+    {
+      std::shared_lock<std::shared_timed_mutex> lk(rplane->peers_mu_);
+      auto it = rplane->peers_.find(me);
+      if (it != rplane->peers_.end()) mine = it->second.get();
+    }
+    if (mine) rplane->CoFlush(mine);
+  }
+}
+
 std::shared_ptr<GpuPlane::CoEvent> GpuPlane::CoAppend(Peer* p, const kern::Seg2& seg) {
   if (!CoalesceEnabled()) return nullptr;
   Coalescer& co = p->co;
+  bool same_process = LocalPeer(p) != nullptr;
   std::lock_guard<std::mutex> lk(co.mu);
   kern::Admit a = kern::CoalesceAdmit(co.segs, co.n, seg);
   if (a != kern::Admit::kAdmit) CoLaunchLocked(p);
   if (a == kern::Admit::kReject) return nullptr;
   if (!co.open) co.open = std::make_shared<CoEvent>(this);
   std::shared_ptr<CoEvent> cev = co.open;
+  size_t open_bytes = co.bytes;
+  int open_count = co.n;
+  if (co.n == 0) g_co_open.fetch_add(1, std::memory_order_acq_rel);
   co.segs[co.n++] = seg;
   co.bytes += seg.nbytes;
   co.n_open.store(co.n, std::memory_order_release);
-  if (co.n >= kern::kMaxBatch || co.bytes >= co_byte_cap_) {
+  bool need_busy = kern::CoalesceHoldNeedsBusy(open_bytes, open_count, seg.nbytes, same_process,
+                                               co_floor_bytes_, co_byte_cap_, co_hold_);
+  bool busy = need_busy && CoBusyLocked(p);
+  if (kern::CoalesceHold(open_bytes, open_count, seg.nbytes, busy, same_process,
+                         co_floor_bytes_, co_byte_cap_, co_hold_) == kern::Hold::kLaunch) {
     CoLaunchLocked(p);
-  } else if (co_hold_) {
-    co.last_append_us = NowUs();
   } else {
-    if (!CoBusyLocked(p)) CoLaunchLocked(p);
+    co.small_hold = !need_busy;
+    int64_t quiet = co_hold_ ? kHoldQuietUs : (need_busy ? 0 : co_quiet_us_);
+    co.quiet_us.store(quiet, std::memory_order_relaxed);
+    co.last_append_us.store(NowUs(), std::memory_order_release);
   }
   return cev;
 }
 
 bool GpuPlane::CoFrontUnlaunched(Peer* p, const std::shared_ptr<CoEvent>& cev) {
   Coalescer& co = p->co;
+  int64_t quiet = co.quiet_us.load(std::memory_order_relaxed);
+  if (quiet > 0 && NowUs() - co.last_append_us.load(std::memory_order_acquire) < quiet) {
+    return false;
+  }
   std::lock_guard<std::mutex> lk(co.mu);
   if (co.open != cev) return true;
-  if (co_hold_ && NowUs() - co.last_append_us < kHoldQuietUs) return false;
+  if (quiet > 0 && NowUs() - co.last_append_us.load(std::memory_order_acquire) < quiet) {
+    return false;
+  }
   CoLaunchLocked(p);
   return true;
 }
@@ -483,7 +550,7 @@
   Coalescer& co = p->co;
   std::lock_guard<std::mutex> lk(co.mu);
   bool busy = CoBusyLocked(p);
-  if (!co_hold_ && !busy) CoLaunchLocked(p);
+  if (!co.small_hold && !busy) CoLaunchLocked(p);
 }
 
 bool GpuPlane::CoalesceAppend(int peer_id, const kern::Seg2& seg) {
@@ -869,7 +936,7 @@
       XPS_HIP_CHECK(hipSetDevice(device_));
       XPS_HIP_CHECK(hipEventRecord(ev, stream));
     }
-    Message resend = msg;
+    Message resend = std::move(msg);
     {
       std::lock_guard<std::mutex> lk(pend_mu_);
       pending_[p->node.id].push_back(Pending{ev, p->node.id, std::string(), std::move(resend),
@@ -877,7 +944,7 @@
     }
     pending_count_.fetch_add(1);
   } else {
-    Message copy = msg;
+    Message copy = std::move(msg);
     if (response) {
       for (auto& d : copy.data) {
         if (!d.on_device() && d.size()) {
@@ -1104,6 +1171,7 @@
   std::vector<int> ids;
   while (!stop_.load()) {
     bool did = false;
+    bool held_wait = false;
     if (pending_count_.load(std::memory_order_acquire) > 0) {
       ids.clear();
       {
@@ -1127,7 +1195,10 @@
           if (cev) {
             front_ev = cev->ev.load(std::memory_order_acquire);
             if (!front_ev) {
-              if (!CoFrontUnlaunched(GetPeer(id), cev)) break;
+              if (!CoFrontUnlaunched(GetPeer(id), cev)) {
+                held_wait = true;
+                break;
+              }
               continue;
             }
           }
@@ -1179,6 +1250,10 @@
       idle = 0;
     } else if (++idle > kSpin) {
       usleep(20);
+    } else if (held_wait) {
+      int64_t until = NowUs() + 1;
+      while (NowUs() < until) {
+      }
     }
   }
 }
diff --git a/csrc/gpu_plane.h b/csrc/gpu_plane.h
--- a/csrc/gpu_plane.h
+++ b/csrc/gpu_plane.h
@@ -22,6 +22,7 @@
 bool FusedAssignEnabled();
 extern std::atomic<uint64_t> g_fused_launches;
 bool CoalesceEnabled();
+extern std::atomic<int> g_co_open;
 
 class Postoffice;
 
@@ -44,6 +45,7 @@
 
   bool CoalesceAppend(int peer_id, const kern::Seg2& seg);
   void CoalesceEnd(int peer_id);
+  void FlushHeld();
   std::vector<std::tuple<int, int64_t, int64_t>> PeerBytes();
   int device() const { return device_; }
 
@@ -73,7 +75,9 @@
     size_t bytes = 0;
     std::shared_ptr<CoEvent> open;
     std::deque<std::shared_ptr<CoEvent>> inflight;
-    int64_t last_append_us = 0;
+    std::atomic<int64_t> last_append_us{0};
+    std::atomic<int64_t> quiet_us{0};
+    bool small_hold = false;
   };
 
   struct Peer {
@@ -85,6 +89,7 @@
     std::atomic<bool> ring_ok{false};
     std::vector<void*> slab_bases;
     bool pool_tried = false;
+    std::atomic<bool> pool_ok{false};
     std::atomic<hipStream_t> streams[2] = {{nullptr}, {nullptr}};
     std::atomic<int64_t> tx_bytes{0};
     std::atomic<int64_t> rx_bytes{0};
@@ -121,6 +126,7 @@
   void CoPruneLocked(Peer* p);
   bool CoBusyLocked(Peer* p);
   void CoFlush(Peer* p);
+  void FlushAllOpen();
   bool CoFrontUnlaunched(Peer* p, const std::shared_ptr<CoEvent>& cev);
   void CoRetired(Peer* p);
   std::shared_ptr<CoEvent> TakeTicket(int peer_id);
@@ -132,6 +138,8 @@
   int device_;
   int lanes_ = 2;
   bool co_hold_ = false;
+  size_t co_floor_bytes_ = 0;
+  int64_t co_quiet_us_ = 0;
   size_t co_byte_cap_ = 1ull << 30;
   uint64_t my_host_hash_;
   ShmRing in_ring_;
diff --git a/csrc/kv_app.h b/csrc/kv_app.h
--- a/csrc/kv_app.h
+++ b/csrc/kv_app.h
@@ -8,6 +8,7 @@
 #include <condition_variable>
 #include <functional>
 #include <mutex>
+#include <optional>
 #include <set>
 #include <unordered_map>
 #include <vector>
@@ -56,6 +57,24 @@
   using SlicedKVs = std::vector<std::pair<bool, KVPairs<V>>>;
   using Slicer = std::function<void(const KVPairs<V>&, const std::vector<Range>&, SlicedKVs*)>;
 
+ private:
+  struct RecvSlice {
+    KVPairs<V> kvs;
+    int option = 0;
+    int64_t val_len = 0;
+  };
+  struct Req {
+    Callback cb;
+    int expected = 0;
+    int acks = 0;
+    std::vector<RecvSlice> got;
+    SArray<V>* dst_vals = nullptr;
+    SArray<int>* dst_lens = nullptr;
+    std::vector<V>* vec_vals = nullptr;
+    std::vector<int>* vec_lens = nullptr;
+  };
+
+ public:
   explicit KVWorker(int app_id, int customer_id, int instance_idx = 0)
       : SimpleApp(Postoffice::GetWorker(instance_idx), DeferCustomer{}) {
     slicer_ = [this](const KVPairs<V>& s, const std::vector<Range>& r, SlicedKVs* out) {
@@ -80,13 +99,14 @@
   int ZPush(const SArray<Key>& keys, const SArray<V>& vals, const SArray<int>& lens = {},
             int cmd = 0, const Callback& cb = nullptr, const SArray<Key>& keys_dev = {}) {
     int ts = obj_->NewRequest(kServerGroup);
-    AddCallback(ts, cb);
+    Req req;
+    req.cb = cb;
     KVPairs<V> kvs;
     kvs.keys = keys;
     kvs.vals = vals;
     kvs.lens = lens;
     kvs.keys_dev = keys_dev;
-    Send(ts, true, false, cmd, kvs);
+    Send(ts, true, false, cmd, kvs, std::move(req));
     return ts;
   }
 
@@ -95,17 +115,15 @@
                 const SArray<Key>& keys_dev = {}) {
     XPS_CHECK(outs && outs->size()) << "ZPushPull needs a pre-sized outs buffer";
     int ts = obj_->NewRequest(kServerGroup);
-    {
-      std::lock_guard<std::mutex> lk(mu_);
-      pull_dst_[ts] = {outs, nullptr};
-    }
-    AddCallback(ts, cb);
+    Req req;
+    req.cb = cb;
+    req.dst_vals = outs;
     KVPairs<V> kvs;
     kvs.keys = keys;
     kvs.vals = vals;
     kvs.lens = lens;
     kvs.keys_dev = keys_dev;
-    Send(ts, true, true, cmd, kvs, outs);
+    Send(ts, true, true, cmd, kvs, std::move(req), outs);
     return ts;
   }
 
@@ -113,21 +131,26 @@
             const Callback& cb = nullptr, const SArray<Key>& keys_dev = {}) {
     XPS_CHECK(vals && vals->size()) << "ZPull needs a pre-sized vals buffer";
     int ts = obj_->NewRequest(kServerGroup);
-    {
-      std::lock_guard<std::mutex> lk(mu_);
-      pull_dst_[ts] = {vals, lens};
-    }
-    AddCallback(ts, cb);
+    Req req;
+    req.cb = cb;
+    req.dst_vals = vals;
+    req.dst_lens = lens;
     KVPairs<V> kvs;
     kvs.keys = keys;
     kvs.vals = *vals;
     if (lens) kvs.lens = *lens;
     kvs.keys_dev = keys_dev;
-    Send(ts, false, true, cmd, kvs);
+    Send(ts, false, true, cmd, kvs, std::move(req));
     return ts;
   }
 
-  void Wait(int timestamp) { obj_->WaitRequest(timestamp); }
+  void Wait(int timestamp) {
+    if (g_co_open.load(std::memory_order_acquire) > 0 && !obj_->IsFinished(timestamp)) {
+      auto* plane = dynamic_cast<GpuPlane*>(po_->van()->plane());
+      if (plane) plane->FlushHeld();
+    }
+    obj_->WaitRequest(timestamp);
+  }
 
   bool HasEntry(const Key& key, size_t nbytes) {
     const auto& ranges = po_->GetServerKeyRanges();
@@ -138,7 +161,7 @@
     std::lock_guard<std::mutex> lk(mu_);
     const EntryRec* rec = FindEntryLocked(sid, key);
     return rec && rec->len == static_cast<int64_t>(nbytes) &&
-           po_->van()->GetNode(sid).shm_uid == rec->uid;
+           po_->van()->NodeShmUid(sid) == rec->uid;
   }
 
   void set_slicer(Slicer s) { slicer_ = std::move(s); }
@@ -146,6 +169,20 @@
   void DefaultSlicer(const KVPairs<V>& send, const std::vector<Range>& ranges, SlicedKVs* sliced) {
     sliced->resize(ranges.size());
     size_t n = send.keys.size();
+    if (n == 1) {
+      if (!send.lens.empty()) XPS_CHECK_EQ(send.lens.size(), n);
+      Key k = send.keys[0];
+      size_t i = ranges.size();
+      while (i > 0 && ranges[i - 1].begin > k) --i;
+      if (i > 0) {
+        (*sliced)[i - 1].first = true;
+        KVPairs<V>& out = (*sliced)[i - 1].second;
+        out = send;
+        size_t len = send.lens.empty() ? send.vals.size() : static_cast<size_t>(send.lens[0]);
+        if (!send.vals.empty() && len != send.vals.size()) out.vals = send.vals.Segment(0, len);
+      }
+      return;
+    }
     std::vector<size_t> pos(ranges.size() + 1);
     const Key* begin = send.keys.begin();
     const Key* end = send.keys.end();
@@ -183,33 +220,30 @@
   int AddPullRequest_(const SArray<Key>& keys, std::vector<V>* vals, std::vector<int>* lens,
                       int cmd, const Callback& cb) {
     int ts = obj_->NewRequest(kServerGroup);
-    {
-      std::lock_guard<std::mutex> lk(mu_);
-      vec_pull_dst_[ts] = {vals, lens};
-    }
-    AddCallback(ts, cb);
+    Req req;
+    req.cb = cb;
+    req.vec_vals = vals;
+    req.vec_lens = lens;
     KVPairs<V> kvs;
     kvs.keys = keys;
-    Send(ts, false, true, cmd, kvs);
+    Send(ts, false, true, cmd, kvs, std::move(req));
     return ts;
   }
 
-  void AddCallback(int ts, const Callback& cb) {
-    if (!cb) return;
-    std::lock_guard<std::mutex> lk(mu_);
-    callbacks_[ts] = cb;
-  }
-
-  void Send(int ts, bool push, bool pull, int cmd, KVPairs<V>& kvs, SArray<V>* dst = nullptr) {
+  void Send(int ts, bool push, bool pull, int cmd, KVPairs<V>& kvs, Req req,
+            SArray<V>* dst = nullptr) {
+    static StageStat prep_stat("worker_send_prep");
+    std::optional<StageScope> prep(std::in_place, &prep_stat);
     SlicedKVs sliced;
     slicer_(kvs, po_->GetServerKeyRanges(), &sliced);
     int skipped = 0;
     for (auto& s : sliced)
       if (!s.first) ++skipped;
     if (skipped) obj_->AddResponse(ts, skipped);
+    req.expected = static_cast<int>(sliced.size()) - skipped;
     {
       std::lock_guard<std::mutex> lk(mu_);
-      expected_[ts] = static_cast<int>(sliced.size()) - skipped;
+      reqs_.emplace(ts, std::move(req));
     }
     if (static_cast<int>(sliced.size()) == skipped) {
       RunCallback(ts);
@@ -248,7 +282,7 @@
               auto it = nit->second.find(s.keys[0]);
               if (it != nit->second.end() &&
                   it->second.len == static_cast<int64_t>(s.vals.nbytes()) &&
-                  po_->van()->GetNode(msg.meta.recver).shm_uid == it->second.uid) {
+                  po_->van()->NodeShmUid(msg.meta.recver) == it->second.uid) {
                 msg.meta.addr = it->second.off;
                 msg.meta.option |= kOptEntryPush;
                 it->second.one_sided = true;
@@ -281,7 +315,7 @@
             std::lock_guard<std::mutex> lk(mu_);
             const EntryRec* rec = FindEntryLocked(msg.meta.recver, s.keys[0]);
             if (rec && rec->len == static_cast<int64_t>(s.vals.nbytes()) &&
-                po_->van()->GetNode(msg.meta.recver).shm_uid == rec->uid) {
+                po_->van()->NodeShmUid(msg.meta.recver) == rec->uid) {
               msg.meta.entry_addr = rec->off;
               msg.meta.option |= kOptEntryPush;
             }
@@ -299,7 +333,7 @@
               auto it = nit->second.find(s.keys[0]);
               if (it != nit->second.end() && it->second.one_sided &&
                   it->second.len == static_cast<int64_t>(s.vals.nbytes()) &&
-                  po_->van()->GetNode(msg.meta.recver).shm_uid == it->second.uid) {
+                  po_->van()->NodeShmUid(msg.meta.recver) == it->second.uid) {
                 eoff = it->second.off;
                 hit = true;
               }
@@ -342,7 +376,9 @@
         }
         if (!s.lens.empty()) msg.AddData(s.lens);
       }
+      prep.reset();
       po_->van()->Send(msg);
+      prep.emplace(&prep_stat);
       if (push && pull && s.keys.size() == 1) {
         bool did = (msg.meta.option & kOptEntryPush) && (msg.meta.option & kOptInPlace);
         std::lock_guard<std::mutex> lk(mu_);
@@ -371,57 +407,49 @@
         kvs.keys = SArray<Key>({msg.meta.key});
       }
     }
+    Req done;
     {
       std::lock_guard<std::mutex> lk(mu_);
       if (msg.meta.pull) {
         if (msg.meta.push && (msg.meta.option & kOptEntryAddr)) {
           CacheEntryLocked(msg.meta.sender, msg.meta.key, msg.meta.entry_addr, msg.meta.val_len);
         }
-        auto& got = recv_kvs_[ts];
-        got.push_back(RecvSlice{kvs, msg.meta.option, msg.meta.val_len});
-        last = static_cast<int>(got.size()) >= expected_[ts];
+      } else if (msg.meta.option & kOptEntryAddr) {
+        CacheEntryLocked(msg.meta.sender, msg.meta.key, msg.meta.addr, msg.meta.val_len);
+      }
+      auto it = reqs_.find(ts);
+      if (it == reqs_.end()) return;
+      Req& r = it->second;
+      if (msg.meta.pull) {
+        r.got.push_back(RecvSlice{kvs, msg.meta.option, msg.meta.val_len});
+        last = static_cast<int>(r.got.size()) >= r.expected;
       } else {
-        if (msg.meta.option & kOptEntryAddr) {
-          CacheEntryLocked(msg.meta.sender, msg.meta.key, msg.meta.addr, msg.meta.val_len);
-        }
-        int n = ++push_acks_[ts];
-        last = n >= expected_[ts];
+        last = ++r.acks >= r.expected;
+      }
+      if (last) {
+        done = std::move(r);
+        reqs_.erase(it);
       }
     }
     if (last) {
-      if (msg.meta.pull) MergePull(ts);
-      RunCallback(ts);
-    }
-  }
-
-  void MergePull(int ts) {
-    std::vector<RecvSlice> got;
-    SArray<V>* dst_vals = nullptr;
-    SArray<int>* dst_lens = nullptr;
-    std::vector<V>* vec_vals = nullptr;
-    std::vector<int>* vec_lens = nullptr;
-    {
-      std::lock_guard<std::mutex> lk(mu_);
-      got.swap(recv_kvs_[ts]);
-      recv_kvs_.erase(ts);
-      auto it = pull_dst_.find(ts);
-      if (it != pull_dst_.end()) {
-        dst_vals = it->second.first;
-        dst_lens = it->second.second;
-        pull_dst_.erase(it);
-      }
-      auto it2 = vec_pull_dst_.find(ts);
-      if (it2 != vec_pull_dst_.end()) {
-        vec_vals = it2->second.first;
-        vec_lens = it2->second.second;
-        vec_pull_dst_.erase(it2);
-      }
-    }
-    std::sort(got.begin(), got.end(), [](const RecvSlice& a, const RecvSlice& b) {
-      Key ka = a.kvs.keys.empty() ? 0 : a.kvs.keys[0];
-      Key kb = b.kvs.keys.empty() ? 0 : b.kvs.keys[0];
-      return ka < kb;
-    });
+      if (msg.meta.pull) MergePull(&done);
+      if (done.cb) done.cb();
+    }
+  }
+
+  void MergePull(Req* req) {
+    std::vector<RecvSlice>& got = req->got;
+    SArray<V>* dst_vals = req->dst_vals;
+    SArray<int>* dst_lens = req->dst_lens;
+    std::vector<V>* vec_vals = req->vec_vals;
+    std::vector<int>* vec_lens = req->vec_lens;
+    if (got.size() > 1) {
+      std::sort(got.begin(), got.end(), [](const RecvSlice& a, const RecvSlice& b) {
+        Key ka = a.kvs.keys.empty() ? 0 : a.kvs.keys[0];
+        Key kb = b.kvs.keys.empty() ? 0 : b.kvs.keys[0];
+        return ka < kb;
+      });
+    }
     if (vec_vals) {
       vec_vals->clear();
       if (vec_lens) vec_lens->clear();
@@ -465,22 +493,13 @@
     Callback cb;
     {
       std::lock_guard<std::mutex> lk(mu_);
-      auto it = callbacks_.find(ts);
-      if (it != callbacks_.end()) {
-        cb = it->second;
-        callbacks_.erase(it);
-      }
-      expected_.erase(ts);
-      push_acks_.erase(ts);
+      auto it = reqs_.find(ts);
+      if (it == reqs_.end()) return;
+      cb = std::move(it->second.cb);
+      reqs_.erase(it);
     }
     if (cb) cb();
   }
-
-  struct RecvSlice {
-    KVPairs<V> kvs;
-    int option = 0;
-    int64_t val_len = 0;
-  };
 
   struct EntryRec {
     uint64_t off;
@@ -491,7 +510,7 @@
   std::unordered_map<int, std::unordered_map<Key, EntryRec>> entry_cache_;
 
   void CacheEntryLocked(int server_id, Key key, uint64_t off, int64_t len) {
-    entry_cache_[server_id][key] = EntryRec{off, len, po_->van()->GetNode(server_id).shm_uid};
+    entry_cache_[server_id][key] = EntryRec{off, len, po_->van()->NodeShmUid(server_id)};
   }
 
   const EntryRec* FindEntryLocked(int server_id, Key key) const {
@@ -503,12 +522,7 @@
 
   Slicer slicer_;
   std::mutex mu_;
-  std::unordered_map<int, Callback> callbacks_;
-  std::unordered_map<int, int> expected_;
-  std::unordered_map<int, int> push_acks_;
-  std::unordered_map<int, std::vector<RecvSlice>> recv_kvs_;
-  std::unordered_map<int, std::pair<SArray<V>*, SArray<int>*>> pull_dst_;
-  std::unordered_map<int, std::pair<std::vector<V>*, std::vector<int>*>> vec_pull_dst_;
+  std::unordered_map<int, Req> reqs_;
 };
 
 template <typename V>
diff --git a/csrc/message.h b/csrc/message.h
--- a/csrc/message.h
+++ b/csrc/message.h
@@ -121,6 +121,10 @@
   template <typename V>
   void AddData(const SArray<V>& v) {
     XPS_CHECK_LT(data.size(), 4u);
+    if (data.empty()) {
+      data.reserve(4);
+      meta.data_type.reserve(4);
+    }
     meta.data_type.push_back(DataTypeOf<V>());
     data.push_back(SArray<char>::View(v));
   }
diff --git a/csrc/postoffice.cc b/csrc/postoffice.cc
--- a/csrc/postoffice.cc
+++ b/csrc/postoffice.cc
@@ -65,6 +65,7 @@
 }
 
 const std::vector<Range>& Postoffice::GetServerKeyRanges() {
+  if (ranges_set_.load(std::memory_order_acquire)) return server_key_ranges_;
   std::lock_guard<std::mutex> lk(mu_);
   if (server_key_ranges_.empty()) {
     int n = std::max(num_servers_, 1);
@@ -76,6 +77,7 @@
       server_key_ranges_.push_back(r);
     }
   }
+  ranges_set_.store(true, std::memory_order_release);
   return server_key_ranges_;
 }
 
@@ -90,15 +92,23 @@
 
 void Postoffice::RemoveCustomer(Customer* c) {
   std::lock_guard<std::mutex> lk(mu_);
+  if (hot_customer_.load(std::memory_order_relaxed) == c) {
+    hot_customer_.store(nullptr, std::memory_order_release);
+  }
   customers_.erase((c->app_id() << 16) | (c->customer_id() & 0xFFFF));
 }
 
 Customer* Postoffice::GetCustomer(int app_id, int customer_id, int timeout_sec) const {
+  Customer* hot = hot_customer_.load(std::memory_order_acquire);
+  if (hot && hot->app_id() == app_id && hot->customer_id() == customer_id) return hot;
   int key = (app_id << 16) | (customer_id & 0xFFFF);
   std::unique_lock<std::mutex> lk(mu_);
   bool ok = customer_cv_.wait_for(lk, std::chrono::seconds(timeout_sec),
                                   [&] { return customers_.count(key) > 0; });
-  return ok ? customers_.at(key) : nullptr;
+  if (!ok) return nullptr;
+  Customer* c = customers_.at(key);
+  hot_customer_.store(c, std::memory_order_release);
+  return c;
 }
 
 void Postoffice::Barrier(int customer_id, int group) {
diff --git a/csrc/postoffice.h b/csrc/postoffice.h
--- a/csrc/postoffice.h
+++ b/csrc/postoffice.h
@@ -45,6 +45,10 @@
   void set_preferred_rank(int r) { preferred_rank_ = r; }
 
   std::vector<int> GetNodeIDs(int group) const;
+  int GroupSize(int group) const {
+    return ((group & kScheduler) ? 1 : 0) + ((group & kServerGroup) ? num_servers_ : 0) +
+           ((group & kWorkerGroup) ? num_workers_ : 0);
+  }
   const std::vector<Range>& GetServerKeyRanges();
 
   void AddCustomer(Customer* c);
@@ -80,6 +84,7 @@
   mutable std::mutex mu_;
   std::unordered_map<int, Customer*> customers_;
   mutable std::condition_variable customer_cv_;
+  mutable std::atomic<Customer*> hot_customer_{nullptr};
 
   std::mutex barrier_mu_;
   std::condition_variable barrier_cv_;
@@ -93,6 +98,7 @@
   time_t start_time_ = time(nullptr);
 
   std::vector<Range> server_key_ranges_;
+  std::atomic<bool> ranges_set_{false};
   std::function<void()> exit_cb_;
 };
 
diff --git a/csrc/pybind.cc b/csrc/pybind.cc
--- a/csrc/pybind.cc
+++ b/csrc/pybind.cc
@@ -564,6 +564,20 @@
           }
         },
         py::arg("open"), py::arg("seg"));
+  m.def("coalesce_hold",
+        [](size_t open_bytes, int open_count, size_t seg_bytes, bool busy, bool same_process,
+           size_t floor_bytes, size_t byte_cap, bool hold_mode) {
+          return kern::CoalesceHold(open_bytes, open_count, seg_bytes, busy, same_process,
+                                    floor_bytes, byte_cap, hold_mode) == kern::Hold::kLaunch
+                     ? "launch"
+                     : "hold";
+        },
+        py::arg("open_bytes"), py::arg("open_count"), py::arg("seg_bytes"), py::arg("busy"),
+        py::arg("same_process"), py::arg("floor_bytes"), py::arg("byte_cap"),
+        py::arg("hold_mode") = false);
+  m.attr("COALESCE_MAX_BATCH") = kern::kMaxBatch2;
+  m.attr("COALESCE_FLOOR_KB") = kern::kCoFloorKb;
+  m.attr("COALESCE_QUIET_US") = kern::kCoQuietUs;
   m.def("tile_runs",
         [](const std::vector<unsigned long long>& chunk_counts,
            unsigned long long chunks_per_block, unsigned long long block_index) {
diff --git a/csrc/server_handlers.cc b/csrc/server_handlers.cc
--- a/csrc/server_handlers.cc
+++ b/csrc/server_handlers.cc
@@ -139,13 +139,13 @@
   char* dst = plane->PeerDst(req.sender, req.addr, len);
   if (!dst) return false;
   XPS_STAGE(dense_fused_assign);
-  XPS_HIP_CHECK(hipSetDevice(HbmPool::Get()->device()));
   Entry* e;
   {
     std::lock_guard<std::mutex> lk(mu_);
     e = &store_[kvs.keys[0]];
     if (e->buf.size() < len) {
       if (!e->buf.empty()) e->retired.push_back(e->buf);
+      XPS_HIP_CHECK(hipSetDevice(HbmPool::Get()->device()));
       e->buf = HbmPool::Get()->AllocArray(len);
       XPS_HIP_CHECK(hipMemset(e->buf.data(), 0, len));
     }
@@ -157,6 +157,7 @@
   bool coalesced = !chain && !e->last_ev &&
                    plane->CoalesceAppend(req.sender, kern::Seg2{e->buf.data(), dst, src, len});
   if (!coalesced) {
+    XPS_HIP_CHECK(hipSetDevice(HbmPool::Get()->device()));
     hipStream_t stream = Stream(req.sender);
     OrderAfter(e, stream);
     kern::DenseAssign2(e->buf.data(), dst, src, len, stream);
diff --git a/csrc/van.cc b/csrc/van.cc
--- a/csrc/van.cc
+++ b/csrc/van.cc
@@ -6,6 +6,7 @@
 
 #include <algorithm>
 #include <chrono>
+#include <optional>
 #include <random>
 #include <set>
 
@@ -76,7 +77,7 @@
     po_->set_node_id(kScheduler);
     {
       std::lock_guard<std::mutex> lk(nodes_mu_);
-      nodes_[kScheduler] = my_node_;
+      nodes_[kScheduler] = std::make_shared<const Node>(my_node_);
     }
     if (po_->num_workers() + po_->num_servers() == 0) ready_ = true;
   } else {
@@ -91,7 +92,7 @@
     }
     {
       std::lock_guard<std::mutex> lk(nodes_mu_);
-      nodes_[kScheduler] = scheduler_;
+      nodes_[kScheduler] = std::make_shared<const Node>(scheduler_);
     }
     Message req;
     req.meta.control.cmd = Control::ADD_NODE;
@@ -142,7 +143,14 @@
   std::lock_guard<std::mutex> lk(nodes_mu_);
   auto it = nodes_.find(id);
   XPS_CHECK(it != nodes_.end()) << "unknown node id " << id;
-  return it->second;
+  return *it->second;
+}
+
+uint64_t Van::NodeShmUid(int id) {
+  std::lock_guard<std::mutex> lk(nodes_mu_);
+  auto it = nodes_.find(id);
+  XPS_CHECK(it != nodes_.end()) << "unknown node id " << id;
+  return it->second->shm_uid;
 }
 
 int64_t Van::Send(Message& msg) {
@@ -174,14 +182,14 @@
     return approx;
   }
   if (plane_ && msg.meta.control.empty()) {
-    Node peer;
+    std::shared_ptr<const Node> peer;
     {
       std::lock_guard<std::mutex> lk(nodes_mu_);
       auto it = nodes_.find(id);
       if (it != nodes_.end()) peer = it->second;
     }
-    if (peer.id != kEmptyNodeID && plane_->CanSend(msg, peer)) {
-      int64_t n = plane_->Send(msg, peer);
+    if (peer && peer->id != kEmptyNodeID && plane_->CanSend(msg, *peer)) {
+      int64_t n = plane_->Send(msg, *peer);
       if (n >= 0) {
         send_bytes_ += n;
         return n;
@@ -221,7 +229,7 @@
     std::lock_guard<std::mutex> lk(nodes_mu_);
     auto it = nodes_.find(id);
     if (it == nodes_.end()) return nullptr;
-    n = it->second;
+    n = *it->second;
   }
   int fd = TcpConnect(n.hostname, n.port, 20);
   if (fd < 0) return nullptr;
@@ -321,6 +329,8 @@
 }
 
 void Van::GatedDeliver(Message& msg) {
+  static StageStat gate_stat("gated_deliver");
+  std::optional<StageScope> gate(std::in_place, &gate_stat);
   uint64_t seq = msg.meta.seq;
   Flow* f;
   {
@@ -331,11 +341,19 @@
   }
   std::unique_lock<std::mutex> lk(f->mu);
   if (seq < f->expected) {
+    gate.reset();
+    InlineData(msg);
+    return;
+  }
+  if (seq == f->expected && f->held.empty()) {
+    f->expected++;
+    gate.reset();
     InlineData(msg);
     return;
   }
   if (f->held.empty()) f->hold_since = std::chrono::steady_clock::now();
   f->held.emplace(seq, std::move(msg));
+  gate.reset();
   while (!f->held.empty() && f->held.begin()->first == f->expected) {
     Message m = std::move(f->held.begin()->second);
     f->held.erase(f->held.begin());
@@ -529,7 +547,7 @@
   {
     std::lock_guard<std::mutex> lk(nodes_mu_);
     for (auto& p : batch) {
-      nodes_[p.first.id] = p.first;
+      nodes_[p.first.id] = std::make_shared<const Node>(p.first);
       reply.meta.control.node.push_back(p.first);
     }
   }
@@ -573,7 +591,7 @@
   XPS_VLOG(1) << "scheduler: recovering node " << assigned << " as " << node.DebugString();
   {
     std::lock_guard<std::mutex> lk(nodes_mu_);
-    nodes_[assigned] = node;
+    nodes_[assigned] = std::make_shared<const Node>(node);
   }
   {
     std::lock_guard<std::mutex> lk(conn_mu_);
@@ -588,7 +606,7 @@
   reply.meta.recver = assigned;
   {
     std::lock_guard<std::mutex> lk(nodes_mu_);
-    for (auto& kv : nodes_) reply.meta.control.node.push_back(kv.second);
+    for (auto& kv : nodes_) reply.meta.control.node.push_back(*kv.second);
   }
   std::string meta;
   PackMeta(reply.meta, &meta);
@@ -612,8 +630,8 @@
     std::lock_guard<std::mutex> lk(nodes_mu_);
     for (auto& n : msg.meta.control.node) {
       auto it = nodes_.find(n.id);
-      if (it != nodes_.end() && it->second.shm_uid != 0 && n.shm_uid != 0 &&
-          it->second.shm_uid != n.shm_uid) {
+      if (it != nodes_.end() && it->second->shm_uid != 0 && n.shm_uid != 0 &&
+          it->second->shm_uid != n.shm_uid) {
         {
           std::lock_guard<std::mutex> lk2(conn_mu_);
           auto cit = conns_.find(n.id);
@@ -624,7 +642,7 @@
         }
         ResetFlow(n.id);
       }
-      nodes_[n.id] = n;
+      nodes_[n.id] = std::make_shared<const Node>(n);
       if (n.shm_uid == my_uid_ && n.role == my_node_.role) {
         my_node_ = n;
         po_->set_node_id(n.id);
@@ -634,7 +652,7 @@
   if (plane_) {
     std::lock_guard<std::mutex> lk(nodes_mu_);
     for (auto& kv : nodes_) {
-      if (kv.second.id != my_node_.id) plane_->OnPeer(kv.second);
+      if (kv.second->id != my_node_.id) plane_->OnPeer(*kv.second);
     }
   }
   if (was_ready) {
diff --git a/csrc/van.h b/csrc/van.h
--- a/csrc/van.h
+++ b/csrc/van.h
@@ -41,6 +41,7 @@
 
   const Node& my_node() const { return my_node_; }
   Node GetNode(int id);
+  uint64_t NodeShmUid(int id);
   bool IsReady() const { return ready_.load(); }
 
   void SetDataPlane(std::shared_ptr<DataPlane> p) { plane_ = std::move(p); }
@@ -95,7 +96,7 @@
   std::atomic<bool> stopping_{false};
 
   std::mutex nodes_mu_;
-  std::unordered_map<int, Node> nodes_;
+  std::unordered_map<int, std::shared_ptr<const Node>> nodes_;
 
   std::mutex sched_mu_;
   std::vector<std::pair<Node, std::shared_ptr<TcpConn>>> pending_nodes_;
```

New measurement: 3834 GB/s, median of 4. Within noise of the previous version (+0.2%).
